# 192459/lmc-atomi

Measured on AMD Instinct MI355X. Metric: lmc_chain_iterations_per_s, higher is better.
Workload: dtype f32; 1 GPU; 512x512 MYULA deblur (5x5 uniform box blur, sigma=0.75) + isotropic TV prox K=10 (tau_reg=0.3), 1024 chains/GPU x 1 GPU, Philox noise, x0=0, posterior moments every 1 it; chains_per_gpu=1024, chains_total=1024, tv_iters=10, sampler=MYULA (algs.py:477-587), parallelism=chains sharded x1, collective=none

## Files before the change

include/lmc_atomi.h:

```cpp
#ifndef LMC_ATOMI_H
#define LMC_ATOMI_H

#include <stddef.h>
#include <stdint.h>

#ifdef __cplusplus
extern "C" {
#endif

#define LMC_ATOMI_ABI_VERSION 3

typedef enum lmc_status {
  LMC_OK = 0,
  LMC_E_INVALID = -1,
  LMC_E_UNSUPPORTED = -2,
  LMC_E_HIP = -3,
  LMC_E_NOMEM = -4,
  LMC_E_STATE = -5
} lmc_status;

typedef enum lmc_data_kind {
  LMC_DATA_NONE = 0,
  LMC_DATA_IDENTITY = 1,
  LMC_DATA_BLUR = 2,
  LMC_DATA_MASK = 3
} lmc_data_kind;

typedef enum lmc_prior_kind {
  LMC_PRIOR_NONE = 0,
  LMC_PRIOR_L2 = 1,
  LMC_PRIOR_L1 = 2,
  LMC_PRIOR_TV_ISO = 3,
  LMC_PRIOR_TV_ANISO = 4,
  LMC_PRIOR_HAAR_L1 = 5,
  LMC_PRIOR_EPROX = 6
} lmc_prior_kind;

typedef enum lmc_ncvx_kind {
  LMC_NCVX_NONE = 0,
  LMC_NCVX_MC_TV = 1,
  LMC_NCVX_ME_TV = 2,
  LMC_NCVX_MC_TV_ANISO = 3,
  LMC_NCVX_ME_TV_ANISO = 4
} lmc_ncvx_kind;

typedef enum lmc_noise_mode {
  LMC_NOISE_PHILOX = 0,
  LMC_NOISE_INJECTED = 1,
  LMC_NOISE_NONE = 2
} lmc_noise_mode;

#define LMC_MAX_BLUR 9
#define LMC_MAX_TV_ITERS 64

typedef struct lmc_problem {
  uint32_t struct_size;
  int32_t H, W;
  int32_t data_kind;
  float sigma_f;
  const float* y_dev;
  const float* mask_dev;
  int32_t kh, kw, oy, ox;
  const float* h_host;
  int32_t prior_kind;
  float prior_sigma;
  int32_t tv_niter;
  float tv_step;
  const float* tv_betas_host;
  int32_t ncvx_kind;
  float ncvx_lambda;
  float ncvx_gamma;
  int32_t ncvx_niter;
  int32_t tv_lagged_output;
  float tv_rtol;
  int32_t step_variant;
  float implicit_tol;
  int32_t tv_warm;
  float ncvx_rtol;
  int32_t tv_exit_path;
  int32_t iterations_per_launch;
  int32_t moments_overlap;
  int32_t moments_bg_workgroups;
  int32_t graph_replay;
  int32_t eprox_kind;
  float eprox_p0, eprox_p1;
  int32_t eprox_scale_mask;
  const float* prox_scale;
  int64_t prox_scale_chain_stride;
  int32_t prox_scale_pixel_stride;
} lmc_problem;

int lmc_version(void);
const char* lmc_last_error(void);
int lmc_device_info(int* device, int* n_cu, size_t* lds_bytes, size_t* hbm_bytes);
int lmc_hbm_copy_probe(size_t bytes, int32_t reps, float* gbs_out, void* stream);


int lmc_blur(const float* x_dev, float* out_dev, int64_t n_img, int32_t H, int32_t W,
             const float* h_host, int32_t kh, int32_t kw, int32_t oy, int32_t ox, int32_t adjoint, void* stream);

int lmc_gradient(const float* x_dev, float* out_dev, int64_t n_img, int32_t H, int32_t W, void* stream);
int lmc_gradient_adjoint(const float* y_dev, float* out_dev, int64_t n_img, int32_t H, int32_t W, void* stream);

int lmc_fused_eval(const lmc_problem* prob, const float* x_dev, float* out_dev, int64_t n_img,
                   float a, float t, float b, float pt, void* stream);

size_t lmc_l2_prox_workspace_bytes(int64_t n_img, int32_t H, int32_t W);
int lmc_l2_prox(const lmc_problem* prob, const float* x_dev, float* out_dev, int64_t n_img, float tau, int32_t niter,
                int32_t warm, void* workspace_dev, void* stream);

int lmc_energies(const lmc_problem* prob, const float* x_dev, int64_t n_img,
                 double* f_out_dev, double* g_out_dev, void* stream);

int lmc_haar_l1_prox(const float* x_dev, float* out_dev, int64_t n_img, int32_t H, int32_t W, float thr, void* stream);

int lmc_chain_probes(const float* x_dev, float* out_dev, int64_t n_img, int32_t H, int32_t W, int32_t ph, int32_t pw, void* stream);

int lmc_dual_project(const float* y_dev, float* out_dev, int64_t n_img, int32_t H, int32_t W,
                     float radius, int32_t isotropic, void* stream);

typedef enum lmc_eprox_kind {
  LMC_EPROX_LAPLACE = 0,
  LMC_EPROX_UNCENTERED_LAPLACE = 1,
  LMC_EPROX_GAUSSIAN = 2,
  LMC_EPROX_GEN_GAUSSIAN_4_3 = 3,
  LMC_EPROX_GEN_GAUSSIAN_3_2 = 4,
  LMC_EPROX_GEN_GAUSSIAN_3 = 5,
  LMC_EPROX_GEN_GAUSSIAN_4 = 6,
  LMC_EPROX_HUBER = 7,
  LMC_EPROX_SMOOTHED_LAPLACE = 8,
  LMC_EPROX_EXP = 9,
  LMC_EPROX_GAMMA = 10,
  LMC_EPROX_CHI = 11,
  LMC_EPROX_UNIFORM = 12,
  LMC_EPROX_TRIANGULAR = 13,
  LMC_EPROX_LAPLACE_CONJ = 14
} lmc_eprox_kind;
int lmc_prox_elementwise(int32_t kind, const float* x_dev, float* out_dev, int64_t n,
                         const float* params_host, int32_t n_params, void* stream);


typedef struct lmc_sampler lmc_sampler;

typedef struct lmc_myula_config {
  uint32_t struct_size;
  lmc_problem problem;
  int32_t n_chains;
  int64_t chain_offset;
  float tau, gamma, epsg;
  uint64_t seed;
  int32_t noise_mode;
  int32_t moments;
  int32_t burn_in;
  int32_t thin;
} lmc_myula_config;

int lmc_myula_create(const lmc_myula_config* cfg, lmc_sampler** out);
void lmc_sampler_destroy(lmc_sampler* s);

int lmc_mymala_create(const lmc_myula_config* cfg, lmc_sampler** out);
int lmc_sampler_get_acceptance(lmc_sampler* s, uint64_t* accepted_dev, double* last_log_alpha_dev, void* stream);

int lmc_sampler_set_state(lmc_sampler* s, const float* x_dev, void* stream);
int lmc_sampler_get_state(lmc_sampler* s, float* x_dev, void* stream);
int lmc_sampler_step(lmc_sampler* s, int32_t n_iters, const float* noise_dev, void* stream);
int64_t lmc_sampler_iteration(const lmc_sampler* s);
int lmc_sampler_set_iteration(lmc_sampler* s, int64_t it);

int lmc_sampler_get_moments(lmc_sampler* s, double* sum_dev, double* sumsq_dev, uint64_t* count, void* stream);
int lmc_sampler_reset_moments(lmc_sampler* s, void* stream);
int lmc_sampler_energies(lmc_sampler* s, double* f_out_dev, double* g_out_dev, void* stream);
int lmc_sampler_noise(lmc_sampler* s, int64_t iteration, float* out_dev, void* stream);
int lmc_sampler_enable_timing(lmc_sampler* s, int32_t on);
int lmc_sampler_last_step_timing(lmc_sampler* s, float* total_ms, int32_t* n_launches);
const char* lmc_sampler_kernel_name(const lmc_sampler* s);
int lmc_sampler_tv_exit_stats(lmc_sampler* s, int32_t which, int32_t* passes_dev, uint64_t* reruns_host, void* stream);

#define LMC_RCCL_UNIQUE_ID_BYTES 128
int lmc_rccl_available(void);
int lmc_rccl_unique_id(void* id128_host);
int lmc_rccl_comm_create(void** comm_out, int32_t world, int32_t rank, const void* id128_host);
int lmc_rccl_comm_destroy(void* comm);
int lmc_allreduce_moments(lmc_sampler* s, void* rccl_comm, double* sum_dev, double* sumsq_dev, uint64_t* count, void* stream);

typedef struct lmc_ulpda_config {
  uint32_t struct_size;
  lmc_problem problem;
  int32_t n_chains;
  int64_t chain_offset;
  float tau, mu, theta;
  int32_t gfirst;
  int32_t cg_niter;
  int32_t warm;
  const float* z_dev;
  uint64_t seed;
  int32_t noise_mode;
  int32_t moments, burn_in, thin;
} lmc_ulpda_config;

int lmc_ulpda_create(const lmc_ulpda_config* cfg, lmc_sampler** out);
int lmc_sampler_set_dual(lmc_sampler* s, const float* y_dev, void* stream);
int lmc_sampler_get_dual(lmc_sampler* s, float* y_dev, void* stream);
int lmc_sampler_set_steps(lmc_sampler* s, float tau, float mu);

float lmc_set_cg_tolerance(float tol);

int lmc_set_step_variant(int32_t variant);

#ifdef __cplusplus
}
#endif
#endif
```

lmc_atomi_amd/_capi.py:

```python
from __future__ import annotations

import ctypes as C
import os
import threading

_HERE = os.path.dirname(os.path.abspath(__file__))
LIB_PATH = os.path.join(_HERE, "lib", "liblmc_atomi.so")
ABI_VERSION = 3

DATA_NONE, DATA_IDENTITY, DATA_BLUR, DATA_MASK = 0, 1, 2, 3
PRIOR_NONE, PRIOR_L2, PRIOR_L1, PRIOR_TV_ISO, PRIOR_TV_ANISO, PRIOR_HAAR_L1, PRIOR_EPROX = 0, 1, 2, 3, 4, 5, 6
NOISE_PHILOX, NOISE_INJECTED, NOISE_NONE = 0, 1, 2
NCVX_NONE, NCVX_MC_TV, NCVX_ME_TV, NCVX_MC_TV_ANISO, NCVX_ME_TV_ANISO = 0, 1, 2, 3, 4
MAX_BLUR = 9
MAX_TV_ITERS = 64
(EPROX_LAPLACE, EPROX_UNCENTERED_LAPLACE, EPROX_GAUSSIAN, EPROX_GEN_GAUSSIAN_4_3, EPROX_GEN_GAUSSIAN_3_2,
 EPROX_GEN_GAUSSIAN_3, EPROX_GEN_GAUSSIAN_4, EPROX_HUBER, EPROX_SMOOTHED_LAPLACE, EPROX_EXP, EPROX_GAMMA,
 EPROX_CHI, EPROX_UNIFORM, EPROX_TRIANGULAR, EPROX_LAPLACE_CONJ) = range(15)


class LMCError(RuntimeError):

    def __init__(self, code, msg):
        super().__init__(f"liblmc_atomi error {code}: {msg}")
        self.code = code


class lmc_problem(C.Structure):
    _fields_ = [
        ("struct_size", C.c_uint32),
        ("H", C.c_int32), ("W", C.c_int32),
        ("data_kind", C.c_int32),
        ("sigma_f", C.c_float),
        ("y_dev", C.c_void_p),
        ("mask_dev", C.c_void_p),
        ("kh", C.c_int32), ("kw", C.c_int32), ("oy", C.c_int32), ("ox", C.c_int32),
        ("h_host", C.POINTER(C.c_float)),
        ("prior_kind", C.c_int32),
        ("prior_sigma", C.c_float),
        ("tv_niter", C.c_int32),
        ("tv_step", C.c_float),
        ("tv_betas_host", C.POINTER(C.c_float)),
        ("ncvx_kind", C.c_int32),
        ("ncvx_lambda", C.c_float),
        ("ncvx_gamma", C.c_float),
        ("ncvx_niter", C.c_int32),
        ("tv_lagged_output", C.c_int32),
        ("tv_rtol", C.c_float),
        ("step_variant", C.c_int32),
        ("implicit_tol", C.c_float),
        ("tv_warm", C.c_int32),
        ("ncvx_rtol", C.c_float),
        ("tv_exit_path", C.c_int32),
        ("iterations_per_launch", C.c_int32),
        ("moments_overlap", C.c_int32),
        ("moments_bg_workgroups", C.c_int32),
        ("graph_replay", C.c_int32),
        ("eprox_kind", C.c_int32), ("eprox_p0", C.c_float), ("eprox_p1", C.c_float), ("eprox_scale_mask", C.c_int32),
        ("prox_scale", C.c_void_p), ("prox_scale_chain_stride", C.c_int64), ("prox_scale_pixel_stride", C.c_int32),
    ]


class lmc_myula_config(C.Structure):
    _fields_ = [
        ("struct_size", C.c_uint32),
        ("problem", lmc_problem),
        ("n_chains", C.c_int32),
        ("chain_offset", C.c_int64),
        ("tau", C.c_float), ("gamma", C.c_float), ("epsg", C.c_float),
        ("seed", C.c_uint64),
        ("noise_mode", C.c_int32),
        ("moments", C.c_int32),
        ("burn_in", C.c_int32),
        ("thin", C.c_int32),
    ]


class lmc_ulpda_config(C.Structure):
    _fields_ = [
        ("struct_size", C.c_uint32),
        ("problem", lmc_problem),
        ("n_chains", C.c_int32),
        ("chain_offset", C.c_int64),
        ("tau", C.c_float), ("mu", C.c_float), ("theta", C.c_float),
        ("gfirst", C.c_int32),
        ("cg_niter", C.c_int32),
        ("warm", C.c_int32),
        ("z_dev", C.c_void_p),
        ("seed", C.c_uint64),
        ("noise_mode", C.c_int32),
        ("moments", C.c_int32), ("burn_in", C.c_int32), ("thin", C.c_int32),
    ]


_P = C.c_void_p
_F = C.POINTER(C.c_float)
_SIGNATURES = {
    "lmc_version": (C.c_int, []),
    "lmc_last_error": (C.c_char_p, []),
    "lmc_device_info": (C.c_int, [C.POINTER(C.c_int), C.POINTER(C.c_int), C.POINTER(C.c_size_t), C.POINTER(C.c_size_t)]),
    "lmc_hbm_copy_probe": (C.c_int, [C.c_size_t, C.c_int32, C.POINTER(C.c_float), _P]),
    "lmc_blur": (C.c_int, [_P, _P, C.c_int64, C.c_int32, C.c_int32, _F, C.c_int32, C.c_int32, C.c_int32, C.c_int32, C.c_int32, _P]),
    "lmc_gradient": (C.c_int, [_P, _P, C.c_int64, C.c_int32, C.c_int32, _P]),
    "lmc_gradient_adjoint": (C.c_int, [_P, _P, C.c_int64, C.c_int32, C.c_int32, _P]),
    "lmc_fused_eval": (C.c_int, [C.POINTER(lmc_problem), _P, _P, C.c_int64, C.c_float, C.c_float, C.c_float, C.c_float, _P]),
    "lmc_l2_prox_workspace_bytes": (C.c_size_t, [C.c_int64, C.c_int32, C.c_int32]),
    "lmc_l2_prox": (C.c_int, [C.POINTER(lmc_problem), _P, _P, C.c_int64, C.c_float, C.c_int32, C.c_int32, _P, _P]),
    "lmc_energies": (C.c_int, [C.POINTER(lmc_problem), _P, C.c_int64, _P, _P, _P]),
    "lmc_mymala_create": (C.c_int, [C.POINTER(lmc_myula_config), C.POINTER(_P)]),
    "lmc_sampler_get_acceptance": (C.c_int, [_P, _P, _P, _P]),
    "lmc_set_cg_tolerance": (C.c_float, [C.c_float]),
    "lmc_chain_probes": (C.c_int, [_P, _P, C.c_int64, C.c_int32, C.c_int32, C.c_int32, C.c_int32, _P]),
    "lmc_haar_l1_prox": (C.c_int, [_P, _P, C.c_int64, C.c_int32, C.c_int32, C.c_float, _P]),
    "lmc_dual_project": (C.c_int, [_P, _P, C.c_int64, C.c_int32, C.c_int32, C.c_float, C.c_int32, _P]),
    "lmc_prox_elementwise": (C.c_int, [C.c_int32, _P, _P, C.c_int64, _F, C.c_int32, _P]),
    "lmc_myula_create": (C.c_int, [C.POINTER(lmc_myula_config), C.POINTER(_P)]),
    "lmc_sampler_destroy": (None, [_P]),
    "lmc_sampler_set_state": (C.c_int, [_P, _P, _P]),
    "lmc_sampler_get_state": (C.c_int, [_P, _P, _P]),
    "lmc_sampler_step": (C.c_int, [_P, C.c_int32, _P, _P]),
    "lmc_sampler_iteration": (C.c_int64, [_P]),
    "lmc_sampler_set_iteration": (C.c_int, [_P, C.c_int64]),
    "lmc_sampler_get_moments": (C.c_int, [_P, _P, _P, C.POINTER(C.c_uint64), _P]),
    "lmc_sampler_reset_moments": (C.c_int, [_P, _P]),
    "lmc_sampler_energies": (C.c_int, [_P, _P, _P, _P]),
    "lmc_sampler_noise": (C.c_int, [_P, C.c_int64, _P, _P]),
    "lmc_sampler_enable_timing": (C.c_int, [_P, C.c_int32]),
    "lmc_sampler_last_step_timing": (C.c_int, [_P, C.POINTER(C.c_float), C.POINTER(C.c_int32)]),
    "lmc_sampler_kernel_name": (C.c_char_p, [_P]),
    "lmc_sampler_tv_exit_stats": (C.c_int, [_P, C.c_int32, _P, C.POINTER(C.c_uint64), _P]),
    "lmc_set_step_variant": (C.c_int, [C.c_int32]),
    "lmc_ulpda_create": (C.c_int, [C.POINTER(lmc_ulpda_config), C.POINTER(_P)]),
    "lmc_sampler_set_dual": (C.c_int, [_P, _P, _P]),
    "lmc_sampler_get_dual": (C.c_int, [_P, _P, _P]),
    "lmc_sampler_set_steps": (C.c_int, [_P, C.c_float, C.c_float]),
    "lmc_rccl_available": (C.c_int, []),
    "lmc_rccl_unique_id": (C.c_int, [_P]),
    "lmc_rccl_comm_create": (C.c_int, [C.POINTER(_P), C.c_int32, C.c_int32, _P]),
    "lmc_rccl_comm_destroy": (C.c_int, [_P]),
    "lmc_allreduce_moments": (C.c_int, [_P, _P, _P, _P, C.POINTER(C.c_uint64), _P]),
}
RCCL_UNIQUE_ID_BYTES = 128
VARIANTS = ["auto", "tile", "(removed)", "split", "point", "block", "rows", "pipe", "pipe2"]

_lib = None
_lock = threading.Lock()


def load(path: str | None = None):
    global _lib
    with _lock:
        if _lib is not None:
            return _lib
        import torch
        p = path or os.environ.get("LMC_ATOMI_LIB", LIB_PATH)
        if not os.path.exists(p):
            raise ImportError(
                f"{p} not found: build it with `python -c 'import __graft_entry__ as g; g.build()'` "
                "(or `make -C lmc_atomi_amd/csrc`).  lmc_atomi_amd has no CPU fallback.")
        lib = C.CDLL(p, mode=C.RTLD_GLOBAL)
        for name, (res, args) in _SIGNATURES.items():
            fn = getattr(lib, name)
            fn.restype = res
            fn.argtypes = args
        v = lib.lmc_version()
        if v != ABI_VERSION:
            raise ImportError(f"liblmc_atomi ABI {v} != binding ABI {ABI_VERSION}")
        _lib = lib
        return lib


def check(rc: int):
    if rc != 0:
        raise LMCError(rc, load().lmc_last_error().decode("utf-8", "replace"))


def exported_symbols():
    return sorted(_SIGNATURES)
```

lmc_atomi_amd/algs.py:

```python
from __future__ import annotations

import ctypes as C
import time

import numpy as np
import torch
from numpy.random import default_rng

from . import _capi, _dev
from .proximal import _Problem


def _prior_descriptor(proxg):
    if proxg is None:
        return {"prior_kind": _capi.PRIOR_NONE}
    fn = getattr(proxg, "prior_descriptor", None)
    if fn is None:
        raise NotImplementedError(
            f"{type(proxg).__name__} has no device functor (prior_descriptor()); new proxes are added as "
            "functors compiled into liblmc_atomi -- there is no CPU fallback")
    return fn()


def _data_descriptor(proxf):
    if proxf is None:
        return {"data_kind": _capi.DATA_NONE}
    fn = getattr(proxf, "descriptor", None)
    if fn is None:
        raise NotImplementedError(f"{type(proxf).__name__} has no device functor (descriptor())")
    return fn()


class MYULASampler:

    def __init__(self, proxf, proxg, dims, n_chains=1, tau=None, gamma=0.1, epsg=1.0, seed=0,
                 chain_offset=0, noise="philox", moments=False, burn_in=0, thin=1, device=None, variant=None, tv_warm=None, policy=None):
        if tau is None:
            raise NotImplementedError("tau=None (backtracking) is not implemented by the reference loop either")
        self.dims = (int(dims[0]), int(dims[1]))
        self.n_chains = int(n_chains)
        self.device = _dev.device(device)
        self.proxf, self.proxg = proxf, proxg
        opts = {"step_variant": variant or 0}
        if tv_warm is not None:
            opts["tv_warm"] = bool(tv_warm)
        opts.update(policy or {})
        self.epsg = epsg
        if np.asarray(epsg).size > 1:
            opts["prox_scale"] = self._epsg_array(epsg)
            epsg = 1.0
        self._problem = _Problem(self.dims, _data_descriptor(proxf), _prior_descriptor(proxg), self.device, options=opts)
        cfg = _capi.lmc_myula_config()
        cfg.struct_size = C.sizeof(_capi.lmc_myula_config)
        cfg.problem = self._problem.c
        cfg.n_chains = self.n_chains
        cfg.chain_offset = int(chain_offset)
        cfg.tau, cfg.gamma, cfg.epsg = float(tau), float(gamma), float(epsg)
        cfg.seed = int(seed) & 0xFFFFFFFFFFFFFFFF
        cfg.noise_mode = {"philox": _capi.NOISE_PHILOX, "injected": _capi.NOISE_INJECTED, "none": _capi.NOISE_NONE}[noise]
        cfg.moments = 1 if moments else 0
        cfg.burn_in = int(burn_in)
        cfg.thin = int(thin)
        self.noise_mode = noise
        self.moments_on = bool(moments)
        self._h = C.c_void_p()
        with torch.cuda.device(self.device):
            _capi.check(getattr(_dev.lib(), self._create_fn)(C.byref(cfg), C.byref(self._h)))

    _create_fn = "lmc_myula_create"

    def _epsg_array(self, epsg):
        e = np.asarray(epsg, dtype=np.float32)
        n = self.dims[0] * self.dims[1]
        if e.size == n and e.shape in ((n,), self.dims):
            cs, ps = 0, 1
        elif e.shape == (self.n_chains,):
            cs, ps = 1, 0
        elif e.size == self.n_chains * n and e.shape[0] == self.n_chains:
            cs, ps = n, 1
        else:
            raise ValueError(f"epsg of shape {e.shape} matches neither the image {self.dims}, nor the {self.n_chains} chains, nor both")
        return _dev.to_dev(np.ascontiguousarray(e.ravel()), self.device), cs, ps

    def close(self):
        if getattr(self, "_h", None) is not None and self._h.value:
            _dev.lib().lmc_sampler_destroy(self._h)
            self._h = C.c_void_p()

    __del__ = close

    def __enter__(self):
        return self

    def __exit__(self, *exc):
        self.close()

    @property
    def shape(self):
        return (self.n_chains,) + self.dims

    def set_state(self, x):
        xt = _dev.to_dev(x, self.device)
        n = self.dims[0] * self.dims[1]
        if xt.numel() == n:
            xt = xt.reshape(1, *self.dims).expand(self.shape).contiguous()
        if xt.numel() != self.n_chains * n:
            raise ValueError(f"state of shape {tuple(xt.shape)} does not match {self.shape}")
        _capi.check(_dev.lib().lmc_sampler_set_state(self._h, _dev.ptr(xt), _dev.stream_ptr(self.device)))
        torch.cuda.current_stream(self.device).synchronize()

    def get_state(self, out=None):
        if out is None:
            out = torch.empty(self.shape, dtype=torch.float32, device=self.device)
        _capi.check(_dev.lib().lmc_sampler_get_state(self._h, _dev.ptr(out), _dev.stream_ptr(self.device)))
        return out

    @property
    def iteration(self):
        return int(_dev.lib().lmc_sampler_iteration(self._h))

    @iteration.setter
    def iteration(self, it):
        _capi.check(_dev.lib().lmc_sampler_set_iteration(self._h, int(it)))

    def step(self, n_iters=1, noise=None):
        nt = None
        if noise is not None:
            nt = _dev.to_dev(noise, self.device)
            if nt.numel() != n_iters * self.n_chains * self.dims[0] * self.dims[1]:
                raise ValueError("noise must have shape [n_iters, n_chains, H, W]")
        _capi.check(_dev.lib().lmc_sampler_step(self._h, int(n_iters), _dev.ptr(nt), _dev.stream_ptr(self.device)))
        if nt is not None:
            torch.cuda.current_stream(self.device).synchronize()

    def enable_timing(self, on=True):
        _capi.check(_dev.lib().lmc_sampler_enable_timing(self._h, 1 if on else 0))

    def last_step_timing(self):
        ms, n = C.c_float(), C.c_int32()
        _capi.check(_dev.lib().lmc_sampler_last_step_timing(self._h, C.byref(ms), C.byref(n)))
        return ms.value, n.value

    @property
    def kernel_name(self):
        return _dev.lib().lmc_sampler_kernel_name(self._h).decode()

    def tv_exit_stats(self, which="prior"):
        passes = torch.empty(self.n_chains, dtype=torch.int32, device=self.device)
        rr = (C.c_uint64 * 4)()
        _capi.check(_dev.lib().lmc_sampler_tv_exit_stats(self._h, {"prior": 0, "ncvx": 1}[which], _dev.ptr(passes), rr, _dev.stream_ptr(self.device)))
        return passes, [int(v) for v in rr]

    def energies(self):
        f = torch.empty(self.n_chains, dtype=torch.float64, device=self.device)
        g = torch.empty(self.n_chains, dtype=torch.float64, device=self.device)
        _capi.check(_dev.lib().lmc_sampler_energies(self._h, _dev.ptr(f), _dev.ptr(g), _dev.stream_ptr(self.device)))
        return f, g

    def noise_field(self, iteration):
        out = torch.empty(self.shape, dtype=torch.float32, device=self.device)
        _capi.check(_dev.lib().lmc_sampler_noise(self._h, int(iteration), _dev.ptr(out), _dev.stream_ptr(self.device)))
        return out

    def moments(self):
        s1 = torch.empty(self.dims, dtype=torch.float64, device=self.device)
        s2 = torch.empty(self.dims, dtype=torch.float64, device=self.device)
        cnt = C.c_uint64()
        _capi.check(_dev.lib().lmc_sampler_get_moments(self._h, _dev.ptr(s1), _dev.ptr(s2), C.byref(cnt),
                                                       _dev.stream_ptr(self.device)))
        return s1, s2, int(cnt.value)

    def reset_moments(self):
        _capi.check(_dev.lib().lmc_sampler_reset_moments(self._h, _dev.stream_ptr(self.device)))

    def allreduce_moments(self, rccl_comm):
        s1 = torch.empty(self.dims, dtype=torch.float64, device=self.device)
        s2 = torch.empty(self.dims, dtype=torch.float64, device=self.device)
        cnt = C.c_uint64()
        comm = rccl_comm if isinstance(rccl_comm, C.c_void_p) else C.c_void_p(int(rccl_comm or 0))
        _capi.check(_dev.lib().lmc_allreduce_moments(self._h, comm, _dev.ptr(s1), _dev.ptr(s2), C.byref(cnt),
                                                     _dev.stream_ptr(self.device)))
        return s1, s2, int(cnt.value)


class ULPDASampler(MYULASampler):

    def __init__(self, proxf, proxg, A, dims, n_chains=1, tau=None, mu=None, theta=1.0, gfirst=True, z=None, seed=0,
                 chain_offset=0, noise="philox", moments=False, burn_in=0, thin=1, device=None, variant=None, implicit_tol=None):
        from .operators import Gradient
        from .proximal import L1, L21
        if not isinstance(A, Gradient):
            raise NotImplementedError("ULPDA on the GPU supports A = Gradient (the reference's operator, prox_lmc_deconv.py:98)")
        if isinstance(proxg, L21):
            prior = {"prior_kind": _capi.PRIOR_TV_ISO, "prior_sigma": proxg.sigma, "tv_niter": 1, "tv_betas": [0.0]}
        elif isinstance(proxg, L1):
            prior = {"prior_kind": _capi.PRIOR_TV_ANISO, "prior_sigma": proxg.sigma}
        else:
            raise NotImplementedError(f"{type(proxg).__name__} has no dual-prox device functor (L21 or L1 expected)")
        self.dims = (int(dims[0]), int(dims[1]))
        self.n_chains = int(n_chains)
        self.device = _dev.device(device)
        self.proxf, self.proxg = proxf, proxg
        tol = 0.0 if implicit_tol is None else (float(implicit_tol) if implicit_tol > 0 else -1.0)
        self._problem = _Problem(self.dims, _data_descriptor(proxf), prior, self.device,
                                 options={"step_variant": variant or 0, "implicit_tol": tol})
        cfg = _capi.lmc_ulpda_config()
        cfg.struct_size = C.sizeof(_capi.lmc_ulpda_config)
        cfg.problem = self._problem.c
        cfg.n_chains = self.n_chains
        cfg.chain_offset = int(chain_offset)
        cfg.tau, cfg.mu, cfg.theta = float(tau), float(mu), float(theta)
        cfg.gfirst = 1 if gfirst else 0
        cfg.cg_niter = int(getattr(proxf, "niter", 10) or 10)
        cfg.warm = 1 if getattr(proxf, "warm", True) else 0
        self._z = None
        if z is not None:
            self._z = _dev.to_dev(z, self.device).reshape(self.dims)
            cfg.z_dev = self._z.data_ptr()
        cfg.seed = int(seed) & 0xFFFFFFFFFFFFFFFF
        cfg.noise_mode = {"philox": _capi.NOISE_PHILOX, "injected": _capi.NOISE_INJECTED, "none": _capi.NOISE_NONE}[noise]
        cfg.moments = 1 if moments else 0
        cfg.burn_in = int(burn_in)
        cfg.thin = int(thin)
        self.noise_mode = noise
        self.moments_on = bool(moments)
        self._h = C.c_void_p()
        with torch.cuda.device(self.device):
            _capi.check(_dev.lib().lmc_ulpda_create(C.byref(cfg), C.byref(self._h)))

    def set_steps(self, tau, mu):
        _capi.check(_dev.lib().lmc_sampler_set_steps(self._h, float(tau), float(mu)))

    def set_dual(self, y):
        yt = _dev.to_dev(y, self.device)
        n2 = 2 * self.dims[0] * self.dims[1]
        if yt.numel() == n2:
            yt = yt.reshape(1, n2).expand(self.n_chains, n2).contiguous()
        if yt.numel() != self.n_chains * n2:
            raise ValueError("dual state must have 2*H*W entries per chain")
        _capi.check(_dev.lib().lmc_sampler_set_dual(self._h, _dev.ptr(yt), _dev.stream_ptr(self.device)))
        torch.cuda.current_stream(self.device).synchronize()

    def get_dual(self):
        out = torch.empty((self.n_chains, 2) + self.dims, dtype=torch.float32, device=self.device)
        _capi.check(_dev.lib().lmc_sampler_get_dual(self._h, _dev.ptr(out), _dev.stream_ptr(self.device)))
        return out


def UnadjustedLangevinPrimalDual(proxf, proxg, A, x0, tau, mu, y0=None, z=None, theta=1., niter=10, seed=0, gfirst=True,
                                 callback=None, callbacky=False, returny=False, show=False, *, n_chains=None, dims=None,
                                 rng="philox", chain_offset=0, burn_in=0, thin=1, device=None, diagnostics=None):
    if dims is None:
        dims = getattr(A, "dims", None) or getattr(proxf, "dims", None)
    if dims is None:
        raise ValueError("image shape unknown: pass dims=(ny, nx)")
    many = n_chains is not None
    C_ = int(n_chains) if many else 1
    n = int(dims[0]) * int(dims[1])
    if rng not in ("philox", "pcg64"):
        raise ValueError("rng must be 'philox' or 'pcg64'")
    if rng == "pcg64" and C_ != 1:
        raise ValueError("rng='pcg64' reproduces the reference's single chain; use n_chains=None")
    taus = np.full(niter, tau, dtype=np.float64) if np.isscalar(tau) else np.asarray(tau, dtype=np.float64)
    mus = np.full(niter, mu, dtype=np.float64) if np.isscalar(mu) else np.asarray(mu, dtype=np.float64)
    smp = ULPDASampler(proxf, proxg, A, dims, n_chains=C_, tau=taus[0], mu=mus[0], theta=theta, gfirst=gfirst, z=z,
                       seed=seed, chain_offset=chain_offset, noise="injected" if rng == "pcg64" else "philox",
                       moments=many, burn_in=burn_in, thin=thin, device=device)
    try:
        smp.set_state(x0)
        if y0 is not None:
            smp.set_dual(y0)
        tstart = time.time()
        if show:
            print('Unadjusted Langevin primal-dual (lmc_atomi_amd / HIP): U(x) = f(x) + x^T z + g(Ax)\n'
                  '---------------------------------------------------------\n'
                  'Proximal operator (f): %s\nProximal operator (g): %s\nLinear operator (A): %s\n'
                  'tau = %s\t\tmu = %s\ntheta = %.2f\t\tniter = %d\tchains = %d\n' %
                  (type(proxf), type(proxg), type(A), str(taus[0]), str(mus[0]), theta, niter, C_))
            print('   Itn       x[0]          f         g o A      U = f + g o A')
        host_rng = default_rng(seed) if rng == "pcg64" else None
        xs = np.empty((niter, n), dtype=np.float64) if not many else None
        ys = np.empty((niter, 2 * n), dtype=np.float64) if (returny and not many) else None
        tracer = None
        if diagnostics and many:
            from .diagnostics import ChainTrace
            tracer = ChainTrace(smp, (8, 8) if diagnostics is True else diagnostics)
        for it in range(niter):
            smp.set_steps(taus[it], mus[it])
            if host_rng is not None:
                xi = host_rng.standard_normal(n)
                smp.step(1, noise=xi.reshape(1, 1, *smp.dims))
            else:
                smp.step(1)
            if not many:
                xs[it] = smp.get_state().reshape(-1).cpu().numpy()
                if returny or callbacky:
                    yk = smp.get_dual().reshape(-1).cpu().numpy()
                    if returny:
                        ys[it] = yk
                if callback is not None:
                    callback(xs[it], yk) if callbacky else callback(xs[it])
            elif callback is not None:
                callback(smp.get_state(), smp.get_dual()) if callbacky else callback(smp.get_state())
            if tracer is not None and it >= burn_in and (it - burn_in) % thin == 0:
                tracer.record()
            if show and (it < 10 or niter - it < 10 or it % max(niter // 10, 1) == 0):
                f, g = smp.energies()
                x00 = float(smp.get_state().reshape(-1)[0])
                print('%6g  %12.5e  %10.3e  %10.3e      %10.3e' % (it + 1, x00, float(f.mean()), float(g.mean()),
                                                                  float((f + g).mean())))
        if show:
            print('\nTotal time (s) = %.2f' % (time.time() - tstart))
            print('---------------------------------------------------------\n')
        if not many:
            return (xs, ys) if returny else xs
        s1, s2, cnt = smp.moments()
        f, g = smp.energies()
        state = smp.get_state()
        torch.cuda.current_stream().synchronize()
        mean, var = mean_var_from_moments(s1, s2, max(cnt, 1))
        diag = tracer.summary() if tracer is not None and len(tracer) else None
        return MYULAResult(state, mean, var, cnt, f, g, time.time() - tstart, diagnostics=diag,
                           trace=tracer.trace() if diag is not None else None)
    finally:
        smp.close()


def mean_var_from_moments(s1, s2, count):
    mean = s1 / count
    var = s2 / count - mean * mean
    return mean, var


class MYULAResult:

    def __init__(self, state, mean, var, count, energy_f, energy_g, elapsed, diagnostics=None, trace=None):
        self.state, self.mean, self.var, self.count = state, mean, var, count
        self.energy_f, self.energy_g, self.elapsed = energy_f, energy_g, elapsed
        self.diagnostics, self.trace = diagnostics, trace


def MoreauYosidaUnadjustedLangevin(proxf, proxg, x0, tau=None, gamma=.1, epsg=1., niter=10, seed=0,
                                   callback=None, show=False, *, n_chains=None, dims=None, rng="philox",
                                   chain_offset=0, burn_in=0, thin=1, device=None, diagnostics=None):
    if dims is None:
        dims = getattr(proxf, "dims", None) or getattr(proxg, "dims", None)
    if dims is None:
        raise ValueError("image shape unknown: pass dims=(ny, nx)")
    many = n_chains is not None
    C_ = int(n_chains) if many else 1
    n = int(dims[0]) * int(dims[1])
    if rng not in ("philox", "pcg64"):
        raise ValueError("rng must be 'philox' or 'pcg64'")
    if rng == "pcg64" and C_ != 1:
        raise ValueError("rng='pcg64' reproduces the reference's single chain; use n_chains=None")
    smp = MYULASampler(proxf, proxg, dims, n_chains=C_, tau=tau, gamma=gamma, epsg=epsg, seed=seed,
                       chain_offset=chain_offset, noise="injected" if rng == "pcg64" else "philox",
                       moments=many, burn_in=burn_in, thin=thin, device=device)
    try:
        smp.set_state(x0)
        tstart = time.time()
        if show:
            print('Moreau--Yosida Unadjusted Langevin (lmc_atomi_amd / HIP)\n'
                  '---------------------------------------------------------\n'
                  'Proximal operator (f): %s\nProximal operator (g): %s\n'
                  'tau = %s\tgamma=%10e\nepsg = %s\tniter = %d\tchains = %d\n' %
                  (type(proxf), type(proxg), str(tau), gamma, str(epsg) if np.asarray(epsg).size == 1 else 'Multi', niter, C_))
            print('   Itn       x[0]          f           g     J = f + eps*g')
        if not many:
            samples = np.empty((niter, n), dtype=np.asarray(x0).dtype if not isinstance(x0, torch.Tensor) else np.float32)
            host_rng = default_rng(seed) if rng == "pcg64" else None
            buf = torch.empty(smp.shape, dtype=torch.float32, device=smp.device)
            for it in range(niter):
                if host_rng is not None:
                    xi = host_rng.standard_normal(n)
                    smp.step(1, noise=xi.reshape(1, 1, *smp.dims))
                else:
                    smp.step(1)
                smp.get_state(buf)
                xk = buf.reshape(-1).cpu().numpy()
                samples[it] = xk
                if callback is not None:
                    callback(samples[it])
                if show and (it < 10 or niter - it < 10 or it % max(niter // 10, 1) == 0):
                    f, g = smp.energies()
                    pf, pg = float(f[0]), float(g[0])
                    print('%6g  %12.5e  %10.3e  %10.3e  %10.3e' % (it + 1, samples[it][0], pf, pg, pf + float(np.sum(epsg * pg))))
            if show:
                print('\nTotal time (s) = %.2f' % (time.time() - tstart))
                print('---------------------------------------------------------\n')
            return samples
        tracer = None
        if diagnostics:
            from .diagnostics import ChainTrace
            tracer = ChainTrace(smp, (8, 8) if diagnostics is True else diagnostics)
        next_rec = burn_in + 1
        done = 0
        while done < niter:
            chunk = niter - done if (callback is None and not show) else 1
            if tracer is not None and next_rec > done:
                chunk = min(chunk, next_rec - done)
            smp.step(chunk)
            done += chunk
            if tracer is not None and done == next_rec:
                tracer.record()
                next_rec += thin
            if callback is not None:
                callback(smp.get_state())
            if show and (done <= 10 or niter - done < 10 or (done - 1) % max(niter // 10, 1) == 0):
                f, g = smp.energies()
                x00 = float(smp.get_state()[0, 0, 0])
                print('%6g  %12.5e  %10.3e  %10.3e  %10.3e' % (done, x00, float(f.mean()), float(g.mean()),
                                                              float((f + (epsg if np.asarray(epsg).size == 1 else float(np.sum(epsg))) * g).mean())))
        s1, s2, cnt = smp.moments()
        f, g = smp.energies()
        state = smp.get_state()
        torch.cuda.current_stream().synchronize()
        mean, var = mean_var_from_moments(s1, s2, max(cnt, 1))
        diag = tracer.summary() if tracer is not None and len(tracer) else None
        return MYULAResult(state, mean, var, cnt, f, g, time.time() - tstart, diagnostics=diag,
                           trace=tracer.trace() if diag is not None else None)
    finally:
        smp.close()


class MYMALASampler(MYULASampler):

    _create_fn = "lmc_mymala_create"

    def acceptance(self):
        acc = torch.empty(self.n_chains, dtype=torch.int64, device=self.device)
        la = torch.empty(self.n_chains, dtype=torch.float64, device=self.device)
        _capi.check(_dev.lib().lmc_sampler_get_acceptance(self._h, _dev.ptr(acc), _dev.ptr(la), _dev.stream_ptr(self.device)))
        return acc, la

    def acceptance_rate(self):
        acc, _ = self.acceptance()
        return acc.double() / max(self.iteration, 1)


def MoreauYosidaMetropolisAdjustedLangevin(proxf, proxg, x0, tau=None, gamma=.1, epsg=1., niter=10, seed=0, callback=None, *,
                                           n_chains=1, dims=None, chain_offset=0, burn_in=0, thin=1, device=None):
    if dims is None:
        dims = getattr(proxf, "dims", None) or getattr(proxg, "dims", None)
    if dims is None:
        raise ValueError("image shape unknown: pass dims=(ny, nx)")
    smp = MYMALASampler(proxf, proxg, dims, n_chains=int(n_chains), tau=tau, gamma=gamma, epsg=epsg, seed=seed,
                        chain_offset=chain_offset, moments=True, burn_in=burn_in, thin=thin, device=device)
    try:
        smp.set_state(x0)
        tstart = time.time()
        if callback is None:
            smp.step(niter)
        else:
            for _ in range(niter):
                smp.step(1)
                callback(smp.get_state())
        s1, s2, cnt = smp.moments()
        f, g = smp.energies()
        state = smp.get_state()
        acc, _ = smp.acceptance()
        torch.cuda.current_stream().synchronize()
        mean, var = mean_var_from_moments(s1, s2, max(cnt, 1))
        res = MYULAResult(state, mean, var, cnt, f, g, time.time() - tstart)
        res.accepted = acc
        res.acceptance_rate = acc.double() / max(niter, 1)
        return res
    finally:
        smp.close()


def set_cg_tolerance(tol=1e-6):
    return float(_dev.lib().lmc_set_cg_tolerance(float(tol)))


def set_step_variant(variant="auto"):
    names = _capi.VARIANTS
    if variant not in names or variant.startswith("("):
        raise ValueError(f"unknown step-kernel variant {variant!r} (the one-group 'stream' kernel of ABI 1 was removed)")
    prev = _dev.lib().lmc_set_step_variant(names.index(variant))
    if prev < 0:
        _capi.check(prev)
    return names[prev]
```

lmc_atomi_amd/csrc/lmc_host.h:

```cpp
#pragma once
#include <string>
#include <vector>

#include "lmc_launch.h"

namespace lmc::host {

int fail(int code, const char* fmt, ...);

#define HIP_TRY(expr)                                                                          \
  do {                                                                                         \
    hipError_t e_ = (expr);                                                                    \
    if (e_ != hipSuccess) return fail(LMC_E_HIP, "%s failed: %s", #expr, hipGetErrorString(e_)); \
  } while (0)

inline hipStream_t S(void* s) { return reinterpret_cast<hipStream_t>(s); }

struct Problem {
  int H = 0, W = 0;
  int data_kind = 0;
  float sigma_f = 0.f;
  const float* y = nullptr;
  const float* mask = nullptr;
  lmc::BlurTaps taps{};
  int prior_kind = 0;
  float prior_sigma = 0.f;
  int tv_niter = 0;
  float tv_step = 0.125f;
  float betas[lmc::kMaxTvIters] = {};
  int ncvx_kind = 0;
  float ncvx_lambda = 0.f, ncvx_gamma = 1.f;
  int ncvx_niter = 0;
  int ncvx_aniso = 0;
  int tv_warm = 0;
  float tv_rtol = 0.f;
  float ncvx_rtol = 0.f;
  int tv_exit_path = 0;
  int iters_per_launch = 0, moments_overlap = 0, moments_bg_wgs = 0;
  int cheb_pair = 1;
  int eprox_kind = 0, eprox_mask = 0;
  float eprox_p0 = 0.f, eprox_p1 = 0.f;
  const float* prox_scale = nullptr;
  int64_t prox_scale_cs = 0, prox_scale_ps = 0;
  int variant = 0;
  float implicit_tol = 0.f;
};

struct RtState {
  int* kc = nullptr;
  int* start = nullptr;
  int* pred = nullptr;
  double* obj = nullptr;
  unsigned long long* reruns = nullptr;
  int stride = 0;
  size_t n = 0;
  hipError_t need(size_t n_img, int niter) {
    if (n_img <= n && niter + 1 <= stride) return hipSuccess;
    release();
    hipError_t e = hipMalloc(&kc, sizeof(int) * n_img);
    if (e == hipSuccess) e = hipMalloc(&start, sizeof(int) * n_img);
    if (e == hipSuccess) e = hipMalloc(&pred, sizeof(int) * n_img);
    if (e == hipSuccess) e = hipMalloc(&obj, sizeof(double) * n_img * (size_t)(niter + 1));
    if (e == hipSuccess) e = hipMalloc(&reruns, sizeof(unsigned long long) * 4);
    if (e == hipSuccess) e = hipMemset(pred, 0, sizeof(int) * n_img);
    if (e == hipSuccess) e = hipMemset(reruns, 0, sizeof(unsigned long long) * 4);
    if (e == hipSuccess) { n = n_img; stride = niter + 1; }
    return e;
  }
  void release() {
    if (kc) (void)hipFree(kc);
    if (start) (void)hipFree(start);
    if (pred) (void)hipFree(pred);
    if (obj) (void)hipFree(obj);
    if (reruns) (void)hipFree(reruns);
    kc = start = pred = nullptr; obj = nullptr; reruns = nullptr; n = 0; stride = 0;
  }
};

struct Scratch {
  float* state[2] = {nullptr, nullptr};
  float* extra = nullptr;
  float* prox = nullptr;
  float* rtmp = nullptr;
  double* dbl = nullptr;
  RtState rt_tv, rt_me;
  size_t n_state[2] = {0, 0}, n_extra = 0, n_prox = 0, n_rtmp = 0, n_dbl = 0;
  template <class T>
  static hipError_t grow(T*& p, size_t& have, size_t n) {
    if (n <= have) return hipSuccess;
    if (p) (void)hipFree(p);
    p = nullptr; have = 0;
    hipError_t e = hipMalloc(&p, sizeof(T) * n);
    if (e == hipSuccess) have = n;
    return e;
  }
  hipError_t need_state(size_t n) {
    hipError_t e = grow(state[0], n_state[0], n);
    return e == hipSuccess ? grow(state[1], n_state[1], n) : e;
  }
  hipError_t need_extra(size_t n) { return grow(extra, n_extra, n); }
  hipError_t need_prox(size_t n) { return grow(prox, n_prox, n); }
  hipError_t need_rtmp(size_t n) { return grow(rtmp, n_rtmp, n); }
  hipError_t need_dbl(size_t n) { return grow(dbl, n_dbl, n); }
};
Scratch& scratch_here();

struct DeviceGuard {
  int prev = -1;
  bool switched = false;
  explicit DeviceGuard(int dev) {
    if (dev < 0) return;
    if (hipGetDevice(&prev) == hipSuccess && prev != dev) switched = hipSetDevice(dev) == hipSuccess;
  }
  ~DeviceGuard() { if (switched) (void)hipSetDevice(prev); }
};

constexpr int kSideBatches = 4;

int fill_taps(lmc::BlurTaps& T, const float* h, int kh, int kw, int oy, int ox);
void default_betas(float* b, int n);
int load_problem(const lmc_problem* p, Problem& q);
int make_step_args(const Problem& q, float a, float t, float b, float pt, float s, lmc::StepArgs& A);
void sanitize_pointers(lmc::StepArgs& A);
int variant_of(const Problem& q);
float tol_of(const Problem& q);
hipError_t launch_step(const lmc::StepArgs& A_in, int variant, hipStream_t st, const char** name, float* state0 = nullptr,
                       float* state1 = nullptr, float* pxbuf = nullptr);

int cg_solve_fused(const Problem& q, float ts, float* u, const float* rhs, float* r, float* p, float* qq, double* scal,
                   int64_t C, int niter, const float* zero_y, hipStream_t st, float* alt_out = nullptr, float** result = nullptr);

bool needs_tv_state(const Problem& q);
int tv_prox_rtol(const Problem& q, float pt, const float* x, float* sol, float* tmp, double* obj, int* flag, int64_t n, float* st0, float* st1,
                 hipStream_t st);
int me_tv_prox(const Problem& q, const float* x, float* extra, int64_t n_img, float* state0, float* state1, hipStream_t st, RtState* rt = nullptr);
int tv_prior_rt(const Problem& q, float pt, lmc::StepArgs& A, RtState& rt, float* proxbuf, float* st0, float* st1, hipStream_t st);
int tv_prior_rt_mode(const Problem& q, const lmc::StepArgs& A_probe, float pt);
lmc::EnergyArgs energy_args(const Problem& q);
int me_tv_energy(const Problem& q, const float* x, int64_t n_img, double* f_out, float* extra, float* st0, float* st1,
                 double* dbl , hipStream_t st, RtState* rt);

}

struct lmc_sampler {
  int kind = 0;
  int device = -1;
  float mu = 0, theta = 1;
  int gfirst = 0, cg_niter = 0, warm = 1;
  const float* z = nullptr;
  float* xhat = nullptr; float* ydual = nullptr; float* uw = nullptr; float* rhs = nullptr;
  float* uw2 = nullptr;
  float* cr = nullptr; float* cp = nullptr; float* cq = nullptr; float* ctmp = nullptr; float* xi = nullptr;
  float* htb = nullptr; double* scal = nullptr; float* zero_y = nullptr;
  float* tvstate[2] = {nullptr, nullptr};
  float* tvwarm[2] = {nullptr, nullptr};
  int wcur = 0;
  float* extra = nullptr;
  float* pxbuf = nullptr;
  float* rtmp = nullptr; double* robj = nullptr; int* rflag = nullptr;
  lmc::host::RtState rt_tv, rt_me;
  int pol_pair = 1;
  int pol_blockpair = 1;
  int pol_overlap = 0;
  int pol_bg_wgs = -1;
  lmc::host::Problem prob;
  int C = 0;
  int64_t chain_offset = 0;
  float tau = 0, gamma = 0, epsg = 1;
  uint64_t seed = 0;
  int noise_mode = 0;
  int moments = 0, burn_in = 0, thin = 1;
  int64_t iteration = 0;
  uint64_t count = 0;
  float* x[2] = {nullptr, nullptr};
  float* xspare = nullptr;
  float* xmid[2] = {nullptr, nullptr};
  int cur = 0;
  double* s1 = nullptr;
  double* s2 = nullptr;
  double* packed = nullptr;
  lmc::StepArgs base{};
  float* mx = nullptr; float* xp = nullptr; float* mxp = nullptr;
  double* mala_d = nullptr;
  int* flag = nullptr;
  unsigned long long* nacc = nullptr;
  bool mala_fresh = false;
  hipStream_t side = nullptr;
  hipEvent_t side_ev[1 + lmc::host::kSideBatches] = {};
  std::vector<hipEvent_t> ev;
  bool timing = false;
  bool timed = false;
  int last_launches = 0;
  std::string kernel_name;
};
```

lmc_atomi_amd/csrc/lmc_launch.h:

```cpp
#pragma once
#include "lmc_common.h"

namespace lmc {

struct EnergyArgs {
  int H, W;
  int data_kind;
  float sigma_f;
  const float* y;
  const float* mask;
  BlurTaps blur;
  int prior_kind;
  float prior_sigma;
  int ncvx_kind;
  float ncvx_lambda, ncvx_gamma;
};

hipError_t launch_step_tile(StepArgs a, hipStream_t st);
bool tile_needs_chunks(const StepArgs& a);
hipError_t launch_step_tile_chunked(const StepArgs& a, float* state0, float* state1, hipStream_t st);
hipError_t launch_axpy_env(double* f, const double* tvv, const double* sq, int64_t n, float lambda, float gamma, hipStream_t st);
hipError_t launch_sqdiff(const float* a, const float* b, int64_t n_img, size_t img, double* out, hipStream_t st);
hipError_t launch_blur(const float* x, float* out, int64_t n_img, int H, int W, const BlurTaps& T, int adjoint,
                       hipStream_t st);
hipError_t launch_gradient(const float* x, float* out, int64_t n_img, int H, int W, bool adjoint, hipStream_t st);
hipError_t launch_dual_project(const float* y, float* out, int64_t n_img, int H, int W, float radius, int iso,
                               hipStream_t st);
hipError_t launch_eprox(int kind, const float* x, float* out, int64_t n, float p0, float p1, hipStream_t st);
hipError_t launch_prior_prox_scaled(int prior, int kind, const float* x, float* out, int64_t n_chains, int64_t img, const float* scale, int64_t cs, int64_t ps,
                                    float pt, float sigma, float p0, float p1, int mask, hipStream_t st);
hipError_t launch_haar_prox(const float* x, float* out, int64_t n_img, int H, int W, float thr, hipStream_t st);
hipError_t launch_chain_probes(const float* x, float* out, int64_t n_img, int H, int W, int ph, int pw, hipStream_t st);
hipError_t launch_haar_value(const float* x, int64_t n_img, int H, int W, float sigma, double* val, hipStream_t st);
hipError_t launch_mc_tv_add(const float* x, float* out, int64_t n_img, int H, int W, float coef, float gamma, hipStream_t st);
hipError_t launch_moments(const float* x, int C, int H, int W, double* s1, double* s2, hipStream_t st);
hipError_t launch_moments_bg(const float* x, int C, int H, int W, double* s1, double* s2, int n_wg, hipStream_t st);
hipError_t launch_energies(const float* x, int64_t n_img, const EnergyArgs& E, double* f_out, double* g_out,
                           hipStream_t st);
hipError_t launch_tv_objective(const float* x, const float* sol, int64_t n, int H, int W, float gam, const int* flag, double* obj, hipStream_t st);
hipError_t launch_tv_rtol_decide(int64_t n, double* prev, double* cur, int* flag, int pass, double rtol, int* n_active, hipStream_t st);
hipError_t launch_tv_rtol_select(const float* tmp, float* sol, const int* flag, int pass, int64_t n, size_t img, hipStream_t st);
hipError_t launch_tv1d_sol(const float* x, const float* rr, float* out, int64_t n, size_t N, float gam, const int* flag, hipStream_t st);
hipError_t launch_tv1d_iter(const float* x, const float* rr_in, float* p, float* rr_out, int64_t n, size_t N, float gam, float cstep, float beta, const int* flag,
                            hipStream_t st);
hipError_t launch_tv1d_objective(const float* x, const float* sol, int64_t n, size_t N, float gam, const int* flag, double* obj, hipStream_t st);
hipError_t launch_tv_rt_begin(int64_t n, const int* pred, int* kc, int* start, double* obj, int stride, int niter, hipStream_t st);
hipError_t launch_tv_rt_decide(int64_t n, int* kc, int* start, int* pred, double* obj, int stride, int niter, double rtol, int round,
                               unsigned long long* reruns, hipStream_t st);
int hbm_copy_probe_shapes();
hipError_t launch_hbm_copy_probe(const float* x, float* y, size_t n_floats, int shape, hipStream_t st);
hipError_t launch_noise(float* out, int C, int H, int W, uint32_t key0, uint32_t key1, uint32_t iteration,
                        uint32_t chain_offset, hipStream_t st);

}

namespace lmc {
bool point_supported(const StepArgs& a);
hipError_t launch_step_point(StepArgs a, hipStream_t st);
bool block_supported(const StepArgs& a);
bool block_pair_supported(const StepArgs& a);
hipError_t launch_step_block(const StepArgs& a, hipStream_t st);
bool rows_supported(const StepArgs& a);
hipError_t launch_step_rows(StepArgs a, hipStream_t st);
bool rows_pair_supported(const StepArgs& a);
hipError_t launch_step_rows_pair(StepArgs a, float* x_mid, hipStream_t st);
int centred_blur_taps(const StepArgs& a, float* uc, float* vc);
int centred_blur_taps(const BlurTaps& T, float* uc, float* vc);
bool pipe_supported(const StepArgs& a);
int pipe_links(const StepArgs& a);
hipError_t launch_step_pipe(StepArgs a, hipStream_t st, float* state0 = nullptr, float* state1 = nullptr, int teams = 0);
bool pipe_teams_covered(const StepArgs& a, int KT);
bool pipe_warm_supported(const StepArgs& a);
hipError_t launch_step_pipe_warm(StepArgs a, hipStream_t st);
bool pipe_rt_supported(const StepArgs& a);
hipError_t launch_step_pipe_rt(StepArgs a, hipStream_t st, float* state0 = nullptr, float* state1 = nullptr);
bool split_supported(const StepArgs& a);
hipError_t launch_step_split(StepArgs a, hipStream_t st);
}

namespace lmc {
hipError_t ulpda_dual_update(const float* xhat, float* y, int64_t C, int H, int W, float mu, float radius, int iso, hipStream_t st);
hipError_t ulpda_rhs(const float* x, const float* y, const float* z, const float* htb, float* rhs, int64_t C, int H, int W,
                     float tau, float ts, hipStream_t st);
hipError_t ulpda_me_rhs(const float* v, const float* extra, const float* htb, float* rhs, int64_t C, int H, int W, float coef,
                        float ts, hipStream_t st);
hipError_t ulpda_ncvx_rhs(const float* v, const float* htb, float* rhs, int64_t C, int H, int W, float coef, float gamma, float ts,
                          hipStream_t st);
hipError_t ulpda_pointwise_prox(const float* v, float* u, const float* b, const float* m, int64_t C, int H, int W, float ts,
                                int kind, hipStream_t st);
hipError_t ulpda_finish_philox(float* x, float* xhat, const float* u, int64_t C, int H, int W, float s, float theta, uint32_t key0,
                               uint32_t key1, uint32_t iteration, uint32_t chain_offset, hipStream_t st);
hipError_t ulpda_finish(float* x, float* xhat, const float* u, const float* xi, int64_t C, int H, int W, float s, float theta,
                        hipStream_t st);
hipError_t cg_dot(const float* p, const float* q, int64_t C, size_t img, double* pq, const int* done, hipStream_t st);
hipError_t cg_init(const float* rhs, const float* q, float* r, float* p, int64_t C, size_t img, double* rs, double* b2, hipStream_t st);
hipError_t cg_update(float* u, float* r, const float* p, const float* q, int64_t C, size_t img, const double* rs, const double* pq,
                     double* rs_new, const int* done, hipStream_t st);
hipError_t cg_dir(float* p, const float* r, int64_t C, size_t img, double* rs, const double* rs_new, const int* done, hipStream_t st);
hipError_t cheb_count(int64_t C, const double* stat, double inv_alpha2, double tol, double inv_log_inv_c, int kmax, int* count,
                      hipStream_t st);
hipError_t cg_check(int64_t C, const double* rsv, const double* b2, double tol2, int* done, hipStream_t st);

struct ChebPairArgs {
  int H, W, C;
  float cbox;
  const float* cur;
  const float* prv;
  const float* rhs;
  float* f1;
  float* f2;
  float* f2_last;
  float a0, tg0, b0, s0, a1, tg1, b1, s1;
  const int* run_count;
  int run_index, last_index, force_last;
  double* dot_out;
};
bool cheb_pair_supported(int H, int W, const BlurTaps& taps);
bool cheb_pair_pays(int64_t C, int H);
hipError_t launch_cheb_pair(ChebPairArgs a, const BlurTaps& taps, hipStream_t st);
}

namespace lmc {
hipError_t mala_propose(const float* mx, const float* xi, float* xp, int64_t C, size_t img, float s, double* d1, hipStream_t st);
hipError_t mala_propose_philox(const float* mx, float* xp, int64_t C, int H, int W, float s, uint32_t key0, uint32_t key1,
                               uint32_t iteration, uint32_t chain_offset, double* d1, hipStream_t st);
hipError_t mala_accept(int C, double* U, const double* fp, const double* gp, float epsg, const double* d1, const double* d2, float tau,
                       uint32_t key0, uint32_t key1, uint32_t iteration, uint32_t chain_offset, int* flag,
                       unsigned long long* nacc, double* log_alpha, hipStream_t st);
hipError_t mala_select(const int* flag, float* x, float* mx, const float* xp, const float* mxp, int64_t C, size_t img, int when,
                       hipStream_t st);
}
```

lmc_atomi_amd/csrc/lmc_problem.hip:

```cpp
#include <cmath>
#include <cstdlib>
#include <cstring>

#include "lmc_host.h"

namespace lmc::host {

int fill_taps(lmc::BlurTaps& T, const float* h, int kh, int kw, int oy, int ox) {
  if (!h) return fail(LMC_E_INVALID, "blur kernel pointer is NULL");
  if (kh < 1 || kw < 1 || kh > lmc::kMaxBlur || kw > lmc::kMaxBlur)
    return fail(LMC_E_UNSUPPORTED, "blur kernel %dx%d outside 1..%d", kh, kw, lmc::kMaxBlur);
  if (oy < 0 || oy >= kh || ox < 0 || ox >= kw) return fail(LMC_E_INVALID, "blur offset (%d,%d) outside kernel", oy, ox);
  T.kh = kh; T.kw = kw; T.oy = oy; T.ox = ox;
  std::memset(T.h, 0, sizeof T.h);
  std::memcpy(T.h, h, sizeof(float) * kh * kw);
  return LMC_OK;
}

void default_betas(float* b, int n) {
  double t = 1.0;
  for (int k = 0; k < n; ++k) {
    const double tn = (1.0 + std::sqrt(4.0 * t * t)) / 2.0;
    b[k] = (float)((t - 1.0) / tn);
    t = tn;
  }
}

int load_problem(const lmc_problem* p, Problem& q) {
  if (!p) return fail(LMC_E_INVALID, "lmc_problem is NULL");
  if (p->struct_size != sizeof(lmc_problem))
    return fail(LMC_E_INVALID, "lmc_problem.struct_size %u != %zu (ABI mismatch)", p->struct_size, sizeof(lmc_problem));
  if (p->H < 1 || p->W < 1 || (int64_t)p->H * p->W > (int64_t)1 << 30) return fail(LMC_E_INVALID, "bad image size %dx%d", p->H, p->W);
  q.H = p->H; q.W = p->W;
  q.data_kind = p->data_kind;
  q.sigma_f = p->sigma_f;
  q.y = p->y_dev;
  q.mask = p->mask_dev;
  switch (p->data_kind) {
    case LMC_DATA_NONE: break;
    case LMC_DATA_IDENTITY:
      if (!p->y_dev) return fail(LMC_E_INVALID, "data term needs y_dev");
      break;
    case LMC_DATA_MASK:
      if (!p->y_dev || !p->mask_dev) return fail(LMC_E_INVALID, "mask data term needs y_dev and mask_dev");
      break;
    case LMC_DATA_BLUR: {
      if (!p->y_dev) return fail(LMC_E_INVALID, "data term needs y_dev");
      int rc = fill_taps(q.taps, p->h_host, p->kh, p->kw, p->oy, p->ox);
      if (rc) return rc;
      break;
    }
    default: return fail(LMC_E_INVALID, "unknown data_kind %d", p->data_kind);
  }
  q.prior_kind = p->prior_kind;
  q.prior_sigma = p->prior_sigma;
  switch (p->prior_kind) {
    case LMC_PRIOR_NONE: case LMC_PRIOR_L2: case LMC_PRIOR_L1: case LMC_PRIOR_TV_ANISO: break;
    case LMC_PRIOR_EPROX:
      if (p->eprox_kind < 0 || p->eprox_kind > LMC_EPROX_LAPLACE_CONJ) return fail(LMC_E_INVALID, "unknown eprox_kind %d", p->eprox_kind);
      if (p->eprox_scale_mask < 0 || p->eprox_scale_mask > 3) return fail(LMC_E_INVALID, "eprox_scale_mask must be 0..3");
      if (!(p->eprox_p0 == p->eprox_p0) || !(p->eprox_p1 == p->eprox_p1)) return fail(LMC_E_INVALID, "eprox parameter is NaN");
      q.eprox_kind = p->eprox_kind; q.eprox_mask = p->eprox_scale_mask; q.eprox_p0 = p->eprox_p0; q.eprox_p1 = p->eprox_p1;
      break;
    case LMC_PRIOR_HAAR_L1:
      if ((p->H & 7) || (p->W & 7)) return fail(LMC_E_UNSUPPORTED, "the Haar-l1 prior needs H and W to be multiples of 8 (got %dx%d)", p->H, p->W);
      break;
    case LMC_PRIOR_TV_ISO:
      if (p->tv_niter < 1 || p->tv_niter > lmc::kMaxTvIters)
        return fail(LMC_E_UNSUPPORTED, "tv_niter %d outside 1..%d", p->tv_niter, lmc::kMaxTvIters);
      if (!(p->tv_rtol >= 0.f) || p->tv_rtol >= 1.f) return fail(LMC_E_INVALID, "tv_rtol must be in [0, 1)");
      q.tv_rtol = p->tv_rtol;
      q.tv_niter = p->tv_niter - (p->tv_lagged_output ? 1 : 0);
      q.tv_step = p->tv_step > 0.f ? p->tv_step : 0.125f;
      if (p->tv_betas_host) std::memcpy(q.betas, p->tv_betas_host, sizeof(float) * p->tv_niter);
      else default_betas(q.betas, p->tv_niter);
      break;
    default: return fail(LMC_E_INVALID, "unknown prior_kind %d", p->prior_kind);
  }
  if (p->prior_kind != LMC_PRIOR_NONE && p->prior_kind != LMC_PRIOR_EPROX && !(p->prior_sigma >= 0.f)) return fail(LMC_E_INVALID, "prior_sigma must be >= 0");
  if (p->ncvx_kind != LMC_NCVX_NONE) {
    if (p->ncvx_kind != LMC_NCVX_MC_TV && p->ncvx_kind != LMC_NCVX_ME_TV && p->ncvx_kind != LMC_NCVX_MC_TV_ANISO && p->ncvx_kind != LMC_NCVX_ME_TV_ANISO)
      return fail(LMC_E_INVALID, "unknown ncvx_kind %d", p->ncvx_kind);
    if (!(p->ncvx_gamma > 0.f)) return fail(LMC_E_INVALID, "ncvx_gamma must be > 0");
    const bool me = p->ncvx_kind == LMC_NCVX_ME_TV || p->ncvx_kind == LMC_NCVX_ME_TV_ANISO;
    if (me && (p->ncvx_niter < 1 || p->ncvx_niter > lmc::kMaxTvIters))
      return fail(LMC_E_INVALID, "ncvx_niter %d outside 1..%d", p->ncvx_niter, lmc::kMaxTvIters);
    q.ncvx_kind = p->ncvx_kind; q.ncvx_lambda = p->ncvx_lambda; q.ncvx_gamma = p->ncvx_gamma;
    if (p->ncvx_kind == LMC_NCVX_ME_TV_ANISO) { q.ncvx_kind = LMC_NCVX_ME_TV; q.ncvx_aniso = 1; }
    if (p->ncvx_kind == LMC_NCVX_MC_TV_ANISO) { q.ncvx_kind = LMC_NCVX_MC_TV; q.ncvx_gamma = -p->ncvx_gamma; }
    q.ncvx_niter = p->ncvx_niter - ((me && p->tv_lagged_output) ? 1 : 0);
    if (me) {
      if (!(p->ncvx_rtol >= 0.f) || p->ncvx_rtol >= 1.f) return fail(LMC_E_INVALID, "ncvx_rtol must be in [0, 1)");
      q.ncvx_rtol = p->ncvx_rtol;
    }
  }
  if (p->tv_exit_path != 0 && p->tv_exit_path != 1) return fail(LMC_E_INVALID, "tv_exit_path must be 0 (device path where covered) or 1 (pass by pass)");
  q.tv_exit_path = p->tv_exit_path;
  if (p->iterations_per_launch < 0 || p->iterations_per_launch > 2) return fail(LMC_E_INVALID, "iterations_per_launch must be 0 (auto), 1 or 2");
  if (p->moments_overlap < -1 || p->moments_overlap > 1) return fail(LMC_E_INVALID, "moments_overlap must be 0 (auto), 1 (on) or -1 (off)");
  if (p->moments_bg_workgroups < 0 || p->graph_replay < 0 || p->graph_replay > 1) return fail(LMC_E_INVALID, "bad moments_bg_workgroups / graph_replay");
  q.iters_per_launch = p->iterations_per_launch; q.moments_overlap = p->moments_overlap;
  q.moments_bg_wgs = p->moments_bg_workgroups;
  {
    const char* e = getenv("LMC_CHEB_PAIR");
    const char* e2 = getenv("LMC_ITERS_PER_LAUNCH");
    const int ipl = q.iters_per_launch ? q.iters_per_launch : (e2 ? atoi(e2) : 0);
    q.cheb_pair = ipl == 1 ? 0 : (ipl == 2 ? 2 : (e ? atoi(e) : 1));
  }
  if (p->step_variant < 0 || p->step_variant > 8 || p->step_variant == 2)
    return fail(LMC_E_INVALID, "step_variant %d: 0 (library default), 1 tile, 3 split, 4 point, 5 block, 6 rows, 7 pipe, 8 pipe2", p->step_variant);
  q.variant = p->step_variant;
  if (p->prox_scale) {
    if (p->prior_kind != LMC_PRIOR_L2 && p->prior_kind != LMC_PRIOR_L1 && p->prior_kind != LMC_PRIOR_EPROX)
      return fail(LMC_E_UNSUPPORTED, "prox_scale (array-valued epsg) is built for the closed-form priors (l2, l1, prox.py closed forms) only");
    if (p->prox_scale_chain_stride < 0 || p->prox_scale_pixel_stride < 0) return fail(LMC_E_INVALID, "prox_scale strides must be >= 0");
    q.prox_scale = p->prox_scale; q.prox_scale_cs = p->prox_scale_chain_stride; q.prox_scale_ps = p->prox_scale_pixel_stride;
  }
  q.tv_warm = (p->tv_warm != 0 && p->prior_kind == LMC_PRIOR_TV_ISO) ? 1 : 0;
  if (!(p->implicit_tol == p->implicit_tol)) return fail(LMC_E_INVALID, "implicit_tol is NaN");
  q.implicit_tol = p->implicit_tol;
  return LMC_OK;
}

int make_step_args(const Problem& q, float a, float t, float b, float pt, float s, lmc::StepArgs& A) {
  std::memset(&A, 0, sizeof A);
  A.H = q.H; A.W = q.W;
  A.data_kind = (t == 0.f) ? LMC_DATA_NONE : q.data_kind;
  A.sigma_f = q.sigma_f;
  A.y = q.y; A.mask = q.mask;
  A.blur = q.taps;
  A.prior_kind = (b == 0.f) ? LMC_PRIOR_NONE : q.prior_kind;
  if (A.prior_kind == LMC_PRIOR_TV_ISO && q.tv_niter == 0) A.prior_kind = LMC_PRIOR_NONE;
  if (A.prior_kind == LMC_PRIOR_HAAR_L1) A.prior_p0 = pt * q.prior_sigma;
  if (A.prior_kind == LMC_PRIOR_L2) A.prior_p0 = 1.f / (1.f + pt * q.prior_sigma);
  if (A.prior_kind == LMC_PRIOR_L1) A.prior_p0 = pt * q.prior_sigma;
  if (A.prior_kind == LMC_PRIOR_EPROX) {
    A.eprox_kind = q.eprox_kind;
    A.prior_p0 = (q.eprox_mask & 1) ? pt * q.eprox_p0 : q.eprox_p0;
    A.prior_p1 = (q.eprox_mask & 2) ? pt * q.eprox_p1 : q.eprox_p1;
  }
  if (A.prior_kind == LMC_PRIOR_TV_ISO) {
    const float gam = pt * q.prior_sigma;
    if (!(gam > 0.f)) return fail(LMC_E_INVALID, "TV prox parameter must be > 0 (got %g)", (double)gam);
    A.tv.niter = q.tv_niter;
    A.tv.gamma = gam;
    A.tv.c = q.tv_step / gam;
    std::memcpy(A.tv.betas, q.betas, sizeof(float) * q.tv_niter);
  }
  if (t != 0.f && q.ncvx_kind == LMC_NCVX_MC_TV) {
    A.ncvx_kind = q.ncvx_kind; A.ncvx_lambda = q.ncvx_lambda; A.ncvx_gamma = q.ncvx_gamma; A.ncvx_inv_gamma = 1.f / q.ncvx_gamma;
  }
  A.a = a; A.t = t; A.b = b; A.s = s;
  A.noise_mode = LMC_NOISE_NONE;
  return LMC_OK;
}

void sanitize_pointers(lmc::StepArgs& A) {
  if (!A.y) A.y = A.x_in;
  if (!A.mask) A.mask = A.x_in;
  if (!A.noise) A.noise = A.x_in;
}

int g_variant = 0;
float g_cg_tol = 1e-6f;
int variant_of(const Problem& q) { return q.variant ? q.variant : g_variant; }
float tol_of(const Problem& q) { return q.implicit_tol > 0.f ? q.implicit_tol : (q.implicit_tol < 0.f ? 0.f : g_cg_tol); }

hipError_t launch_step(const lmc::StepArgs& A_in, int variant, hipStream_t st, const char** name, float* state0, float* state1, float* pxbuf) {
  int v = variant;
  if ((v == 0 || v == 5) && lmc::block_supported(A_in)) {
    if (name) *name = "myula_step_block_kernel";
    return lmc::launch_step_block(A_in, st);
  }
  if ((v == 0 || v == 5) && A_in.ncvx_kind == LMC_NCVX_MC_TV) {
    lmc::StepArgs B = A_in;
    B.ncvx_kind = LMC_NCVX_NONE;
    if (lmc::block_supported(B)) {
      if (name) *name = "myula_step_block_kernel";
      hipError_t e = lmc::launch_step_block(B, st);
      if (e != hipSuccess) return e;
      return lmc::launch_mc_tv_add(A_in.x_in, A_in.x_out, A_in.C, A_in.H, A_in.W, A_in.t * A_in.ncvx_lambda, A_in.ncvx_gamma, st);
    }
  }
  if (v == 5) return hipErrorInvalidConfiguration;
  lmc::StepArgs A = A_in;
  if (A.prior_kind == LMC_PRIOR_HAAR_L1) {
    if (!pxbuf) return hipErrorInvalidConfiguration;
    hipError_t e = lmc::launch_haar_prox(A.x_in, pxbuf, A.C, A.H, A.W, A.prior_p0, st);
    if (e != hipSuccess) return e;
    A.prior_kind = LMC_PRIOR_NONE;
    A.prox_ext = pxbuf;
  }
  if ((v == 0 || v == 6) && lmc::rows_supported(A)) {
    if (name) *name = "myula_step_rows_kernel";
    return lmc::launch_step_rows(A, st);
  }
  if (v == 6) return hipErrorInvalidConfiguration;
  if (v == 0 || v == 7 || v == 8) {
    const int links = lmc::pipe_links(A);
    if (links == 1 || (links > 1 && state0 && state1 && v != 8)) {
      if (name) *name = "myula_step_pipe_kernel";
      return lmc::launch_step_pipe(A, st, state0, state1, v == 7 ? 1 : v == 8 ? 2 : 0);
    }
  }
  if (v == 7 || v == 8) return hipErrorInvalidConfiguration;
  if (A.prior_kind == LMC_PRIOR_EPROX) {
    if ((v == 0 || v == 4) && lmc::point_supported(A)) v = 4;
    else {
      if (!pxbuf) return hipErrorInvalidConfiguration;
      hipError_t e = lmc::launch_eprox(A.eprox_kind, A.x_in, pxbuf, (int64_t)A.C * A.H * A.W, A.prior_p0, A.prior_p1, st);
      if (e != hipSuccess) return e;
      A.prior_kind = LMC_PRIOR_NONE;
      A.prox_ext = pxbuf;
    }
  }
  if (v == 0) v = lmc::split_supported(A) ? 3 : (lmc::point_supported(A) ? 4 : 1);
  if (v == 4) {
    if (!lmc::point_supported(A)) return hipErrorInvalidConfiguration;
    if (name) *name = "myula_step_point_kernel";
    return lmc::launch_step_point(A, st);
  }
  if (v == 3) {
    if (!lmc::split_supported(A)) return hipErrorInvalidConfiguration;
    if (name) *name = "myula_step_split_kernel";
    return lmc::launch_step_split(A, st);
  }
  if (name) *name = "myula_step_tile_kernel";
  if (lmc::tile_needs_chunks(A)) {
    if (!state0 || !state1) return hipErrorInvalidConfiguration;
    return lmc::launch_step_tile_chunked(A, state0, state1, st);
  }
  return lmc::launch_step_tile(A, st);
}

}

using namespace lmc::host;

extern "C" {

float lmc_set_cg_tolerance(float tol) {
  const float prev = g_cg_tol;
  if (tol >= 0.f) g_cg_tol = tol;
  return prev;
}

int lmc_set_step_variant(int32_t variant) {
  if (variant < 0 || variant > 8 || variant == 2)
    return fail(LMC_E_INVALID, "variant must be 0 (auto), 1 (tile), 3 (split), 4 (point), 5 (block), 6 (rows), 7 (pipe) or 8 (pipe2); 2 (the one-group "
                "streaming kernel of ABI 1) was removed");
  const int prev = g_variant;
  g_variant = variant;
  return prev;
}

}
```

lmc_atomi_amd/csrc/lmc_sampler.hip:

```cpp
#include <cmath>
#include <cstdlib>
#include <new>

#include "lmc_host.h"

using namespace lmc::host;

namespace {
int env_int(const char* name, int dflt) { const char* e = getenv(name); return e ? atoi(e) : dflt; }

template <class Cfg>
int check_config(const Cfg& cfg, bool steps_ok, const char* steps_msg) {
  if (cfg.n_chains < 1) return fail(LMC_E_INVALID, "n_chains must be >= 1");
  if (cfg.chain_offset < 0 || cfg.chain_offset + cfg.n_chains > 0xFFFFFFFFLL)
    return fail(LMC_E_INVALID, "global chain ids must fit 32 bits");
  if (!steps_ok) return fail(LMC_E_INVALID, "%s", steps_msg);
  if (cfg.noise_mode < LMC_NOISE_PHILOX || cfg.noise_mode > LMC_NOISE_NONE) return fail(LMC_E_INVALID, "bad noise_mode");
  return LMC_OK;
}

hipError_t alloc_moments(lmc_sampler* s) {
  if (!s->moments) return hipSuccess;
  const size_t mb = sizeof(double) * (size_t)s->prob.H * s->prob.W;
  hipError_t e = hipMalloc(&s->s1, mb);
  if (e == hipSuccess) e = hipMalloc(&s->s2, mb);
  if (e == hipSuccess) e = hipMemset(s->s1, 0, mb);
  if (e == hipSuccess) e = hipMemset(s->s2, 0, mb);
  return e;
}

int alloc_failed(lmc_sampler* s, hipError_t e) {
  const int rc = fail(e == hipErrorOutOfMemory ? LMC_E_NOMEM : LMC_E_HIP, "sampler allocation failed: %s", hipGetErrorString(e));
  lmc_sampler_destroy(s);
  return rc;
}
}

extern "C" {


int lmc_myula_create(const lmc_myula_config* cfg, lmc_sampler** out) {
  if (!cfg || !out) return fail(LMC_E_INVALID, "NULL argument");
  *out = nullptr;
  if (cfg->struct_size != sizeof(lmc_myula_config))
    return fail(LMC_E_INVALID, "lmc_myula_config.struct_size %u != %zu (ABI mismatch)", cfg->struct_size, sizeof(lmc_myula_config));
  int rc = check_config(*cfg, cfg->tau > 0.f && cfg->gamma > 0.f, "tau and gamma must be > 0");
  if (rc) return rc;
  if (cfg->moments && cfg->thin < 1) return fail(LMC_E_INVALID, "thin must be >= 1");
  lmc_sampler* s = new (std::nothrow) lmc_sampler();
  if (!s) return fail(LMC_E_NOMEM, "host allocation failed");
  rc = load_problem(&cfg->problem, s->prob);
  if (rc) { delete s; return rc; }
  if (hipGetDevice(&s->device) != hipSuccess) { delete s; return fail(LMC_E_HIP, "hipGetDevice failed"); }
  s->C = cfg->n_chains;
  s->chain_offset = cfg->chain_offset;
  s->tau = cfg->tau; s->gamma = cfg->gamma; s->epsg = cfg->epsg;
  s->seed = cfg->seed;
  s->noise_mode = cfg->noise_mode;
  s->moments = cfg->moments; s->burn_in = cfg->burn_in; s->thin = cfg->thin < 1 ? 1 : cfg->thin;
  rc = make_step_args(s->prob, 1.f - s->tau / s->gamma, s->tau, s->tau / s->gamma, s->epsg * s->gamma,
                      std::sqrt(2.f * s->tau), s->base);
  if (rc) { delete s; return rc; }
  s->base.C = s->C;
  s->base.noise_mode = s->noise_mode;
  s->base.key0 = (uint32_t)(s->seed & 0xFFFFFFFFu);
  s->base.key1 = (uint32_t)(s->seed >> 32);
  s->base.chain_offset = (uint32_t)s->chain_offset;
  const size_t nbytes = sizeof(float) * (size_t)s->C * s->prob.H * s->prob.W;
  hipError_t e = hipMalloc(&s->x[0], nbytes);
  if (e == hipSuccess) e = hipMalloc(&s->x[1], nbytes);
  if (e == hipSuccess) e = hipMemset(s->x[0], 0, nbytes);
  if (e == hipSuccess && needs_tv_state(s->prob)) {
    e = hipMalloc(&s->tvstate[0], 4 * nbytes);
    if (e == hipSuccess) e = hipMalloc(&s->tvstate[1], 4 * nbytes);
  }
  if (e == hipSuccess && s->prob.ncvx_kind == LMC_NCVX_ME_TV) e = hipMalloc(&s->extra, nbytes);
  if (e == hipSuccess && (s->prob.prior_kind == LMC_PRIOR_HAAR_L1 || s->prob.prior_kind == LMC_PRIOR_EPROX || s->prob.prox_scale)) e = hipMalloc(&s->pxbuf, nbytes);
  if (e == hipSuccess && s->prob.tv_rtol > 0.f && s->base.prior_kind == LMC_PRIOR_TV_ISO) {
    if (s->prob.tv_warm) { lmc_sampler_destroy(s); return fail(LMC_E_UNSUPPORTED, "tv_rtol > 0 and tv_warm exclude each other"); }
    const int mode = tv_prior_rt_mode(s->prob, s->base, s->epsg * s->gamma);
    if (mode != 2) e = s->rt_tv.need((size_t)s->C, s->prob.tv_niter);
    if (e == hipSuccess && mode != 1 && !s->pxbuf) e = hipMalloc(&s->pxbuf, nbytes);
    if (mode == 2) {
      if (e == hipSuccess) e = hipMalloc(&s->rtmp, nbytes);
      if (e == hipSuccess) e = hipMalloc(&s->robj, sizeof(double) * 2 * (size_t)s->C);
      if (e == hipSuccess) e = hipMalloc(&s->rflag, sizeof(int) * ((size_t)s->C + 1));
    }
  }
  if (e == hipSuccess && s->prob.ncvx_kind == LMC_NCVX_ME_TV && s->prob.ncvx_rtol > 0.f) e = s->rt_me.need((size_t)s->C, s->prob.ncvx_niter);
  {
    const Problem& q = s->prob;
    const int ipl = q.iters_per_launch ? q.iters_per_launch : env_int("LMC_ITERS_PER_LAUNCH", 0);
    s->pol_pair = ipl == 1 ? 0 : (ipl == 2 ? 2 : env_int("LMC_ROWS_PAIR", 1));
    s->pol_blockpair = ipl == 1 ? 0 : (ipl == 2 ? 1 : (env_int("LMC_BLOCK_PAIR", 1) != 0));
    s->pol_overlap = q.moments_overlap ? q.moments_overlap : (getenv("LMC_MOMENTS_OVERLAP") ? (env_int("LMC_MOMENTS_OVERLAP", 0) ? 1 : -1) : 0);
    s->pol_bg_wgs = q.moments_bg_wgs > 0 ? q.moments_bg_wgs : env_int("LMC_MOMENTS_BG_WGS", -1);
    if (q.prox_scale) { s->pol_pair = 0; s->pol_blockpair = 0; }
  }
  if (e == hipSuccess && s->prob.tv_warm) {
    lmc::StepArgs probe = s->base;
    probe.x_in = s->x[0];
    if (s->base.prior_kind != LMC_PRIOR_TV_ISO || !lmc::pipe_warm_supported(probe)) {
      lmc_sampler_destroy(s);
      return fail(LMC_E_UNSUPPORTED, "tv_warm: needs tv_niter in {1, 2, 3} (after tv_lagged_output) and the full-width pipeline kernel "
                  "(W > 128, W %% 4 == 0 (%% 8 above 256), separable blur <= 7 taps / pointwise / no data term)");
    }
    for (int i = 0; i < 2 && e == hipSuccess; ++i) {
      e = hipMalloc(&s->tvwarm[i], 2 * nbytes);
      if (e == hipSuccess) e = hipMemset(s->tvwarm[i], 0, 2 * nbytes);
    }
  }
  if (e == hipSuccess) e = alloc_moments(s);
  if (e != hipSuccess) return alloc_failed(s, e);
  s->kernel_name = "(no step launched yet)";
  *out = s;
  return LMC_OK;
}

void lmc_sampler_destroy(lmc_sampler* s) {
  if (!s) return;
  DeviceGuard dg(s->device);
  for (float* b : {s->xmid[0], s->xmid[1], s->xspare, s->zero_y, s->xhat, s->ydual, s->uw, s->uw2, s->rhs, s->cr, s->cp, s->cq, s->ctmp, s->xi, s->htb, s->tvstate[0], s->tvstate[1], s->extra, s->pxbuf,
                   s->mx, s->xp, s->mxp, s->tvwarm[0], s->tvwarm[1], s->rtmp})
    if (b) (void)hipFree(b);
  if (s->robj) (void)hipFree(s->robj);
  if (s->rflag) (void)hipFree(s->rflag);
  s->rt_tv.release();
  s->rt_me.release();
  if (s->mala_d) (void)hipFree(s->mala_d);
  if (s->flag) (void)hipFree(s->flag);
  if (s->nacc) (void)hipFree(s->nacc);
  if (s->scal) (void)hipFree(s->scal);
  if (s->x[0]) (void)hipFree(s->x[0]);
  if (s->x[1]) (void)hipFree(s->x[1]);
  if (s->s1) (void)hipFree(s->s1);
  if (s->s2) (void)hipFree(s->s2);
  if (s->packed) (void)hipFree(s->packed);
  for (hipEvent_t e : s->ev) (void)hipEventDestroy(e);
  if (s->side) { (void)hipStreamSynchronize(s->side); (void)hipStreamDestroy(s->side); }
  for (hipEvent_t e : s->side_ev) if (e) (void)hipEventDestroy(e);
  delete s;
}

int lmc_sampler_set_state(lmc_sampler* s, const float* x_dev, void* stream) {
  if (!s || !x_dev) return fail(LMC_E_INVALID, "NULL argument");
  DeviceGuard dg(s->device);
  const size_t nbytes = sizeof(float) * (size_t)s->C * s->prob.H * s->prob.W;
  HIP_TRY(hipMemcpyAsync(s->x[s->cur], x_dev, nbytes, hipMemcpyDeviceToDevice, S(stream)));
  if (s->kind == 1) HIP_TRY(hipMemcpyAsync(s->xhat, x_dev, nbytes, hipMemcpyDeviceToDevice, S(stream)));
  if (s->tvwarm[s->wcur]) HIP_TRY(hipMemsetAsync(s->tvwarm[s->wcur], 0, 2 * nbytes, S(stream)));
  s->mala_fresh = false;
  return LMC_OK;
}

int lmc_sampler_get_state(lmc_sampler* s, float* x_dev, void* stream) {
  if (!s || !x_dev) return fail(LMC_E_INVALID, "NULL argument");
  DeviceGuard dg(s->device);
  const size_t nbytes = sizeof(float) * (size_t)s->C * s->prob.H * s->prob.W;
  HIP_TRY(hipMemcpyAsync(x_dev, s->x[s->cur], nbytes, hipMemcpyDeviceToDevice, S(stream)));
  return LMC_OK;
}

static int ulpda_step(lmc_sampler* s, int32_t n_iters, const float* noise_dev, hipStream_t st);
static int mymala_step(lmc_sampler* s, int32_t n_iters, const float* noise_dev, hipStream_t st);

static int sampler_energies_at(lmc_sampler* s, const float* x, double* f_out_dev, double* g_out_dev, hipStream_t st) {
  HIP_TRY(lmc::launch_energies(x, s->C, energy_args(s->prob), f_out_dev, g_out_dev, st));
  if (s->prob.prior_kind == LMC_PRIOR_HAAR_L1 && g_out_dev)
    HIP_TRY(lmc::launch_haar_value(x, s->C, s->prob.H, s->prob.W, s->prob.prior_sigma, g_out_dev, st));
  if (s->prob.ncvx_kind == LMC_NCVX_ME_TV && f_out_dev) {
    Scratch& sc = scratch_here();
    HIP_TRY(sc.need_dbl(3 * (size_t)s->C + 2));
    int rc = me_tv_energy(s->prob, x, s->C, f_out_dev, s->extra, s->tvstate[0], s->tvstate[1], sc.dbl, st, &s->rt_me);
    if (rc) return rc;
  }
  return LMC_OK;
}

static bool kept(const lmc_sampler* s, int64_t it) { return s->moments && it >= s->burn_in && (it - s->burn_in) % s->thin == 0; }

static int me_tv_extra(lmc_sampler* s, lmc::StepArgs& A, hipStream_t st) {
  if (s->prob.ncvx_kind != LMC_NCVX_ME_TV) return LMC_OK;
  int rc = me_tv_prox(s->prob, A.x_in, s->extra, s->C, s->tvstate[0], s->tvstate[1], st, &s->rt_me);
  if (rc) return rc;
  A.extra = s->extra;
  A.extra_coef = -s->prob.ncvx_lambda / s->prob.ncvx_gamma;
  return LMC_OK;
}

static int sampler_update(lmc_sampler* s, const float* x_in, float* x_out, bool with_noise, const float* noise, uint32_t iteration,
                          hipStream_t st, const char** kname, double* f_out = nullptr, double* g_out = nullptr, bool* fused = nullptr) {
  lmc::StepArgs A = s->base;
  if (fused) *fused = false;
  if (f_out && g_out && (variant_of(s->prob) == 0 || variant_of(s->prob) == 7) && s->prob.ncvx_kind == LMC_NCVX_NONE && s->prob.prior_kind == LMC_PRIOR_TV_ISO) {
    lmc::StepArgs probe = A;
    probe.x_in = x_in;
    if (lmc::pipe_supported(probe)) {
      HIP_TRY(hipMemsetAsync(f_out, 0, sizeof(double) * s->C, st));
      HIP_TRY(hipMemsetAsync(g_out, 0, sizeof(double) * s->C, st));
      A.f_out = f_out; A.g_out = g_out; A.g_scale = s->prob.prior_sigma;
      if (fused) *fused = true;
    }
  }
  A.x_in = x_in;
  A.x_out = x_out;
  A.iteration = iteration;
  A.noise = noise;
  if (!with_noise) { A.s = 0.f; A.noise_mode = LMC_NOISE_NONE; A.noise = nullptr; }
  sanitize_pointers(A);
  int rc = me_tv_extra(s, A, st);
  if (rc) return rc;
  hipError_t e = launch_step(A, variant_of(s->prob), st, kname, s->tvstate[0], s->tvstate[1], s->pxbuf);
  if (e == hipErrorInvalidConfiguration) return fail(LMC_E_UNSUPPORTED, "no step-kernel variant covers this configuration");
  HIP_TRY(e);
  return LMC_OK;
}

struct SideMoments {
  lmc_sampler* s;
  hipStream_t st;
  bool overlap;
  int bg_wgs;
  const float* reads[kSideBatches][2] = {};
  int head = 0, n = 0;

  hipError_t wait_through(int i) {
    const int slot = (head + i) % kSideBatches;
    head = (slot + 1) % kSideBatches;
    n -= i + 1;
    return hipStreamWaitEvent(st, s->side_ev[1 + slot], 0);
  }
  hipError_t before_write(const float* a, const float* b = nullptr) {
    for (int i = n - 1; i >= 0; --i)
      for (const float* r : reads[(head + i) % kSideBatches])
        if (r && (r == a || r == b)) return wait_through(i);
    return hipSuccess;
  }
  hipError_t join() { return n ? wait_through(n - 1) : hipSuccess; }
  int keep(const float* a, const float* b, bool beside) {
    if (!a && !b) return LMC_OK;
    if (beside) {
      if (n == kSideBatches) HIP_TRY(wait_through(0));
      const int slot = (head + n) % kSideBatches;
      HIP_TRY(hipEventRecord(s->side_ev[0], st));
      HIP_TRY(hipStreamWaitEvent(s->side, s->side_ev[0], 0));
      for (const float* x : {a, b})
        if (x) HIP_TRY(lmc::launch_moments_bg(x, s->C, s->prob.H, s->prob.W, s->s1, s->s2, bg_wgs, s->side));
      HIP_TRY(hipEventRecord(s->side_ev[1 + slot], s->side));
      reads[slot][0] = a;
      reads[slot][1] = b;
      ++n;
    } else {
      HIP_TRY(join());
      for (const float* x : {a, b})
        if (x) HIP_TRY(lmc::launch_moments(x, s->C, s->prob.H, s->prob.W, s->s1, s->s2, st));
    }
    s->count += (uint64_t)s->C * ((a ? 1 : 0) + (b ? 1 : 0));
    return LMC_OK;
  }
};

static hipError_t xmid_array(lmc_sampler* s, float** out) {
  float*& xm = s->xmid[s->last_launches & 1];
  const hipError_t e = xm ? hipSuccess : hipMalloc(&xm, sizeof(float) * (size_t)s->C * s->prob.H * s->prob.W);
  *out = xm;
  return e;
}


static int myula_rows_pair(lmc_sampler* s, SideMoments& m, int left) {
  if (!s->pol_pair || left < 2 || s->tvwarm[0] || s->rtmp || s->prob.ncvx_kind != LMC_NCVX_NONE ||
      (variant_of(s->prob) != 0 && variant_of(s->prob) != 6) || (s->pol_pair != 2 && (long long)s->C * s->prob.H < (1 << 17)))
    return 0;
  lmc::StepArgs A = s->base;
  A.x_in = s->x[s->cur];
  A.iteration = (uint32_t)s->iteration;
  A.noise = nullptr;
  sanitize_pointers(A);
  if (!lmc::rows_pair_supported(A)) return 0;
  if (!s->xspare) HIP_TRY(hipMalloc(&s->xspare, sizeof(float) * (size_t)s->C * s->prob.H * s->prob.W));
  const bool keep_mid = kept(s, s->iteration), keep_out = kept(s, s->iteration + 1);
  float* mid = keep_mid ? s->x[s->cur ^ 1] : nullptr;
  if (keep_mid && m.overlap) HIP_TRY(xmid_array(s, &mid));
  HIP_TRY(m.before_write(s->xspare, mid));
  A.x_out = s->xspare;
  if (s->timing) HIP_TRY(hipEventRecord(s->ev[2 * s->last_launches], m.st));
  HIP_TRY(lmc::launch_step_rows_pair(A, mid, m.st));
  if (s->timing) HIP_TRY(hipEventRecord(s->ev[2 * s->last_launches + 1], m.st));
  s->kernel_name = "myula_step_rows_pair_kernel";
  int rc = m.keep(mid, keep_out ? s->xspare : nullptr, m.overlap);
  if (rc) return rc;
  std::swap(s->x[s->cur], s->xspare);
  s->iteration += 2;
  ++s->last_launches;
  return 2;
}

static int myula_block_pair(lmc_sampler* s, SideMoments& m, int left) {
  if (!s->pol_blockpair || left < 2 || s->tvwarm[0] || s->rtmp || s->prob.ncvx_kind != LMC_NCVX_NONE ||
      (variant_of(s->prob) != 0 && variant_of(s->prob) != 5))
    return 0;
  lmc::StepArgs A = s->base;
  A.x_in = s->x[s->cur];
  A.x_out = s->x[s->cur ^ 1];
  A.iteration = (uint32_t)s->iteration;
  A.noise = nullptr;
  sanitize_pointers(A);
  if (!lmc::block_pair_supported(A)) return 0;
  const bool four = left >= 4 && !kept(s, s->iteration) && !kept(s, s->iteration + 1) && !kept(s, s->iteration + 2);
  const int nf = four ? 4 : 2;
  const bool keep_mid = !four && kept(s, s->iteration), keep_out = kept(s, s->iteration + nf - 1);
  A.fused_iters = nf;
  A.x_mid = keep_mid ? s->x[s->cur] : nullptr;
  if (keep_mid && m.overlap) HIP_TRY(xmid_array(s, &A.x_mid));
  HIP_TRY(m.before_write(A.x_out, A.x_mid));
  if (s->timing) HIP_TRY(hipEventRecord(s->ev[2 * s->last_launches], m.st));
  HIP_TRY(lmc::launch_step_block(A, m.st));
  if (s->timing) HIP_TRY(hipEventRecord(s->ev[2 * s->last_launches + 1], m.st));
  s->kernel_name = four ? "myula_step_block_kernel(4 iterations)" : "myula_step_block_kernel(2 iterations)";
  int rc = m.keep(A.x_mid, keep_out ? A.x_out : nullptr, m.overlap);
  if (rc) return rc;
  s->cur ^= 1;
  s->iteration += nf;
  ++s->last_launches;
  return nf;
}

static int myula_single(lmc_sampler* s, SideMoments& m, const float* noise, bool last) {
  hipStream_t st = m.st;
  lmc::StepArgs A = s->base;
  A.x_in = s->x[s->cur];
  A.x_out = s->x[s->cur ^ 1];
  A.iteration = (uint32_t)s->iteration;
  A.noise = noise;
  sanitize_pointers(A);
  int rc = me_tv_extra(s, A, st);
  if (rc) return rc;
  HIP_TRY(m.before_write(A.x_out));
  if (s->timing) HIP_TRY(hipEventRecord(s->ev[2 * s->last_launches], st));
  const char* kname = nullptr;
  hipError_t e;
  bool stepped = false;
  if (s->rt_tv.kc && A.prior_kind == LMC_PRIOR_TV_ISO) {
    rc = tv_prior_rt(s->prob, s->epsg * s->gamma, A, s->rt_tv, s->pxbuf, s->tvstate[0], s->tvstate[1], st);
    if (rc < 0) return rc;
    if (rc == 2) return fail(LMC_E_STATE, "the device-side early exit no longer covers this sampler");
    if (rc == 1) { stepped = true; kname = "myula_step_pipe_kernel(per-chain exit)"; }
  }
  if (s->rtmp && A.prior_kind == LMC_PRIOR_TV_ISO) {
    rc = tv_prox_rtol(s->prob, s->epsg * s->gamma, A.x_in, s->pxbuf, s->rtmp, s->robj, s->rflag, s->C, s->tvstate[0], s->tvstate[1], st);
    if (rc) return rc;
    A.prior_kind = LMC_PRIOR_NONE;
    A.prox_ext = s->pxbuf;
  }
  if (s->prob.prox_scale && A.prior_kind != LMC_PRIOR_NONE) {
    const Problem& q = s->prob;
    HIP_TRY(lmc::launch_prior_prox_scaled(q.prior_kind, q.eprox_kind, A.x_in, s->pxbuf, s->C, (int64_t)q.H * q.W, q.prox_scale, q.prox_scale_cs, q.prox_scale_ps,
                                          s->epsg * s->gamma, q.prior_sigma, q.eprox_p0, q.eprox_p1, q.eprox_mask, st));
    A.prior_kind = LMC_PRIOR_NONE;
    A.prox_ext = s->pxbuf;
  }
  if (stepped) {
    e = hipSuccess;
  } else if (s->tvwarm[0]) {
    A.tv_in = s->tvwarm[s->wcur];
    A.tv_out = s->tvwarm[s->wcur ^ 1];
    e = lmc::launch_step_pipe_warm(A, st);
    kname = "myula_step_pipe_kernel(warm)";
    s->wcur ^= 1;
  } else {
    e = launch_step(A, variant_of(s->prob), st, &kname, s->tvstate[0], s->tvstate[1], s->pxbuf);
  }
  if (e == hipErrorInvalidConfiguration) return fail(LMC_E_UNSUPPORTED, "no step-kernel variant covers this configuration");
  HIP_TRY(e);
  if (kname) s->kernel_name = kname;
  if (s->timing) HIP_TRY(hipEventRecord(s->ev[2 * s->last_launches + 1], st));
  s->cur ^= 1;
  if (kept(s, s->iteration)) {
    const bool beside = m.overlap && !last &&
                        (s->pol_overlap > 0 || s->base.prior_kind == LMC_PRIOR_TV_ISO || (long long)s->C * s->prob.H * s->prob.W <= (1LL << 25));
    rc = m.keep(s->x[s->cur], nullptr, beside);
    if (rc) return rc;
  }
  ++s->iteration;
  ++s->last_launches;
  return 1;
}

static int myula_step(lmc_sampler* s, int32_t n_iters, const float* noise_dev, hipStream_t st) {
  const size_t per_iter = (size_t)s->C * s->prob.H * s->prob.W;
  s->timed = false;
  s->last_launches = 0;
  if (n_iters == 0) return LMC_OK;
  if (s->timing) {
    while ((int)s->ev.size() < 2 * n_iters) {
      hipEvent_t e;
      HIP_TRY(hipEventCreate(&e));
      s->ev.push_back(e);
    }
  }
  const bool overlap = !s->timing && s->pol_overlap >= 0 && s->moments && n_iters > 1;
  const int bg_wgs = s->pol_bg_wgs >= 0 ? s->pol_bg_wgs : ((long long)per_iter <= (1LL << 25) ? 128 : 256);
  if (overlap && !s->side) {
    int prio_least = 0, prio_greatest = 0;
    HIP_TRY(hipDeviceGetStreamPriorityRange(&prio_least, &prio_greatest));
    HIP_TRY(hipStreamCreateWithPriority(&s->side, hipStreamNonBlocking, prio_least));
    for (hipEvent_t& e : s->side_ev) HIP_TRY(hipEventCreateWithFlags(&e, hipEventDisableTiming));
  }
  SideMoments m{s, st, overlap, bg_wgs};
  for (int k = 0; k < n_iters;) {
    int done = 0;
    if (!noise_dev) done = myula_rows_pair(s, m, n_iters - k);
    if (!noise_dev && !done) done = myula_block_pair(s, m, n_iters - k);
    if (!done) done = myula_single(s, m, noise_dev ? noise_dev + (size_t)k * per_iter : nullptr, k + 1 == n_iters);
    if (done < 0) {
      (void)m.join();
      return done;
    }
    k += done;
  }
  HIP_TRY(m.join());
  s->timed = s->timing;
  return LMC_OK;
}

int lmc_sampler_step(lmc_sampler* s, int32_t n_iters, const float* noise_dev, void* stream) {
  if (!s) return fail(LMC_E_INVALID, "NULL sampler");
  DeviceGuard dg(s->device);
  if (n_iters < 0) return fail(LMC_E_INVALID, "n_iters < 0");
  if (s->noise_mode == LMC_NOISE_INJECTED && !noise_dev && n_iters > 0)
    return fail(LMC_E_INVALID, "noise_mode is INJECTED but noise_dev is NULL");
  if (s->noise_mode != LMC_NOISE_INJECTED && noise_dev)
    return fail(LMC_E_INVALID, "noise_dev given but noise_mode is not INJECTED");
  if (s->iteration + n_iters > 0xFFFFFFFFLL) return fail(LMC_E_STATE, "iteration counter would exceed 32 bits");
  if (s->kind == 2) return mymala_step(s, n_iters, noise_dev, S(stream));
  if (s->kind == 1) return ulpda_step(s, n_iters, noise_dev, S(stream));
  return myula_step(s, n_iters, noise_dev, S(stream));
}

int lmc_mymala_create(const lmc_myula_config* cfg, lmc_sampler** out) {
  int rc = lmc_myula_create(cfg, out);
  if (rc) return rc;
  lmc_sampler* s = *out;
  *out = nullptr;
  if (s->tvwarm[0]) { lmc_sampler_destroy(s); return fail(LMC_E_UNSUPPORTED, "MYMALA needs a proposal mean that is a function of x alone: tv_warm is not allowed"); }
  if (s->rtmp || s->rt_tv.kc) { lmc_sampler_destroy(s); return fail(LMC_E_UNSUPPORTED, "MYMALA with tv_rtol > 0 is not built (use the fixed-count prox, tv_rtol = 0)"); }
  if (s->prob.prox_scale) { lmc_sampler_destroy(s); return fail(LMC_E_UNSUPPORTED, "MYMALA takes a scalar epsg (the reference's array-valued epsg is MYULA's, algs.py:509)"); }
  s->kind = 2;
  const size_t nbytes = sizeof(float) * (size_t)s->C * s->prob.H * s->prob.W;
  hipError_t e = hipMalloc(&s->mx, nbytes);
  if (e == hipSuccess) e = hipMalloc(&s->xp, nbytes);
  if (e == hipSuccess) e = hipMalloc(&s->mxp, nbytes);
  if (e == hipSuccess) e = hipMalloc(&s->mala_d, sizeof(double) * 6 * (size_t)s->C);
  if (e == hipSuccess) e = hipMalloc(&s->flag, sizeof(int) * (size_t)s->C);
  if (e == hipSuccess) e = hipMalloc(&s->nacc, sizeof(unsigned long long) * (size_t)s->C);
  if (e == hipSuccess) e = hipMemset(s->nacc, 0, sizeof(unsigned long long) * (size_t)s->C);
  if (e == hipSuccess) e = hipMemset(s->mala_d, 0, sizeof(double) * 6 * (size_t)s->C);
  if (e != hipSuccess) return alloc_failed(s, e);
  *out = s;
  return LMC_OK;
}

static int mymala_step(lmc_sampler* s, int32_t n_iters, const float* noise_dev, hipStream_t st) {
  const size_t img = (size_t)s->prob.H * s->prob.W, per_iter = (size_t)s->C * img;
  const int C = s->C;
  double *U = s->mala_d, *fp = U + C, *gp = U + 2 * C, *d1 = U + 3 * C, *d2 = U + 4 * C, *la = U + 5 * C;
  float* x = s->x[s->cur];
  s->timed = false;
  s->last_launches = 0;
  const char* kname = nullptr;
  if (!s->mala_fresh && n_iters > 0) {
    bool fused = false;
    int rc = sampler_update(s, x, s->mx, false, nullptr, (uint32_t)s->iteration, st, &kname, fp, gp, &fused);
    if (rc) return rc;
    if (!fused) rc = sampler_energies_at(s, x, fp, gp, st);
    if (rc) return rc;
    HIP_TRY(hipMemsetAsync(d1, 0, sizeof(double) * C, st));
    HIP_TRY(lmc::launch_axpy_env(fp, gp, d1, C, -s->epsg, 1.f, st));
    HIP_TRY(hipMemcpyAsync(U, fp, sizeof(double) * C, hipMemcpyDeviceToDevice, st));
    s->mala_fresh = true;
  }
  for (int k = 0; k < n_iters; ++k) {
    const float* xi = noise_dev ? noise_dev + (size_t)k * per_iter : s->xi;
    if (s->noise_mode == LMC_NOISE_PHILOX) {
      HIP_TRY(lmc::mala_propose_philox(s->mx, s->xp, C, s->prob.H, s->prob.W, s->base.s, s->base.key0, s->base.key1, (uint32_t)s->iteration,
                                       s->base.chain_offset, d1, st));
    } else if (s->noise_mode == LMC_NOISE_NONE) {
      HIP_TRY(hipMemcpyAsync(s->xp, s->mx, sizeof(float) * per_iter, hipMemcpyDeviceToDevice, st));
      HIP_TRY(hipMemsetAsync(d1, 0, sizeof(double) * C, st));
    } else {
      HIP_TRY(lmc::mala_propose(s->mx, xi, s->xp, C, img, s->base.s, d1, st));
    }
    bool fused = false;
    int rc = sampler_update(s, s->xp, s->mxp, false, nullptr, (uint32_t)s->iteration, st, &kname, fp, gp, &fused);
    if (rc) return rc;
    if (!fused) rc = sampler_energies_at(s, s->xp, fp, gp, st);
    if (rc) return rc;
    HIP_TRY(lmc::launch_sqdiff(x, s->mxp, C, img, d2, st));
    HIP_TRY(lmc::mala_accept(C, U, fp, gp, s->epsg, d1, d2, s->tau, s->base.key0, s->base.key1, (uint32_t)s->iteration, s->base.chain_offset,
                             s->flag, s->nacc, la, st));
    HIP_TRY(lmc::mala_select(s->flag, x, s->mx, s->xp, s->mxp, C, img, 1, st));
    if (kept(s, s->iteration)) {
      HIP_TRY(lmc::launch_moments(x, C, s->prob.H, s->prob.W, s->s1, s->s2, st));
      s->count += (uint64_t)C;
    }
    ++s->iteration;
  }
  if (kname) s->kernel_name = kname;
  return LMC_OK;
}

int lmc_sampler_get_acceptance(lmc_sampler* s, uint64_t* accepted_dev, double* last_log_alpha_dev, void* stream) {
  if (!s) return fail(LMC_E_INVALID, "NULL sampler");
  DeviceGuard dg(s->device);
  if (s->kind != 2) return fail(LMC_E_STATE, "not a MYMALA sampler");
  if (accepted_dev) HIP_TRY(hipMemcpyAsync(accepted_dev, s->nacc, sizeof(uint64_t) * (size_t)s->C, hipMemcpyDeviceToDevice, S(stream)));
  if (last_log_alpha_dev)
    HIP_TRY(hipMemcpyAsync(last_log_alpha_dev, s->mala_d + 5 * (size_t)s->C, sizeof(double) * (size_t)s->C, hipMemcpyDeviceToDevice, S(stream)));
  return LMC_OK;
}

int lmc_sampler_enable_timing(lmc_sampler* s, int32_t on) {
  if (!s) return fail(LMC_E_INVALID, "NULL sampler");
  s->timing = on != 0;
  s->timed = false;
  return LMC_OK;
}


static int ulpda_step(lmc_sampler* s, int32_t n_iters, const float* noise_dev, hipStream_t st) {
  const int H = s->prob.H, W = s->prob.W;
  const int64_t C = s->C;
  const size_t per_iter = (size_t)C * H * W;
  const int iso = s->prob.prior_kind == LMC_PRIOR_TV_ISO;
  s->timed = false;
  s->last_launches = 0;
  bool used_pairs = false;
  for (int k = 0; k < n_iters; ++k) {
    float* x = s->x[s->cur];
    const float ts = s->tau * s->prob.sigma_f;
    const float* htb_nc = s->prob.data_kind == LMC_DATA_BLUR ? s->htb : s->prob.y;
    const float ts_nc = s->prob.data_kind == LMC_DATA_BLUR ? ts : 0.f;
    if (s->gfirst)
      HIP_TRY(lmc::ulpda_dual_update(s->xhat, s->ydual, C, H, W, s->mu, s->prob.prior_sigma, iso, st));
    if (s->prob.ncvx_kind == LMC_NCVX_MC_TV) {
      HIP_TRY(lmc::ulpda_rhs(x, s->ydual, s->z, nullptr, s->ctmp, C, H, W, s->tau, ts, st));
      HIP_TRY(lmc::ulpda_ncvx_rhs(s->ctmp, htb_nc, s->rhs, C, H, W, s->tau * s->prob.ncvx_lambda, s->prob.ncvx_gamma, ts_nc, st));
    } else if (s->prob.ncvx_kind == LMC_NCVX_ME_TV) {
      HIP_TRY(lmc::ulpda_rhs(x, s->ydual, s->z, nullptr, s->ctmp, C, H, W, s->tau, ts, st));
      int rc = me_tv_prox(s->prob, s->ctmp, s->extra, C, s->tvstate[0], s->tvstate[1], st, &s->rt_me);
      if (rc) return rc;
      HIP_TRY(lmc::ulpda_me_rhs(s->ctmp, s->extra, htb_nc, s->rhs, C, H, W, s->tau * s->prob.ncvx_lambda / s->prob.ncvx_gamma, ts_nc, st));
    } else {
      HIP_TRY(lmc::ulpda_rhs(x, s->ydual, s->z, s->prob.data_kind == LMC_DATA_BLUR ? s->htb : nullptr, s->rhs, C, H, W, s->tau, ts, st));
    }
    const float* u = s->rhs;
    if (s->prob.data_kind == LMC_DATA_BLUR) {
      if (!s->warm) HIP_TRY(hipMemsetAsync(s->uw, 0, sizeof(float) * per_iter, st));
      float* where = s->uw;
      { int rc = cg_solve_fused(s->prob, ts, s->uw, s->rhs, s->cr, s->cp, s->cq, s->scal, C, s->cg_niter, s->zero_y, st, s->uw2, &where); if (rc) return rc; }
      if (where != s->uw) { s->uw2 = s->uw; s->uw = where; used_pairs = true; }
      u = s->uw;
    } else if (s->prob.data_kind != LMC_DATA_NONE) {
      HIP_TRY(lmc::ulpda_pointwise_prox(s->rhs, s->uw, s->prob.y, s->prob.mask, C, H, W, ts, s->prob.data_kind, st));
      u = s->uw;
    }
    if (s->noise_mode == LMC_NOISE_PHILOX && (W & 3) == 0) {
      HIP_TRY(lmc::ulpda_finish_philox(x, s->xhat, u, C, H, W, std::sqrt(2.f * s->tau), s->theta, s->base.key0, s->base.key1,
                                       (uint32_t)s->iteration, s->base.chain_offset, st));
    } else {
      const float* xi = nullptr;
      if (s->noise_mode == LMC_NOISE_INJECTED) xi = noise_dev + (size_t)k * per_iter;
      else if (s->noise_mode == LMC_NOISE_PHILOX) {
        HIP_TRY(lmc::launch_noise(s->xi, (int)C, H, W, s->base.key0, s->base.key1, (uint32_t)s->iteration, s->base.chain_offset, st));
        xi = s->xi;
      }
      HIP_TRY(lmc::ulpda_finish(x, s->xhat, u, xi, C, H, W, std::sqrt(2.f * s->tau), s->theta, st));
    }
    if (!s->gfirst)
      HIP_TRY(lmc::ulpda_dual_update(s->xhat, s->ydual, C, H, W, s->mu, s->prob.prior_sigma, iso, st));
    if (kept(s, s->iteration)) {
      HIP_TRY(lmc::launch_moments(x, s->C, H, W, s->s1, s->s2, st));
      s->count += (uint64_t)s->C;
    }
    ++s->iteration;
  }
  s->kernel_name = used_pairs ? "ulpda (multi-kernel, chebyshev pairs)" : "ulpda (multi-kernel)";
  return LMC_OK;
}

int lmc_ulpda_create(const lmc_ulpda_config* cfg, lmc_sampler** out) {
  if (!cfg || !out) return fail(LMC_E_INVALID, "NULL argument");
  *out = nullptr;
  if (cfg->struct_size != sizeof(lmc_ulpda_config))
    return fail(LMC_E_INVALID, "lmc_ulpda_config.struct_size %u != %zu (ABI mismatch)", cfg->struct_size, sizeof(lmc_ulpda_config));
  int rc = check_config(*cfg, cfg->tau > 0.f && cfg->mu > 0.f, "tau and mu must be > 0");
  if (rc) return rc;
  if (cfg->problem.prior_kind != LMC_PRIOR_TV_ISO && cfg->problem.prior_kind != LMC_PRIOR_TV_ANISO)
    return fail(LMC_E_UNSUPPORTED, "ULPDA needs g o A with g = L21 (LMC_PRIOR_TV_ISO) or L1 (LMC_PRIOR_TV_ANISO)");
  if (!(cfg->problem.prior_sigma > 0.f)) return fail(LMC_E_INVALID, "prior_sigma (dual ball radius) must be > 0");
  if (cfg->problem.data_kind == LMC_DATA_BLUR && cfg->cg_niter < 1) return fail(LMC_E_INVALID, "cg_niter must be >= 1");
  if (cfg->problem.ncvx_kind != LMC_NCVX_NONE && cfg->problem.data_kind == LMC_DATA_NONE)
    return fail(LMC_E_UNSUPPORTED, "the non-convex term belongs to a data term (blur, identity or mask)");
  lmc_sampler* s = new (std::nothrow) lmc_sampler();
  if (!s) return fail(LMC_E_NOMEM, "host allocation failed");
  lmc_problem pr = cfg->problem;
  if (pr.prior_kind == LMC_PRIOR_TV_ISO && pr.tv_niter < 1) pr.tv_niter = 1;
  rc = load_problem(&pr, s->prob);
  if (rc) { delete s; return rc; }
  if (hipGetDevice(&s->device) != hipSuccess) { delete s; return fail(LMC_E_HIP, "hipGetDevice failed"); }
  s->kind = 1;
  s->C = cfg->n_chains;
  s->chain_offset = cfg->chain_offset;
  s->tau = cfg->tau; s->mu = cfg->mu; s->theta = cfg->theta;
  s->gfirst = cfg->gfirst != 0; s->cg_niter = cfg->cg_niter; s->warm = cfg->warm != 0;
  s->z = cfg->z_dev;
  s->seed = cfg->seed;
  s->noise_mode = cfg->noise_mode;
  s->moments = cfg->moments; s->burn_in = cfg->burn_in; s->thin = cfg->thin < 1 ? 1 : cfg->thin;
  s->base.key0 = (uint32_t)(s->seed & 0xFFFFFFFFu);
  s->base.key1 = (uint32_t)(s->seed >> 32);
  s->base.chain_offset = (uint32_t)s->chain_offset;
  const size_t n = (size_t)s->C * s->prob.H * s->prob.W, img = (size_t)s->prob.H * s->prob.W;
  hipError_t e = hipSuccess;
  auto alloc = [&](float** p, size_t count) { if (e == hipSuccess) e = hipMalloc(p, sizeof(float) * count); if (e == hipSuccess) e = hipMemset(*p, 0, sizeof(float) * count); };
  alloc(&s->x[0], n); alloc(&s->xhat, n); alloc(&s->ydual, 2 * n); alloc(&s->uw, n); alloc(&s->rhs, n);
  if (s->noise_mode == LMC_NOISE_PHILOX) alloc(&s->xi, n);
  if (s->prob.data_kind == LMC_DATA_BLUR) {
    alloc(&s->cr, n); alloc(&s->cp, n); alloc(&s->cq, n); alloc(&s->ctmp, n); alloc(&s->htb, img); alloc(&s->zero_y, img);
    if (lmc::cheb_pair_supported(s->prob.H, s->prob.W, s->prob.taps)) alloc(&s->uw2, n);
    if (e == hipSuccess) e = hipMalloc(&s->scal, sizeof(double) * (4 * (size_t)s->C + 1));
    if (e == hipSuccess) e = lmc::launch_blur(s->prob.y, s->htb, 1, s->prob.H, s->prob.W, s->prob.taps, 1, nullptr);
    if (e == hipSuccess) e = hipDeviceSynchronize();
  }
  if (s->prob.ncvx_kind != LMC_NCVX_NONE && !s->ctmp) alloc(&s->ctmp, n);
  if (s->prob.ncvx_kind == LMC_NCVX_ME_TV) {
    alloc(&s->extra, n);
    if (needs_tv_state(s->prob)) { alloc(&s->tvstate[0], 4 * n); alloc(&s->tvstate[1], 4 * n); }
    if (e == hipSuccess && s->prob.ncvx_rtol > 0.f) e = s->rt_me.need((size_t)s->C, s->prob.ncvx_niter);
  }
  if (e == hipSuccess) e = alloc_moments(s);
  if (e != hipSuccess) return alloc_failed(s, e);
  s->kernel_name = "(no step launched yet)";
  *out = s;
  return LMC_OK;
}

int lmc_sampler_set_dual(lmc_sampler* s, const float* y_dev, void* stream) {
  if (!s || !y_dev) return fail(LMC_E_INVALID, "NULL argument");
  DeviceGuard dg(s->device);
  if (s->kind != 1) return fail(LMC_E_STATE, "not a ULPDA sampler");
  HIP_TRY(hipMemcpyAsync(s->ydual, y_dev, sizeof(float) * 2 * (size_t)s->C * s->prob.H * s->prob.W, hipMemcpyDeviceToDevice, S(stream)));
  return LMC_OK;
}

int lmc_sampler_get_dual(lmc_sampler* s, float* y_dev, void* stream) {
  if (!s || !y_dev) return fail(LMC_E_INVALID, "NULL argument");
  DeviceGuard dg(s->device);
  if (s->kind != 1) return fail(LMC_E_STATE, "not a ULPDA sampler");
  HIP_TRY(hipMemcpyAsync(y_dev, s->ydual, sizeof(float) * 2 * (size_t)s->C * s->prob.H * s->prob.W, hipMemcpyDeviceToDevice, S(stream)));
  return LMC_OK;
}

int lmc_sampler_set_steps(lmc_sampler* s, float tau, float mu) {
  if (!s) return fail(LMC_E_INVALID, "NULL sampler");
  if (s->kind != 1) return fail(LMC_E_STATE, "not a ULPDA sampler");
  if (!(tau > 0.f) || !(mu > 0.f)) return fail(LMC_E_INVALID, "tau and mu must be > 0");
  s->tau = tau; s->mu = mu;
  return LMC_OK;
}

int64_t lmc_sampler_iteration(const lmc_sampler* s) { return s ? s->iteration : -1; }

int lmc_sampler_set_iteration(lmc_sampler* s, int64_t it) {
  if (!s || it < 0 || it > 0xFFFFFFFFLL) return fail(LMC_E_INVALID, "bad iteration");
  s->iteration = it;
  return LMC_OK;
}

int lmc_sampler_get_moments(lmc_sampler* s, double* sum_dev, double* sumsq_dev, uint64_t* count, void* stream) {
  if (!s) return fail(LMC_E_INVALID, "NULL sampler");
  DeviceGuard dg(s->device);
  if (!s->moments) return fail(LMC_E_STATE, "sampler was created with moments = 0");
  const size_t mb = sizeof(double) * (size_t)s->prob.H * s->prob.W;
  if (sum_dev) HIP_TRY(hipMemcpyAsync(sum_dev, s->s1, mb, hipMemcpyDeviceToDevice, S(stream)));
  if (sumsq_dev) HIP_TRY(hipMemcpyAsync(sumsq_dev, s->s2, mb, hipMemcpyDeviceToDevice, S(stream)));
  HIP_TRY(hipStreamSynchronize(S(stream)));
  if (count) *count = s->count;
  return LMC_OK;
}

int lmc_sampler_reset_moments(lmc_sampler* s, void* stream) {
  if (!s) return fail(LMC_E_INVALID, "NULL sampler");
  DeviceGuard dg(s->device);
  if (!s->moments) return fail(LMC_E_STATE, "sampler was created with moments = 0");
  const size_t mb = sizeof(double) * (size_t)s->prob.H * s->prob.W;
  HIP_TRY(hipMemsetAsync(s->s1, 0, mb, S(stream)));
  HIP_TRY(hipMemsetAsync(s->s2, 0, mb, S(stream)));
  s->count = 0;
  return LMC_OK;
}

int lmc_sampler_energies(lmc_sampler* s, double* f_out_dev, double* g_out_dev, void* stream) {
  if (!s) return fail(LMC_E_INVALID, "NULL sampler");
  DeviceGuard dg(s->device);
  return sampler_energies_at(s, s->x[s->cur], f_out_dev, g_out_dev, S(stream));
}

int lmc_sampler_noise(lmc_sampler* s, int64_t iteration, float* out_dev, void* stream) {
  if (!s || !out_dev) return fail(LMC_E_INVALID, "NULL argument");
  DeviceGuard dg(s->device);
  if (iteration < 0 || iteration > 0xFFFFFFFFLL) return fail(LMC_E_INVALID, "bad iteration");
  HIP_TRY(lmc::launch_noise(out_dev, s->C, s->prob.H, s->prob.W, s->base.key0, s->base.key1, (uint32_t)iteration,
                            s->base.chain_offset, S(stream)));
  return LMC_OK;
}

int lmc_sampler_last_step_timing(lmc_sampler* s, float* total_ms, int32_t* n_launches) {
  if (!s) return fail(LMC_E_INVALID, "NULL sampler");
  DeviceGuard dg(s->device);
  if (!s->timed || s->last_launches < 1)
    return fail(LMC_E_STATE, "no timed lmc_sampler_step call to report (lmc_sampler_enable_timing first)");
  HIP_TRY(hipEventSynchronize(s->ev[2 * s->last_launches - 1]));
  float ms = 0.f;
  for (int k = 0; k < s->last_launches; ++k) {
    float d = 0.f;
    HIP_TRY(hipEventElapsedTime(&d, s->ev[2 * k], s->ev[2 * k + 1]));
    ms += d;
  }
  if (total_ms) *total_ms = ms;
  if (n_launches) *n_launches = s->last_launches;
  return LMC_OK;
}

const char* lmc_sampler_kernel_name(const lmc_sampler* s) { return s ? s->kernel_name.c_str() : ""; }

int lmc_sampler_tv_exit_stats(lmc_sampler* s, int32_t which, int32_t* passes_dev, uint64_t* reruns_host, void* stream) {
  if (!s || (which != 0 && which != 1)) return fail(LMC_E_INVALID, "bad arguments");
  DeviceGuard dg(s->device);
  RtState& rt = which == 0 ? s->rt_tv : s->rt_me;
  if (!rt.kc) return fail(LMC_E_STATE, "this sampler does not run the device-side early exit for that prox (tv_rtol / ncvx_rtol = 0, or the pass-by-pass path)");
  hipStream_t st = S(stream);
  if (passes_dev) HIP_TRY(hipMemcpyAsync(passes_dev, rt.pred, sizeof(int) * (size_t)s->C, hipMemcpyDeviceToDevice, st));
  unsigned long long r[4] = {0, 0, 0, 0};
  if (reruns_host) HIP_TRY(hipMemcpyAsync(r, rt.reruns, sizeof r, hipMemcpyDeviceToHost, st));
  HIP_TRY(hipStreamSynchronize(st));
  if (reruns_host) for (int i = 0; i < 4; ++i) reruns_host[i] = r[i];
  return LMC_OK;
}

}
```

lmc_atomi_amd/csrc/lmc_step_pipe.hip:

```cpp
#include "lmc_step_pipe_kernel.h"

namespace lmc {

int centred_blur_taps(const StepArgs& a, float* uc, float* vc);

bool pipe_geometry_ok(const StepArgs& a) {
  if (a.prior_kind != LMC_PRIOR_TV_ISO || a.prox_ext) return false;
  if (a.W <= 128 || a.H < 1 || a.W > 16384) return false;
  if (a.W > 512 && (a.f_out || a.g_out)) return false;
  if ((a.W & (a.W > 256 ? 7 : 3)) && !(a.tv.niter == 10 || (a.tv.niter >= 20 && a.tv.niter % 10 == 0))) return false;
  if (a.data_kind == LMC_DATA_BLUR) {
    float uc[kMaxBlur], vc[kMaxBlur];
    if (centred_blur_taps(a, uc, vc) == 0) return false;
  } else if (a.data_kind != LMC_DATA_NONE && a.data_kind != LMC_DATA_IDENTITY && a.data_kind != LMC_DATA_MASK) {
    return false;
  }
  if (a.data_kind != LMC_DATA_BLUR && (a.ncvx_kind != LMC_NCVX_NONE || a.f_out)) return false;
  return true;
}

int pipe_links(const StepArgs& a) {
  if (a.prior_kind != LMC_PRIOR_TV_ISO || a.tv.niter > kMaxTvIters) return 0;
  const int n = a.tv.niter;
  const bool single = n == 2 || n == 6 || n == 8 || n == 9 || n == 10;
  if (!single && (n < 19 || (n % 10 != 0 && n % 10 != 9))) return 0;
  if (a.tv_in || a.tv_out || a.tv_state_only || a.tv_warm) return 0;
  if (!pipe_geometry_ok(a)) return 0;
  return single ? 1 : (n + 9) / 10;
}

bool pipe_supported(const StepArgs& a) { return pipe_links(a) == 1; }

bool pipe_warm_supported(const StepArgs& a) {
  const int n = a.tv.niter;
  if (!(n == 1 || n == 2 || n == 3)) return false;
  return pipe_geometry_ok(a);
}

int pipe_taps(StepArgs& a) {
  int KT = 0;
  if (a.data_kind == LMC_DATA_BLUR) {
    float uc[kMaxBlur] = {0}, vc[kMaxBlur] = {0};
    KT = centred_blur_taps(a, uc, vc);
    for (int i = 0; i < kMaxBlur; ++i) { a.blur.h[i] = i < KT ? uc[i] : 0.f; a.blur.h[kMaxBlur + i] = i < KT ? vc[i] : 0.f; }
  }
  return KT;
}

hipError_t launch_step_pipe_warm(StepArgs a, hipStream_t st) {
  if (!pipe_warm_supported(a) || !a.tv_in || !a.tv_out || a.tv_in == a.tv_out) return hipErrorInvalidConfiguration;
  a.tv_warm = 1;
  a.tv_state_only = 0;
  const int KT = pipe_taps(a);
  return pipe_dispatch_chain(a, a.tv.niter, KT, st);
}

bool pipe_teams_covered(const StepArgs& a, int KT) {
  return a.tv.niter == 10 && KT == 5 && a.W >= 264 && a.W <= 512 && (a.W & 7) == 0 && !a.f_out && !a.g_out &&
         a.ncvx_kind == LMC_NCVX_NONE && !a.extra;
}

hipError_t launch_step_pipe(StepArgs a, hipStream_t st, float* state0, float* state1, int teams) {
  const int links = pipe_links(a);
  if (links == 0 || (links > 1 && (!state0 || !state1))) return hipErrorInvalidConfiguration;
  const int KT = pipe_taps(a);
  const bool two = links == 1 && pipe_teams_covered(a, KT);
  if (teams == 2 && !two) return hipErrorInvalidConfiguration;
  if (two && teams != 1) return pipe_launch_teams<10, 5>(a, st);
  if (links == 1) {
    switch (a.tv.niter) {
      case 2: return pipe_dispatch_k<2, false>(a, KT, st);
      case 6: return pipe_dispatch_k<6, false>(a, KT, st);
      case 8: return pipe_dispatch_k<8, false>(a, KT, st);
      case 9: return pipe_dispatch_k<9, false>(a, KT, st);
      default: return pipe_dispatch_k<10, false>(a, KT, st);
    }
  }
  float* st_buf[2] = {state0, state1};
  for (int j = 0; j < links; ++j) {
    StepArgs b = a;
    const int kl = (j == links - 1) ? a.tv.niter - 10 * j : 10;
    b.tv.niter = kl;
    for (int i = 0; i < kl; ++i) b.tv.betas[i] = a.tv.betas[10 * j + i];
    b.tv_in = j > 0 ? st_buf[(j - 1) & 1] : nullptr;
    b.tv_out = j < links - 1 ? st_buf[j & 1] : nullptr;
    b.tv_state_only = j < links - 1;
    hipError_t e = pipe_dispatch_chain(b, kl, b.tv_state_only ? 0 : KT, st);
    if (e != hipSuccess) return e;
  }
  return hipSuccess;
}

}
```

lmc_atomi_amd/csrc/lmc_step_pipe_kernel.h:

```cpp
#pragma once
#include "lmc_device.h"
#include "lmc_launch.h"

namespace lmc {

#ifndef LMC_RT_SPREAD
#define LMC_RT_SPREAD 1
#endif
#ifndef LMC_RT_CHAIN_MAP
#define LMC_RT_CHAIN_MAP 1
#endif
#ifndef LMC_RT_MAP_SPREAD
#define LMC_RT_MAP_SPREAD 3
#endif
#ifndef LMC_WARM_MIN_WAVES
#define LMC_WARM_MIN_WAVES 1
#endif
#ifdef LMC_EXP_NOBARRIER
#define PIPE_TICK_SYNC() asm volatile("" ::: "memory")
#elif defined(LMC_EXP_SLEEP_MASK)
#define PIPE_TICK_SYNC() do { __syncthreads(); if ((LMC_EXP_SLEEP_MASK >> wave) & 1) __builtin_amdgcn_s_sleep(LMC_EXP_SLEEP_N); } while (0)
#else
#define PIPE_TICK_SYNC() __syncthreads()
#endif

template <int K>
struct PipeGeom {
  static constexpr int D = (2 * K + 2 > 10) ? 2 * K + 2 : 10;
  static constexpr int E = D - (2 * K + 2);
  static constexpr int RB = D + 1;
  static constexpr int NT = (K + 1) / 2;
};

template <int K, int PXL, bool CHAIN = false, int TEAMS = 1>
struct PipeLds {
  static constexpr int BW = 64 * PXL;
  static constexpr int RP = TEAMS * BW;
  static constexpr int o_x = 0;
  static constexpr int o_hand = o_x + PipeGeom<K>::RB * RP;
  static constexpr int o_hand_last = o_hand + (PipeGeom<K>::NT - 1) * 8 * RP;
  static constexpr int o_hand0 = o_hand_last + 4 * RP;
  static constexpr int o_g = CHAIN ? o_hand0 + 8 * RP : o_hand + PipeGeom<K>::NT * 2 * 4 * RP;
  static constexpr int SLAB = 2 * 4 * PXL * 64;
  static constexpr int o_slab = o_g + 2 * RP;
  static constexpr int o_seam = o_slab + TEAMS * SLAB;
  static constexpr int total = o_seam + (TEAMS == 2 ? 64 : 0);
};

template <int PXL>
__device__ __forceinline__ void prow_load(float (&v)[PXL], const float* row, int lane) {
#pragma unroll
  for (int g = 0; g < PXL / 4; ++g) {
    const float4 q = *reinterpret_cast<const float4*>(row + g * 256 + lane * 4);
    v[4 * g] = q.x; v[4 * g + 1] = q.y; v[4 * g + 2] = q.z; v[4 * g + 3] = q.w;
  }
}
template <int PXL>
__device__ __forceinline__ void prow_store(float* row, int lane, const float (&v)[PXL]) {
#pragma unroll
  for (int g = 0; g < PXL / 4; ++g)
    *reinterpret_cast<float4*>(row + g * 256 + lane * 4) = make_float4(v[4 * g], v[4 * g + 1], v[4 * g + 2], v[4 * g + 3]);
}

typedef float v2f __attribute__((ext_vector_type(2)));
__device__ __forceinline__ v2f pk_fma(v2f a, v2f b, v2f c) { return __builtin_elementwise_fma(a, b, c); }
__device__ __forceinline__ v2f pk_set(float a) { return v2f{a, a}; }

template <int NP>
__device__ __forceinline__ void pairs_load(v2f (&v)[NP], const float* row, int lane) {
#pragma unroll
  for (int g = 0; g < NP / 2; ++g) {
    const float4 q = *reinterpret_cast<const float4*>(row + g * 256 + lane * 4);
    v[2 * g] = v2f{q.x, q.y};
    v[2 * g + 1] = v2f{q.z, q.w};
  }
}
template <int NP>
__device__ __forceinline__ void pairs_store(float* row, int lane, const v2f (&v)[NP]) {
#pragma unroll
  for (int g = 0; g < NP / 2; ++g)
    *reinterpret_cast<float4*>(row + g * 256 + lane * 4) = make_float4(v[2 * g].x, v[2 * g].y, v[2 * g + 1].x, v[2 * g + 1].y);
}

template <int NP>
struct DualRow { v2f rr[NP], ss[NP], p[NP], q[NP]; };

__device__ __forceinline__ float wave_from_left(float v, float edge) {
  return __builtin_bit_cast(float, __builtin_amdgcn_update_dpp(__builtin_bit_cast(int, edge), __builtin_bit_cast(int, v), 0x138, 0xf, 0xf, false));
}
__device__ __forceinline__ float wave_from_right(float v, float edge) {
  return __builtin_bit_cast(float, __builtin_amdgcn_update_dpp(__builtin_bit_cast(int, edge), __builtin_bit_cast(int, v), 0x130, 0xf, 0xf, false));
}

template <int NP>
struct PipeCr { float cstep, cr_last; v2f ncrv[NP]; };
template <int NP, bool LASTLANE>
__device__ __forceinline__ v2f pipe_ncr(const PipeCr<NP>& c, int i) {
  if constexpr (LASTLANE) return i == NP - 1 ? v2f{-c.cstep, -c.cr_last} : pk_set(-c.cstep);
  else return c.ncrv[i];
}

struct StageObj { v2f sq, tv; };
template <int NP, bool PERPIX = false>
struct ObjMask {
  float md; v2f mlast;
  v2f mx[PERPIX ? NP : 1], my[PERPIX ? NP : 1];
};
template <int NP, bool LASTLANE>
__device__ __forceinline__ v2f obj_sq(const ObjMask<NP, !LASTLANE>* om, int i, v2f T) {
  if constexpr (LASTLANE) return T;
  else return T * om->mx[i];
}
template <int NP, bool LASTLANE>
__device__ __forceinline__ v2f obj_tv(const ObjMask<NP, !LASTLANE>* om, int i, v2f dxv, v2f dyv) {
  v2f dxm, dym;
  if constexpr (LASTLANE) { dxm = dxv * pk_set(om->md); dym = i == NP - 1 ? dyv * om->mlast : dyv; }
  else { dxm = dxv * pk_set(om->md) * om->mx[i]; dym = dyv * om->my[i]; }
  const v2f n = pk_fma(dxm, dxm, dym * dym);
  return v2f{__builtin_amdgcn_sqrtf(n.x), __builtin_amdgcn_sqrtf(n.y)};
}

template <int NP, bool LASTLANE = true, bool OBJ = false, bool SEAML = false, bool SEAMR = false>
__device__ __forceinline__ void pipe_stage(const v2f (&xa)[NP], const v2f (&r1)[NP], const v2f (&s1)[NP], const DualRow<NP>& in0,
                                           v2f (&solb)[NP], float gam, float cdown, const PipeCr<NP>& cr, float beta,
                                           DualRow<NP>& out, StageObj* ob = nullptr, const ObjMask<NP, !LASTLANE>* om = nullptr,
                                           float ssl_edge = 0.f, float solr_edge = 0.f) {
  v2f sol[NP];
  const float ssl0 = SEAML ? wave_from_left(s1[NP - 1].y, ssl_edge) : dpp_left0(s1[NP - 1].y);
  const v2f ngam = pk_set(-gam), ncd = pk_set(-cdown), vb = pk_set(beta);
#pragma unroll
  for (int i = 0; i < NP; ++i) {
    const v2f ssl = v2f{i == 0 ? ssl0 : s1[i - 1].y, s1[i].x};
    const v2f T = (r1[i] - in0.rr[i]) + (s1[i] - ssl);
    sol[i] = pk_fma(ngam, T, xa[i]);
    if constexpr (OBJ) { const v2f Tm = obj_sq<NP, LASTLANE>(om, i, T); ob->sq = i == 0 ? Tm * Tm : pk_fma(Tm, Tm, ob->sq); }
  }
  const float solr_last = SEAMR ? wave_from_right(solb[0].x, solr_edge) : dpp_right0(solb[0].x);
#pragma unroll
  for (int i = 0; i < NP; ++i) {
    const v2f solr = v2f{solb[i].y, i == NP - 1 ? solr_last : solb[i + 1].x};
    const v2f ncr = pipe_ncr<NP, LASTLANE>(cr, i);
    const v2f dxv = sol[i] - solb[i], dyv = solr - solb[i];
    if constexpr (OBJ) {
      const v2f nr = obj_tv<NP, LASTLANE>(om, i, dxv, dyv);
      ob->tv = i == 0 ? nr : ob->tv + nr;
    }
    const v2f r = pk_fma(ncd, dxv, in0.rr[i]);
    const v2f s = pk_fma(ncr, dyv, in0.ss[i]);
    const v2f n2 = pk_fma(r, r, s * s);
    const v2f inv = v2f{__builtin_amdgcn_fmed3f(__builtin_amdgcn_rsqf(n2.x), 0.f, 1.f), __builtin_amdgcn_fmed3f(__builtin_amdgcn_rsqf(n2.y), 0.f, 1.f)};
    const v2f pn = r * inv, qn = s * inv;
    out.rr[i] = pk_fma(vb, pn - in0.p[i], pn);
    out.ss[i] = pk_fma(vb, qn - in0.q[i], qn);
    out.p[i] = pn;
    out.q[i] = qn;
  }
#pragma unroll
  for (int i = 0; i < NP; ++i) solb[i] = sol[i];
}

template <int NP, bool LASTLANE = true, bool OBJ = false, bool SEAMR = false>
__device__ __forceinline__ void pipe_stage_first(const v2f (&xa)[NP], v2f (&solb)[NP], float cdown, const PipeCr<NP>& cr, float beta,
                                                 DualRow<NP>& out, StageObj* ob = nullptr, const ObjMask<NP, !LASTLANE>* om = nullptr,
                                                 float solr_edge = 0.f) {
  const float solr_last = SEAMR ? wave_from_right(solb[0].x, solr_edge) : dpp_right0(solb[0].x);
  const v2f ncd = pk_set(-cdown), vb = pk_set(beta);
  if constexpr (OBJ) ob->sq = pk_set(0.f);
#pragma unroll
  for (int i = 0; i < NP; ++i) {
    const v2f solr = v2f{solb[i].y, i == NP - 1 ? solr_last : solb[i + 1].x};
    const v2f ncr = pipe_ncr<NP, LASTLANE>(cr, i);
    const v2f dxv = xa[i] - solb[i], dyv = solr - solb[i];
    if constexpr (OBJ) {
      const v2f nr = obj_tv<NP, LASTLANE>(om, i, dxv, dyv);
      ob->tv = i == 0 ? nr : ob->tv + nr;
    }
    const v2f r = ncd * dxv;
    const v2f s = ncr * dyv;
    const v2f n2 = pk_fma(r, r, s * s);
    const v2f inv = v2f{__builtin_amdgcn_fmed3f(__builtin_amdgcn_rsqf(n2.x), 0.f, 1.f), __builtin_amdgcn_fmed3f(__builtin_amdgcn_rsqf(n2.y), 0.f, 1.f)};
    const v2f pn = r * inv, qn = s * inv;
    out.rr[i] = pk_fma(vb, pn, pn);
    out.ss[i] = pk_fma(vb, qn, qn);
    out.p[i] = pn;
    out.q[i] = qn;
  }
#pragma unroll
  for (int i = 0; i < NP; ++i) solb[i] = xa[i];
}

template <int PXL>
__device__ __forceinline__ void gload_row(float (&dst)[PXL], const float* __restrict__ row, int c0, int W, bool ok, bool al = true) {
  if (al) {
#pragma unroll
    for (int g = 0; g < PXL / 4; ++g) {
      const bool okg = ok && c0 + 4 * g < W;
      const float4 v = *reinterpret_cast<const float4*>(row + (okg ? c0 + 4 * g : 0));
      dst[4 * g] = okg ? v.x : 0.f; dst[4 * g + 1] = okg ? v.y : 0.f; dst[4 * g + 2] = okg ? v.z : 0.f; dst[4 * g + 3] = okg ? v.w : 0.f;
    }
  } else {
#pragma unroll
    for (int g = 0; g < PXL / 4; ++g) {
      float v[4];
      load4_dword_aligned(v[0], v[1], v[2], v[3], row, c0 + 4 * g, W);
#pragma unroll
      for (int q = 0; q < 4; ++q) dst[4 * g + q] = (ok && c0 + 4 * g + q < W) ? v[q] : 0.f;
    }
  }
}

template <int PXL>
__device__ __forceinline__ void gload_raw(float (&dst)[PXL], const float* __restrict__ row, int c0, int W, bool al = true) {
  if (al) {
#pragma unroll
    for (int g = 0; g < PXL / 4; ++g) {
      const float4 v = *reinterpret_cast<const float4*>(row + (c0 + 4 * g < W ? c0 + 4 * g : 0));
      dst[4 * g] = v.x; dst[4 * g + 1] = v.y; dst[4 * g + 2] = v.z; dst[4 * g + 3] = v.w;
    }
  } else {
#pragma unroll
    for (int g = 0; g < PXL / 4; ++g) load4_dword_aligned_raw(dst[4 * g], dst[4 * g + 1], dst[4 * g + 2], dst[4 * g + 3], row, c0 + 4 * g, W);
  }
}
template <int PXL, bool AL>
__device__ __forceinline__ void gfix_raw(float (&r)[PXL], int c0, int W) {
  if constexpr (!AL) unshift_row_dword_aligned<PXL>(r, c0, W);
}

__device__ __forceinline__ void gstore4(float* __restrict__ row, int c, int lo, int hi, bool al, float v0, float v1, float v2, float v3) {
  if (al) {
    if (c >= lo && c < hi) *reinterpret_cast<float4*>(row + c) = make_float4(v0, v1, v2, v3);
  } else store4_dword_aligned(row, c, lo, hi, v0, v1, v2, v3);
}

__host__ __device__ constexpr int pipe_halo(int K, int KT, int PXL) {
  const int need = (K + 1 > KT - 1 ? K + 1 : KT - 1);
  return (need + PXL - 1) / PXL * PXL;
}

#ifndef LMC_PIPE2_ROLES
#define LMC_PIPE2_ROLES 0x5D3BC4A291E6F780ull
#endif
template <int K, int PXL, int KT, bool CHAIN, bool WARM, bool AL, bool RT, int TEAMS>
__device__ __forceinline__ void pipe_body(const StepArgs& A) {
  static_assert(!WARM || CHAIN, "the warm dual uses the state hand-over of the chained launches");
  static_assert(!RT || (!WARM && (K & 1) == 0), "per-chain exit: cold start, even K");
  static_assert(!RT || AL || pipe_halo(K, KT, PXL) >= K + 2, "per-chain exit on column strips: the halo holds the objective's extra column");
  static_assert(TEAMS == 1 || (TEAMS == 2 && K == 10 && PXL == 4 && KT == 5 && AL && !CHAIN && !WARM && !RT),
                "two teams: one fixed-count launch, 5 taps, aligned rows, 4 pixels per lane");
  using G = PipeGeom<K>;
  using L = PipeLds<K, PXL, CHAIN, TEAMS>;
  constexpr int D = G::D, E = G::E, RB = G::RB, NT = G::NT, BW = L::BW, RP = L::RP, HW = KT > 0 ? (KT - 1) / 2 : 0;
  constexpr int LAGT = TEAMS == 2 ? 1 : 0;
  static_assert(K >= 1, "at least one dual iteration");
  static_assert(D >= KT + 1 + LAGT, "the blur pipeline reads ring rows at least one tick old");
  extern __shared__ float lds_all[];
  const int lane = threadIdx.x & 63;
  const int hw_wave = __builtin_amdgcn_readfirstlane(threadIdx.x >> 6);
  int team = 0;
  const int chain = blockIdx.x;
  const int H = A.H, W = A.W;
  int kc = K;
  bool state_only = CHAIN && A.tv_state_only;
  if constexpr (RT) {
    const int kc_g = __builtin_amdgcn_readfirstlane(A.rt_kc[chain]);
    if (kc_g <= A.rt_base) return;
    if (CHAIN && A.rt_start && A.rt_base < K * (__builtin_amdgcn_readfirstlane(A.rt_start[chain]) & 0xFFFF)) return;
    kc = min(kc_g - A.rt_base, K);
    state_only = CHAIN && kc_g > A.rt_base + K;
  }
  int wave = hw_wave;
  if constexpr (TEAMS == 2) {
    const unsigned nib = (unsigned)(LMC_PIPE2_ROLES >> (4 * hw_wave)) & 15u;
    team = nib >> 3;
    wave = nib & 7;
  } else if constexpr (K == 10 && !RT && !CHAIN) {
    const unsigned code = A.ncvx_kind == LMC_NCVX_MC_TV ? 0x76354210u : (KT == 7 ? 0x75264310u : 0x76325410u);
    wave = (code >> (4 * hw_wave)) & 15;
  }
  if constexpr (K == 10 && !RT && CHAIN) wave = (0x67325410u >> (4 * hw_wave)) & 15;
  if constexpr (RT && K == 10) {
#ifndef LMC_RT_MAP
#define LMC_RT_MAP 0
#endif
    if (LMC_RT_SPREAD && LMC_RT_MAP_SPREAD >= 3 && kc <= NT) {
      const unsigned code = kc >= 5 ? 0x76543210u : kc == 4 ? 0x67514320u
                                                              : 0x64753210u;
      wave = (code >> (4 * hw_wave)) & 15;
    } else if (kc <= 4) {
      if (LMC_RT_MAP == 0) wave = hw_wave == 3 ? 6 : hw_wave == 4 ? 7 : hw_wave == 5 ? 4 : hw_wave == 6 ? 3 : hw_wave == 7 ? 5 : hw_wave;
      else if (LMC_RT_MAP == 1) wave = hw_wave == 4 ? 6 : hw_wave == 6 ? 4 : hw_wave;
      else wave = hw_wave == 3 ? 6 : hw_wave == 4 ? 5 : hw_wave == 5 ? 4 : hw_wave == 6 ? 3 : hw_wave;
    }
    else if (CHAIN && LMC_RT_CHAIN_MAP) wave = ((LMC_RT_CHAIN_MAP == 2 ? 0x76345210u : 0x67254310u) >> (4 * hw_wave)) & 15;
    else wave = hw_wave == 4 ? 6 : hw_wave == 6 ? 4 : hw_wave;
  }
#ifdef LMC_EXP_PERM
  if (TEAMS == 1 && A.PH && (LMC_EXP_PERM == 1 || CHAIN)) wave = (A.PH >> (4 * hw_wave)) & 15;
#endif
  constexpr int HALO = pipe_halo(K, KT, PXL);
  const int strip = blockIdx.y;
  const int strip_u = gridDim.y > 1 ? BW - 2 * HALO : W;
  int c0 = (strip ? strip * strip_u - HALO : 0) + lane * PXL;
  int st_lo = strip * strip_u, st_hi = min(W, st_lo + strip_u);
  if constexpr (TEAMS == 2) {
    const int Wt = W >> 1;
    c0 = team ? Wt + lane * PXL : Wt - BW + lane * PXL;
    st_lo = team ? Wt : 0;
    st_hi = team ? W : Wt;
  }
  const bool cok = c0 >= st_lo && c0 < st_hi;
  const int cl = TEAMS == 2 ? (cok ? c0 : 0) : c0;
  auto col_in = [&](int k) __attribute__((always_inline)) -> bool { return TEAMS == 2 ? cok : c0 + k < W; };
  constexpr bool al = AL;
  const size_t img = (size_t)H * W;
  const float* __restrict__ xin = A.x_in + (size_t)chain * img;
  float* __restrict__ xout = A.x_out + (size_t)chain * img;

  for (int e = threadIdx.x; e < (TEAMS == 2 ? L::total : L::o_slab); e += blockDim.x) lds_all[e] = 0.f;
  __syncthreads();
  float* const lds = lds_all + team * BW;
  float* const slab_base = lds_all + L::o_slab + team * L::SLAB;
  float* const seam = lds_all + L::o_seam;
  constexpr int SA = 0, SB = 4 * (NT + 1), SR = SB + 4 * NT;
  static_assert(TEAMS == 1 || SR + 8 <= L::total - L::o_seam, "seam records");

  const int T_end = (H + D + 3) & ~3;
  float* const xring = lds + L::o_x;
  auto ring_row = [&](int row) -> float* { return xring + ((unsigned)(row + RB) % (unsigned)RB) * RP; };

#ifdef LMC_EXP_SKIP
  if ((LMC_EXP_SKIP >> wave) & 1) return;
#endif
#ifndef LMC_PRIO_L
#define LMC_PRIO_L 3
#define LMC_PRIO_C 3
#define LMC_PRIO_T 1
#define LMC_PRIO_N 0
#endif
  if (wave == 0) __builtin_amdgcn_s_setprio(LMC_PRIO_L);
  else if (wave == NT + 1) __builtin_amdgcn_s_setprio(LMC_PRIO_C);
  else if (wave <= NT) __builtin_amdgcn_s_setprio(LMC_PRIO_T);
  else __builtin_amdgcn_s_setprio(LMC_PRIO_N);
  auto roles = [&](auto team_tag) __attribute__((always_inline)) {
  constexpr int TM = decltype(team_tag)::value;
  if (wave == 0) {
    const float* __restrict__ uv = A.blur.h;
    constexpr bool kRing4 = (KT == 5);
    constexpr int NWIN = KT > 1 ? KT - 1 : 1;
    constexpr int kXPF = 4;
    float xpre[kXPF][PXL], hxw[NWIN][PXL], hrw[NWIN][PXL], ypre[4][PXL];
    constexpr int kYPF = (KT == 7 || TEAMS == 2) ? 2 : 3;
#pragma unroll
    for (int a = 0; a < NWIN; ++a)
#pragma unroll
      for (int k = 0; k < PXL; ++k) { hxw[a][k] = 0.f; hrw[a][k] = 0.f; }
#pragma unroll
    for (int u = 0; u < kXPF; ++u) gload_raw<PXL>(xpre[u], xin + (size_t)min(u, H - 1) * W, cl, W, al);
    if constexpr (KT > 0) {
#pragma unroll
      for (int u = 0; u < kYPF; ++u) {
        const int r = u + 1 - D + (KT - 1) - HW + LAGT;
        gload_raw<PXL>(ypre[u], A.y + (size_t)min(max(r, 0), H - 1) * W, cl, W, al);
      }
    }
    const bool pw_id = KT == 0 && A.data_kind == LMC_DATA_IDENTITY, pw_mask = KT == 0 && A.data_kind == LMC_DATA_MASK;
    float mpre[KT == 0 ? 4 : 1][KT == 0 ? PXL : 1];
    if constexpr (KT == 0) {
#pragma unroll
      for (int u = 0; u < 4; ++u)
#pragma unroll
        for (int k = 0; k < PXL; ++k) { ypre[u][k] = 0.f; mpre[u][k] = 0.f; }
      if (pw_id || pw_mask) {
#pragma unroll
        for (int u = 0; u < kYPF; ++u) {
          const size_t ro = (size_t)min(max(u + 1 - D, 0), H - 1) * W;
          gload_raw<PXL>(ypre[u], A.y + ro, c0, W, al);
          if (pw_mask) gload_raw<PXL>(mpre[u], A.mask + ro, c0, W, al);
        }
      }
    }
    constexpr int nsf = CHAIN ? (WARM ? 2 : 4) : 0;
    constexpr int kSPF = 2;
    float spre[CHAIN ? kSPF : 1][CHAIN ? nsf : 1][CHAIN ? PXL : 1];
    const float* const sin = CHAIN && A.tv_in ? A.tv_in + (size_t)chain * nsf * img : nullptr;
    if constexpr (CHAIN) {
#pragma unroll
      for (int u = 0; u < kSPF; ++u) {
        const int rs = u - E - 1;
#pragma unroll
        for (int f = 0; f < nsf; ++f)
          gload_raw<PXL>(spre[u][f], sin ? sin + (size_t)f * img + (size_t)min(max(rs, 0), H - 1) * W : xin, c0, W, al);
      }
    }
    double facc = 0.0;
    float Rprev[TEAMS == 2 ? PXL : 1];
#pragma unroll
    for (int k = 0; k < (TEAMS == 2 ? PXL : 1); ++k) Rprev[k] = 0.f;
    auto tick = [&](auto uu, const int t) __attribute__((always_inline)) {
      constexpr int U = decltype(uu)::value, P = U & 1;
      if constexpr (KT > 0) {
        const int r3 = t + kYPF + 1 - D + (KT - 1) - HW + LAGT;
        gload_raw<PXL>(ypre[(U + kYPF) & 3], A.y + (size_t)min(max(r3, 0), H - 1) * W, cl, W, al);
      } else if (pw_id || pw_mask) {
        const size_t ro = (size_t)min(max(t + kYPF + 1 - D, 0), H - 1) * W;
        gload_raw<PXL>(ypre[(U + kYPF) & 3], A.y + ro, c0, W, al);
        if (pw_mask) gload_raw<PXL>(mpre[(U + kYPF) & 3], A.mask + ro, c0, W, al);
      }
      {
        float xv[PXL];
        gfix_raw<PXL, AL>(xpre[U], c0, W);
#pragma unroll
        for (int k = 0; k < PXL; ++k) xv[k] = (t < H && col_in(k)) ? xpre[U][k] : 0.f;
        prow_store<PXL>(ring_row(t), lane, xv);
        gload_raw<PXL>(xpre[U], xin + (size_t)min(t + kXPF, H - 1) * W, cl, W, al);
      }
      if constexpr (CHAIN) {
        float* hb = lds + L::o_hand0 + P * 4 * RP;
        constexpr int SP = U & (kSPF - 1);
        const int rh = t - E - 1;
        const bool rowok_h = sin && rh >= 0 && rh < H;
#pragma unroll
        for (int f = 0; f < nsf; ++f) {
          gfix_raw<PXL, AL>(spre[SP][f], c0, W);
          float sv[PXL];
#pragma unroll
          for (int k = 0; k < PXL; ++k) sv[k] = (rowok_h && c0 + (AL ? (k & ~3) : k) < W) ? spre[SP][f][k] : 0.f;
          prow_store<PXL>(hb + f * RP, lane, sv);
        }
        const int rs = t + kSPF - E - 1;
#pragma unroll
        for (int f = 0; f < nsf; ++f)
          gload_raw<PXL>(spre[SP][f], sin ? sin + (size_t)f * img + (size_t)min(max(rs, 0), H - 1) * W : xin, c0, W, al);
      }
      if constexpr (KT > 0) {
      const int i = t + 1 - D + (KT - 1) + LAGT;
      float hxn[PXL];
      {
        float xi[PXL], e[PXL + 2 * HW];
        const float* const xr = ring_row(i);
        prow_load<PXL>(xi, xr, lane);
#pragma unroll
        for (int m = 0; m < HW; ++m) e[m] = (TEAMS == 2 && TM == 1) ? wave_from_left(xi[PXL - HW + m], xr[m - HW]) : dpp_left0(xi[PXL - HW + m]);
#pragma unroll
        for (int k = 0; k < PXL; ++k) e[HW + k] = xi[k];
#pragma unroll
        for (int m = 0; m < HW; ++m) e[HW + PXL + m] = (TEAMS == 2 && TM == 0) ? wave_from_right(xi[m], xr[BW + m]) : dpp_right0(xi[m]);
#pragma unroll
        for (int k = 0; k < PXL; ++k) {
          float acc = uv[kMaxBlur] * e[k + 2 * HW];
#pragma unroll
          for (int b = 1; b < KT; ++b) acc = fmaf(uv[kMaxBlur + b], e[k + 2 * HW - b], acc);
          hxn[k] = acc;
        }
      }
      const int r = i - HW;
      float R[PXL];
      {
        const bool rowok = r >= 0 && r < H;
        const float rmask = rowok ? 1.f : 0.f;
        gfix_raw<PXL, AL>(ypre[U & 3], c0, W);
#pragma unroll
        for (int k = 0; k < PXL; ++k) {
          float acc = uv[0] * hxn[k];
#pragma unroll
          for (int a = 1; a < KT; ++a) acc = fmaf(uv[a], hxw[kRing4 ? ((U - a) & 3) : a - 1][k], acc);
          R[k] = (acc - ypre[U & 3][k]) * ((TEAMS == 2 ? cok : AL ? c0 < W : c0 + k < W) ? rmask : 0.f);
        }
        if (TEAMS == 1 && A.f_out) {
#pragma unroll
          for (int k = 0; k < PXL; ++k) facc = fma((double)R[k], (double)R[k], facc);
        }
        if constexpr (!kRing4) {
#pragma unroll
          for (int a = KT - 2; a >= 1; --a)
#pragma unroll
            for (int k = 0; k < PXL; ++k) hxw[a][k] = hxw[a - 1][k];
        }
#pragma unroll
        for (int k = 0; k < PXL; ++k) hxw[kRing4 ? (U & 3) : 0][k] = hxn[k];
      }
      if constexpr (TEAMS == 2) {
        if (TM == 0 ? lane == 63 : lane == 0) {
#pragma unroll
          for (int m = 0; m < HW; ++m) seam[SR + P * 4 + 2 * TM + m] = R[TM == 0 ? PXL - HW + m : m];
        }
#pragma unroll
        for (int k = 0; k < PXL; ++k) { const float tmp = R[k]; R[k] = Rprev[k]; Rprev[k] = tmp; }
      }
      {
        float e[PXL + 2 * HW], gout[PXL];
        const float* const sr = seam + SR + (P ^ 1) * 4;
#pragma unroll
        for (int m = 0; m < HW; ++m) e[m] = (TEAMS == 2 && TM == 1) ? wave_from_left(R[PXL - HW + m], sr[m]) : dpp_left0(R[PXL - HW + m]);
#pragma unroll
        for (int k = 0; k < PXL; ++k) e[HW + k] = R[k];
#pragma unroll
        for (int m = 0; m < HW; ++m) e[HW + PXL + m] = (TEAMS == 2 && TM == 0) ? wave_from_right(R[m], sr[2 + m]) : dpp_right0(R[m]);
#pragma unroll
        for (int k = 0; k < PXL; ++k) {
          float hrn = uv[kMaxBlur] * e[k];
#pragma unroll
          for (int b = 1; b < KT; ++b) hrn = fmaf(uv[kMaxBlur + b], e[k + b], hrn);
          float acc = uv[KT - 1] * hrn;
#pragma unroll
          for (int a = 0; a < KT - 1; ++a) acc = fmaf(uv[a], hrw[kRing4 ? ((U - (KT - 1 - a)) & 3) : KT - 2 - a][k], acc);
          if constexpr (!kRing4) {
#pragma unroll
            for (int a = KT - 2; a >= 1; --a) hrw[a][k] = hrw[a - 1][k];
          }
          hrw[kRing4 ? (U & 3) : 0][k] = hrn;
          gout[k] = A.sigma_f * acc;
        }
        prow_store<PXL>(lds + L::o_g + P * RP, lane, gout);
      }
      }
      if constexpr (KT == 0) {
        if (pw_id || pw_mask) {
          const int i = t + 1 - D;
          float xi[PXL], gout[PXL];
          prow_load<PXL>(xi, ring_row(i), lane);
          const bool rowok = i >= 0 && i < H;
          gfix_raw<PXL, AL>(ypre[U & 3], c0, W);
          if (pw_mask) gfix_raw<PXL, AL>(mpre[U & 3], c0, W);
#pragma unroll
          for (int k = 0; k < PXL; ++k) {
            float g = 0.f;
            if (rowok && c0 + k < W) {
              if (pw_id) g = A.sigma_f * (xi[k] - ypre[U & 3][k]);
              else g = A.sigma_f * mpre[U & 3][k] * fmaf(mpre[U & 3][k], xi[k], -ypre[U & 3][k]);
            }
            gout[k] = g;
          }
          prow_store<PXL>(lds + L::o_g + P * RP, lane, gout);
        }
      }
      PIPE_TICK_SYNC();
    };
    for (int t = 0; t < T_end; t += 4) static_for<0, 4>([&](auto uu) { tick(uu, t + decltype(uu)::value); });
    if (TEAMS == 1 && A.f_out) {
      const double tot = wave_sum(facc);
      if (lane == 0) unsafeAtomicAdd(&A.f_out[chain], 0.5 * (double)A.sigma_f * tot);
    }
  } else if (wave <= NT) {
    auto t_role = [&](auto first_tag, auto single_tag) __attribute__((always_inline)) {
    constexpr bool FIRST = decltype(first_tag)::value;
    constexpr bool SINGLE = decltype(single_tag)::value;
    const int k1 = 2 * wave - 1, k2 = 2 * wave;
    const bool spread = RT && LMC_RT_SPREAD && kc <= NT;
    const int g1 = spread ? wave : k1, g2 = k2;
    const float gam = A.tv.gamma, cstep = A.tv.c;
    const float beta1 = A.tv.betas[g1 - 1], beta2 = SINGLE ? 0.f : A.tv.betas[g2 - 1];
    PipeCr<PXL / 2> crc;
    crc.cstep = cstep;
    crc.cr_last = (c0 + PXL - 1 == W - 1 || (TEAMS == 2 && !cok)) ? 0.f : cstep;
#pragma unroll
    for (int i = 0; i < PXL / 2; ++i) crc.ncrv[i] = v2f{c0 + 2 * i == W - 1 ? 0.f : -cstep, c0 + 2 * i + 1 == W - 1 ? 0.f : -cstep};
    float* const hout = lds + L::o_hand + (wave - 1) * 8 * RP;
    const bool from_state = CHAIN && wave == 1 && A.tv_in != nullptr;
    constexpr bool warm = WARM;
    const float* const hin = from_state ? lds + L::o_hand0 : hout - 8 * RP;
    constexpr int nof = warm ? 2 : 4;
    float* const sout = CHAIN && wave == NT && A.tv_out && (!RT || state_only) ? A.tv_out + (size_t)chain * nof * img : nullptr;
    constexpr int NP = PXL / 2;
    const bool live1 = !RT || g1 <= kc, live2 = !RT || (!spread && g2 <= kc);
    const bool fullpass2 = spread && wave < kc;
    ObjMask<NP, !AL> om;
    om.md = 0.f;
    om.mlast = v2f{1.f, (c0 + PXL - 1 == W - 1) ? 0.f : 1.f};
    if constexpr (RT && !AL) {
#pragma unroll
      for (int i = 0; i < NP; ++i) {
        const int ca = c0 + 2 * i, cb = ca + 1;
        const bool ina = ca >= st_lo && ca < st_hi, inb_ = cb >= st_lo && cb < st_hi;
        om.mx[i] = v2f{ina ? 1.f : 0.f, inb_ ? 1.f : 0.f};
        om.my[i] = v2f{ina && ca < W - 1 ? 1.f : 0.f, inb_ && cb < W - 1 ? 1.f : 0.f};
      }
    }
    double osq1 = 0.0, otv1 = 0.0, osq2 = 0.0, otv2 = 0.0;
    DualRow<NP> inb[2], o1[2];
    v2f sol1[NP], sol2[NP];
    v2f xk[2][NP];
#pragma unroll
    for (int k = 0; k < NP; ++k) {
      sol1[k] = sol2[k] = pk_set(0.f);
      xk[0][k] = xk[1][k] = pk_set(0.f);
#pragma unroll
      for (int pp = 0; pp < 2; ++pp) {
        inb[pp].rr[k] = inb[pp].ss[k] = inb[pp].p[k] = inb[pp].q[k] = pk_set(0.f);
        o1[pp].rr[k] = o1[pp].ss[k] = o1[pp].p[k] = o1[pp].q[k] = pk_set(0.f);
      }
    }
    auto emit = [&](const DualRow<NP>& out, const int P, const int brow, const bool live) __attribute__((always_inline)) {
      if (RT && !live) {
        float* hb = hout + P * ((!CHAIN || wave < NT) ? 4 : 2) * RP;
        pairs_store<NP>(hb, lane, out.rr);
        pairs_store<NP>(hb + RP, lane, out.ss);
      } else if (!CHAIN || wave < NT) {
        float* hb = hout + P * 4 * RP;
#ifdef LMC_EXP_NO_HSTORE
        if (A.tv.niter == 12345)
#endif
        {
        pairs_store<NP>(hb, lane, out.rr);
        pairs_store<NP>(hb + RP, lane, out.ss);
#ifdef LMC_EXP_HALF_HSTORE
        if (A.tv.niter == 12345)
#endif
        if (wave < NT) {
        pairs_store<NP>(hb + 2 * RP, lane, out.p);
        pairs_store<NP>(hb + 3 * RP, lane, out.q);
        }
        }
      } else {
        float* hb = hout + P * 2 * RP;
        pairs_store<NP>(hb, lane, out.rr);
        pairs_store<NP>(hb + RP, lane, out.ss);
        if (sout && brow >= 0 && brow < H) {
#pragma unroll
          for (int g = 0; g < NP / 2; ++g) {
            float* d = sout + (size_t)brow * W;
            const int cg = c0 + 4 * g;
            if (warm) {
              gstore4(d, cg, st_lo, st_hi, al, out.p[2 * g].x, out.p[2 * g].y, out.p[2 * g + 1].x, out.p[2 * g + 1].y);
              gstore4(d + img, cg, st_lo, st_hi, al, out.q[2 * g].x, out.q[2 * g].y, out.q[2 * g + 1].x, out.q[2 * g + 1].y);
            } else {
              gstore4(d, cg, st_lo, st_hi, al, out.rr[2 * g].x, out.rr[2 * g].y, out.rr[2 * g + 1].x, out.rr[2 * g + 1].y);
              gstore4(d + img, cg, st_lo, st_hi, al, out.ss[2 * g].x, out.ss[2 * g].y, out.ss[2 * g + 1].x, out.ss[2 * g + 1].y);
              gstore4(d + 2 * img, cg, st_lo, st_hi, al, out.p[2 * g].x, out.p[2 * g].y, out.p[2 * g + 1].x, out.p[2 * g + 1].y);
              gstore4(d + 3 * img, cg, st_lo, st_hi, al, out.q[2 * g].x, out.q[2 * g].y, out.q[2 * g + 1].x, out.q[2 * g + 1].y);
            }
          }
        }
      }
    };
    constexpr bool SL = TEAMS == 2 && TM == 1, SRt = TEAMS == 2 && TM == 0;
    const float* const seam_in = seam + (TM == 1 ? SA + 2 * wave - 2 : SB + 2 * (wave - 1));
    float* const seam_out = seam + (TM == 0 ? SA + 2 * wave - 1 : SB + 2 * (wave - 1));
    auto tick = [&](auto uu, const int t) __attribute__((always_inline)) {
      constexpr int P = decltype(uu)::value & 1;
      const int a2 = t - E - 2 * k2, a1 = t - E - 2 * k1;
      float2 edge = make_float2(0.f, 0.f);
      if constexpr (TEAMS == 2) edge = *reinterpret_cast<const float2*>(seam_in + (P ^ 1) * (TM == 1 ? 2 * (NT + 1) : 2 * NT));
      float ss2_edge = 0.f;
      if constexpr (!SINGLE) {
        const float cdown = ((unsigned)(a2 - 1) >= (unsigned)(H - 1)) ? 0.f : cstep;
        DualRow<NP> out;
        if (live2) {
          StageObj ob;
          om.md = cdown != 0.f ? 1.f : 0.f;
          pipe_stage<NP, AL, RT, SL, SRt>(xk[P], o1[P ^ 1].rr, o1[P ^ 1].ss, o1[P], sol2, gam, cdown, crc, beta2, out, &ob, &om, edge.y, edge.y);
          if constexpr (RT) { osq2 += (double)(ob.sq.x + ob.sq.y); otv2 += (double)(ob.tv.x + ob.tv.y); }
        } else {
#pragma unroll
          for (int k = 0; k < NP; ++k) { out.rr[k] = o1[P].rr[k]; out.ss[k] = o1[P].ss[k]; }
          if (fullpass2) {
#pragma unroll
            for (int k = 0; k < NP; ++k) { out.p[k] = o1[P].p[k]; out.q[k] = o1[P].q[k]; }
          }
        }
        emit(out, P, a2 - 1, live2 || fullpass2);
        ss2_edge = out.ss[NP - 1].y;
      }
      {
        if constexpr (!FIRST) {
          if (k1 > 1 || from_state) {
            const float* hb = hin + (P ^ 1) * 4 * RP;
            pairs_load<NP>(inb[P].rr, hb, lane);
            pairs_load<NP>(inb[P].ss, hb + RP, lane);
            if (from_state && warm) {
#pragma unroll
              for (int k = 0; k < NP; ++k) { inb[P].p[k] = inb[P].rr[k]; inb[P].q[k] = inb[P].ss[k]; }
            } else if (live1) {
              pairs_load<NP>(inb[P].p, hb + 2 * RP, lane);
              pairs_load<NP>(inb[P].q, hb + 3 * RP, lane);
            }
          }
        }
        if (live1) {
          pairs_load<NP>(xk[P], ring_row(a1), lane);
          const float cdown = ((unsigned)(a1 - 1) >= (unsigned)(H - 1)) ? 0.f : cstep;
          StageObj ob;
          om.md = cdown != 0.f ? 1.f : 0.f;
          if constexpr (FIRST) pipe_stage_first<NP, AL, RT, SRt>(xk[P], sol1, cdown, crc, beta1, o1[P], &ob, &om, edge.x);
          else pipe_stage<NP, AL, RT, SL, SRt>(xk[P], inb[P].rr, inb[P].ss, inb[P ^ 1], sol1, gam, cdown, crc, beta1, o1[P], &ob, &om, edge.x, edge.x);
          if constexpr (RT) { osq1 += (double)(ob.sq.x + ob.sq.y); otv1 += (double)(ob.tv.x + ob.tv.y); }
        } else {
#pragma unroll
          for (int k = 0; k < NP; ++k) { o1[P].rr[k] = inb[P ^ 1].rr[k]; o1[P].ss[k] = inb[P ^ 1].ss[k]; }
        }
        if constexpr (SINGLE) emit(o1[P], P, a1 - 1, live1);
      }
      if constexpr (TEAMS == 2) {
        float* const so = seam_out + P * (TM == 0 ? 2 * (NT + 1) : 2 * NT);
        if (TM == 0 ? lane == 63 : lane == 0) {
          so[0] = TM == 0 ? o1[P].ss[NP - 1].y : sol1[0].x;
          so[1] = TM == 0 ? ss2_edge : sol2[0].x;
        }
      }
      PIPE_TICK_SYNC();
    };
    for (int t = 0; t < T_end; t += 4) static_for<0, 4>([&](auto uu) { tick(uu, t + decltype(uu)::value); });
    if constexpr (RT) {
      const double dg = (double)gam;
      double* const ob = A.rt_obj + (size_t)chain * A.rt_stride + A.rt_base;
      if (live1) {
        const double tot = wave_sum(0.5 * dg * dg * osq1 + dg * otv1);
        if (lane == 0) unsafeAtomicAdd(ob + (g1 - 1), tot);
      }
      if (!SINGLE && live2) {
        const double tot = wave_sum(0.5 * dg * dg * osq2 + dg * otv2);
        if (lane == 0) unsafeAtomicAdd(ob + (g2 - 1), tot);
      }
    }
    };
    constexpr bool kOdd = (K & 1) != 0;
    bool ran = false;
    if constexpr (!CHAIN) {
      if (wave == 1) {
        if constexpr (K == 1) t_role(std::true_type{}, std::true_type{});
        else t_role(std::true_type{}, std::false_type{});
        ran = true;
      }
    }
    if constexpr (kOdd) {
      if (!ran && wave == NT) { t_role(std::false_type{}, std::true_type{}); ran = true; }
    }
    if constexpr (K > 1) {
      if (!ran) t_role(std::false_type{}, std::false_type{});
    }
  } else if (wave == NT + 2) {
    float* const slab = slab_base + lane;
    const uint32_t iter = A.iteration;
    auto tick = [&](auto uu, const int t) __attribute__((always_inline)) {
      constexpr int U = decltype(uu)::value;
      constexpr int NI = ((U - D) % 4 + 4) % 4;
      const int o = t - D;
      if (A.noise_mode == LMC_NOISE_PHILOX && !state_only) {
        const int qn = ((o - NI) >> 2) + 1;
        if (qn >= 0 && 4 * qn < H) {
          float* const sl = slab + (qn & 1) * (4 * PXL * 64);
#pragma unroll
          for (int kk = 0; kk < PXL / 4; ++kk) {
            const int k = NI * (PXL / 4) + kk;
            float n4[4];
            quad_normals(A.key0, A.key1, iter, A.chain_offset + (uint32_t)chain, (uint32_t)qn * (uint32_t)W + (uint32_t)(c0 + k), n4);
#pragma unroll
            for (int q = 0; q < 4; ++q) sl[(q * PXL + k) * 64] = n4[q];
          }
        }
      }
      PIPE_TICK_SYNC();
    };
    for (int t = 0; t < T_end; t += 4) static_for<0, 4>([&](auto uu) { tick(uu, t + decltype(uu)::value); });
  } else {
    auto c_role = [&](auto vm_tag) __attribute__((always_inline)) {
    constexpr bool VM = decltype(vm_tag)::value;
    const float gam = A.tv.gamma;
    const float* const hin = lds + L::o_hand + (NT - 1) * 8 * RP;
    constexpr int HSTR = CHAIN ? 2 * RP : 4 * RP;
    float* const slab = slab_base + lane;
    double gacc = 0.0;
    float crr[2][PXL], xprev[PXL];
#pragma unroll
    for (int k = 0; k < PXL; ++k) crr[0][k] = crr[1][k] = xprev[k] = 0.f;
    const bool want_obj = RT && !state_only && A.rt_base + kc < A.rt_total;
    double osq = 0.0, otv = 0.0;
    float pprev[RT ? PXL : 1];
#pragma unroll
    for (int k = 0; k < (RT ? PXL : 1); ++k) pprev[k] = 0.f;
    constexpr bool PM = RT && !AL;
    float cmx[PM ? PXL : 1], cmy[PM ? PXL : 1];
    if constexpr (PM) {
#pragma unroll
      for (int j = 0; j < PXL; ++j) {
        const bool in = c0 + j >= st_lo && c0 + j < st_hi;
        cmx[j] = in ? 1.f : 0.f;
        cmy[j] = in && c0 + j + 1 < W ? 1.f : 0.f;
      }
    }
    float exq[4][PXL];
#pragma unroll
    for (int u = 0; u < 4; ++u)
#pragma unroll
      for (int k = 0; k < PXL; ++k) exq[u][k] = 0.f;
    constexpr bool XT = TEAMS == 1;
    if (XT && VM && A.extra) {
#pragma unroll
      for (int u = 0; u < 3; ++u) {
        const int r = u - D;
        gload_raw<PXL>(exq[u], A.extra + (size_t)chain * img + (size_t)min(max(r, 0), H - 1) * W, cl, W, al);
      }
    }
    auto tick = [&](auto uu, const int t) __attribute__((always_inline)) {
      constexpr int U = decltype(uu)::value, P = U & 1;
      constexpr int NI = ((U - D) % 4 + 4) % 4;
      const int o = t - D;
      if (state_only) { PIPE_TICK_SYNC(); return; }
      if (XT && VM && A.extra) {
        const int r3 = o + 3;
        gload_raw<PXL>(exq[(U + 3) & 3], A.extra + (size_t)chain * img + (size_t)min(max(r3, 0), H - 1) * W, cl, W, al);
      }
      float css[PXL], xo[PXL], gv[PXL], prox[PXL];
      prow_load<PXL>(crr[P], hin + (P ^ 1) * HSTR, lane);
      prow_load<PXL>(css, hin + (P ^ 1) * HSTR + RP, lane);
      prow_load<PXL>(xo, ring_row(o), lane);
      if (KT > 0 || A.data_kind == LMC_DATA_IDENTITY || A.data_kind == LMC_DATA_MASK) {
        prow_load<PXL>(gv, lds + L::o_g + (P ^ 1) * RP, lane);
      } else {
#pragma unroll
        for (int j = 0; j < PXL; ++j) gv[j] = 0.f;
      }
      const float ssl0 = (TEAMS == 2 && TM == 1) ? wave_from_left(css[PXL - 1], seam[SA + (P ^ 1) * 2 * (NT + 1) + 2 * NT]) : dpp_left0(css[PXL - 1]);
      float dvs = 0.f;
#pragma unroll
      for (int j = 0; j < PXL; ++j) {
        const float ssl = j == 0 ? ssl0 : css[j - 1];
        const float dv = (crr[P][j] - crr[P ^ 1][j]) + (css[j] - ssl);
        prox[j] = fmaf(-gam, dv, xo[j]);
        if constexpr (PM) { const float dm = dv * cmx[j]; dvs = fmaf(dm, dm, dvs); }
        else if constexpr (RT) dvs = fmaf(dv, dv, dvs);
      }
      if constexpr (RT) {
        if (want_obj && o >= 0 && o < H) {
          osq += (double)dvs;
          if (o >= 1) {
            const float pr_last = dpp_right0(pprev[0]);
            float tvs = 0.f;
#pragma unroll
            for (int j = 0; j < PXL; ++j) {
              if constexpr (PM) {
                const float dx = (prox[j] - pprev[j]) * cmx[j];
                const float dy = ((j == PXL - 1 ? pr_last : pprev[j + 1]) - pprev[j]) * cmy[j];
                tvs += __builtin_amdgcn_sqrtf(fmaf(dx, dx, dy * dy));
              } else {
                const float dx = prox[j] - pprev[j];
                const float dy = (c0 + j + 1 < W) ? (j == PXL - 1 ? pr_last : pprev[j + 1]) - pprev[j] : 0.f;
                tvs += __builtin_amdgcn_sqrtf(fmaf(dx, dx, dy * dy));
              }
            }
            otv += (double)tvs;
          }
#pragma unroll
          for (int j = 0; j < PXL; ++j) pprev[j] = prox[j];
        }
      }
      if (XT && A.ncvx_kind == LMC_NCVX_MC_TV) {
        float xp[PXL], vx[PXL], vy[PXL];
        prow_load<PXL>(xp, ring_row(o + 1), lane);
        const float x0_r = dpp_right0(xo[0]);
        const bool an = A.ncvx_gamma < 0.f, rowin = o >= 0 && o < H, down = o + 1 < H;
        const float gth = fabsf(A.ncvx_gamma);
#pragma unroll
        for (int j = 0; j < PXL; ++j) {
          const float dx = (rowin && down) ? xp[j] - xo[j] : 0.f;
          const float dy = (rowin && c0 + j + 1 < W) ? (j == PXL - 1 ? x0_r : xo[j + 1]) - xo[j] : 0.f;
          if (an) {
            vx[j] = __builtin_amdgcn_rcpf(fmaxf(fabsf(dx), gth)) * dx;
            vy[j] = __builtin_amdgcn_rcpf(fmaxf(fabsf(dy), gth)) * dy;
          } else {
            const float w = __builtin_amdgcn_rcpf(fmaxf(__builtin_amdgcn_sqrtf(fmaf(dx, dx, dy * dy)), gth));
            vx[j] = w * dx;
            vy[j] = w * dy;
          }
        }
        const float vy_l = dpp_left0(vy[PXL - 1]);
#pragma unroll
        for (int j = 0; j < PXL; ++j) {
          gv[j] -= A.ncvx_lambda * -((vx[j] - xprev[j]) + (vy[j] - (j == 0 ? vy_l : vy[j - 1])));
          xprev[j] = vx[j];
        }
      }
      if (XT && A.g_out && o >= 0 && o < H) {
        float xq[PXL];
        prow_load<PXL>(xq, ring_row(o + 1), lane);
        const float xr_last = dpp_right0(xo[0]);
        const bool down = o + 1 < H;
#pragma unroll
        for (int j = 0; j < PXL; ++j) {
          const float dx = down ? xq[j] - xo[j] : 0.f;
          const float dy = (c0 + j + 1 < W) ? (j == PXL - 1 ? xr_last : xo[j + 1]) - xo[j] : 0.f;
          gacc += (double)__builtin_amdgcn_sqrtf(fmaf(dx, dx, dy * dy));
        }
      }
      if (o >= 0 && o < H) {
        const float* const slr = slab + ((o >> 2) & 1) * (4 * PXL * 64);
        const size_t go = (size_t)o * W;
#pragma unroll
        for (int g = 0; g < PXL / 4; ++g) {
          if (c0 + 4 * g < st_hi && c0 + 4 * g + 3 >= st_lo) {
            float xi[4] = {0.f, 0.f, 0.f, 0.f}, ex[4] = {0.f, 0.f, 0.f, 0.f};
            if (A.noise_mode == LMC_NOISE_PHILOX) {
#pragma unroll
              for (int q = 0; q < 4; ++q) xi[q] = slr[(NI * PXL + 4 * g + q) * 64];
            } else if (VM && A.noise_mode == LMC_NOISE_INJECTED) {
              const float* nrow = A.noise + (size_t)chain * img + go;
              if (al) {
                const float4 v = *reinterpret_cast<const float4*>(nrow + c0 + 4 * g);
                xi[0] = v.x; xi[1] = v.y; xi[2] = v.z; xi[3] = v.w;
              } else load4_dword_aligned(xi[0], xi[1], xi[2], xi[3], nrow, c0 + 4 * g, W);
            }
            if (XT && VM && A.extra) {
              ex[0] = exq[U][4 * g]; ex[1] = exq[U][4 * g + 1]; ex[2] = exq[U][4 * g + 2]; ex[3] = exq[U][4 * g + 3];
              if constexpr (!AL) unshift4_dword_aligned(ex[0], ex[1], ex[2], ex[3], c0 + 4 * g, W);
            }
            float ov[4];
#pragma unroll
            for (int q = 0; q < 4; ++q) {
              const float x = xo[4 * g + q];
              float gr = gv[4 * g + q];
              if (XT && VM && A.extra) gr = fmaf(A.extra_coef, x - ex[q], gr);
              ov[q] = fmaf(A.a, x, fmaf(-A.t, gr, fmaf(A.b, prox[4 * g + q], A.s * xi[q])));
            }
            gstore4(xout + go, c0 + 4 * g, st_lo, st_hi, al, ov[0], ov[1], ov[2], ov[3]);
          }
        }
      }
      PIPE_TICK_SYNC();
    };
    for (int t = 0; t < T_end; t += 4) static_for<0, 4>([&](auto uu) { tick(uu, t + decltype(uu)::value); });
    if (XT && A.g_out) {
      const double tot = wave_sum(gacc);
      if (lane == 0) unsafeAtomicAdd(&A.g_out[chain], (double)A.g_scale * tot);
    }
    if constexpr (RT) {
      if (want_obj) {
        const float pr_last = dpp_right0(pprev[0]);
        float tvs = 0.f;
#pragma unroll
        for (int j = 0; j < PXL; ++j) {
          if constexpr (PM) tvs += fabsf((j == PXL - 1 ? pr_last : pprev[j + 1]) - pprev[j]) * cmy[j];
          else tvs += (c0 + j + 1 < W) ? fabsf((j == PXL - 1 ? pr_last : pprev[j + 1]) - pprev[j]) : 0.f;
        }
        otv += (double)tvs;
        const double dg = (double)gam;
        const double tot = wave_sum(0.5 * dg * dg * osq + dg * otv);
        if (lane == 0) unsafeAtomicAdd(A.rt_obj + (size_t)chain * A.rt_stride + A.rt_base + kc, tot);
      }
    }
    };
    if (A.extra != nullptr || A.noise_mode == LMC_NOISE_INJECTED) c_role(std::true_type{});
    else c_role(std::false_type{});
  }
  };
  if constexpr (TEAMS == 2) {
    if (team) roles(std::integral_constant<int, 1>{});
    else roles(std::integral_constant<int, 0>{});
  } else {
    roles(std::integral_constant<int, 0>{});
  }
}

template <int K, int PXL, int KT, bool CHAIN = false, bool WARM = false, bool AL = true, bool RT = false>
__global__ __launch_bounds__(64 * ((K + 1) / 2 + 3), (PXL == 8 || CHAIN) ? (WARM ? LMC_WARM_MIN_WAVES : 1) : 2) void myula_step_pipe_kernel(const StepArgs A) {
  pipe_body<K, PXL, KT, CHAIN, WARM, AL, RT, 1>(A);
}

template <int K, int KT>
__global__ __launch_bounds__(128 * ((K + 1) / 2 + 3), 4) void myula_step_pipe2_kernel(const StepArgs A) {
  pipe_body<K, 4, KT, false, false, true, false, 2>(A);
}


template <int K, int PXL, int KT, bool CHAIN = false>
static constexpr size_t pipe_lds_bytes() { return sizeof(float) * (size_t)PipeLds<K, PXL, CHAIN>::total; }

template <int PXL, int KT, bool CHAIN, int K = 10, bool WARM = false, bool AL = true, bool RT = false>
static hipError_t pipe_launch_one(const StepArgs& a, hipStream_t st) {
  auto kern = myula_step_pipe_kernel<K, PXL, KT, CHAIN, WARM, AL, RT>;
  constexpr size_t lb = pipe_lds_bytes<K, PXL, KT, CHAIN>();
  static bool attr_set[64] = {};
  int dev = 0;
  hipError_t e = hipGetDevice(&dev);
  if (e != hipSuccess) return e;
  if (dev < 0 || dev >= 64 || !attr_set[dev]) {
    e = hipFuncSetAttribute(reinterpret_cast<const void*>(kern), hipFuncAttributeMaxDynamicSharedMemorySize, (int)lb);
    if (e != hipSuccess) return e;
    if (dev >= 0 && dev < 64) attr_set[dev] = true;
  }
  const int BWk = 64 * PXL, U = BWk - 2 * pipe_halo(K, KT, PXL);
  const int nstrips = a.W <= BWk ? 1 : (a.W + U - 1) / U;
#ifdef LMC_EXP_PERM
  StepArgs b = a;
  if (const char* e = getenv("LMC_EXP_PERM")) b.PH = (int)strtoul(e, nullptr, 16);
  hipLaunchKernelGGL(kern, dim3(a.C, nstrips), dim3(64 * ((K + 1) / 2 + 3)), lb, st, b);
  return hipGetLastError();
#endif
  hipLaunchKernelGGL(kern, dim3(a.C, nstrips), dim3(64 * ((K + 1) / 2 + 3)), lb, st, a);
  return hipGetLastError();
}

template <int K, int KT>
static hipError_t pipe_launch_teams(const StepArgs& a, hipStream_t st) {
  auto kern = myula_step_pipe2_kernel<K, KT>;
  constexpr size_t lb = sizeof(float) * (size_t)PipeLds<K, 4, false, 2>::total;
  static_assert(lb <= 160 * 1024, "LDS of one workgroup");
  static bool attr_set[64] = {};
  int dev = 0;
  hipError_t e = hipGetDevice(&dev);
  if (e != hipSuccess) return e;
  if (dev < 0 || dev >= 64 || !attr_set[dev]) {
    e = hipFuncSetAttribute(reinterpret_cast<const void*>(kern), hipFuncAttributeMaxDynamicSharedMemorySize, (int)lb);
    if (e != hipSuccess) return e;
    if (dev >= 0 && dev < 64) attr_set[dev] = true;
  }
  hipLaunchKernelGGL(kern, dim3(a.C), dim3(128 * ((K + 1) / 2 + 3)), lb, st, a);
  return hipGetLastError();
}

template <int K, bool CHAIN>
static hipError_t pipe_dispatch_unaligned(const StepArgs& a, int KT, hipStream_t st) {
  if (a.W > 256) {
    if (KT == 5) return pipe_launch_one<8, 5, CHAIN, K, false, false>(a, st);
    if (KT == 7) return pipe_launch_one<8, 7, CHAIN, K, false, false>(a, st);
    return pipe_launch_one<8, 0, CHAIN, K, false, false>(a, st);
  }
  if (KT == 5) return pipe_launch_one<4, 5, CHAIN, K, false, false>(a, st);
  if (KT == 7) return pipe_launch_one<4, 7, CHAIN, K, false, false>(a, st);
  return pipe_launch_one<4, 0, CHAIN, K, false, false>(a, st);
}

template <int K, bool CHAIN, bool WARM = false>
static hipError_t pipe_dispatch_k(const StepArgs& a, int KT, hipStream_t st) {
  const bool lastlane = (a.W & (a.W > 256 ? 7 : 3)) == 0;
  if constexpr (K == 10 && !WARM) {
    if (!lastlane) return pipe_dispatch_unaligned<K, CHAIN>(a, KT, st);
  }
  if (!lastlane) return hipErrorInvalidConfiguration;
  if (a.W > 256) {
    if (KT == 5) return pipe_launch_one<8, 5, CHAIN, K, WARM>(a, st);
    if (KT == 7) return pipe_launch_one<8, 7, CHAIN, K, WARM>(a, st);
    return pipe_launch_one<8, 0, CHAIN, K, WARM>(a, st);
  }
  if (KT == 5) return pipe_launch_one<4, 5, CHAIN, K, WARM>(a, st);
  if (KT == 7) return pipe_launch_one<4, 7, CHAIN, K, WARM>(a, st);
  return pipe_launch_one<4, 0, CHAIN, K, WARM>(a, st);
}

bool pipe_geometry_ok(const StepArgs& a);
int pipe_taps(StepArgs& a);

hipError_t pipe_dispatch_chain(const StepArgs& a, int K, int KT, hipStream_t st);

}
```

Before: 596,100 chain-it/s.

## Stream multiple chains through persistent two-team pipe workgroups

Turns the two-team pipelined MYULA step kernel into a persistent kernel. It launches at most one workgroup per CU, or a cap set by LMC_PIPE_WGS, and each workgroup streams its chains back-to-back through the same row pipeline. Per-role row/chain cursors (StackRow) replace the per-chain row indices so loads, noise generation and stores follow the stacked chain sequence. The aim is to pay pipeline fill and drain once per workgroup rather than once per chain, and to avoid tail imbalance from 1024 separate workgroups. The cost is lower concurrency per CU (one resident workgroup instead of several) and extra index bookkeeping.

Result: no change. 592,600 chain-it/s (-0.6%).

```diff
diff --git a/include/lmc_atomi.h b/include/lmc_atomi.h
--- a/include/lmc_atomi.h
+++ b/include/lmc_atomi.h
@@ -174,6 +174,7 @@
 int lmc_sampler_enable_timing(lmc_sampler* s, int32_t on);
 int lmc_sampler_last_step_timing(lmc_sampler* s, float* total_ms, int32_t* n_launches);
 const char* lmc_sampler_kernel_name(const lmc_sampler* s);
+int32_t lmc_sampler_step_workgroups(const lmc_sampler* s);
 int lmc_sampler_tv_exit_stats(lmc_sampler* s, int32_t which, int32_t* passes_dev, uint64_t* reruns_host, void* stream);
 
 #define LMC_RCCL_UNIQUE_ID_BYTES 128
diff --git a/lmc_atomi_amd/_capi.py b/lmc_atomi_amd/_capi.py
--- a/lmc_atomi_amd/_capi.py
+++ b/lmc_atomi_amd/_capi.py
@@ -128,6 +128,7 @@
     "lmc_sampler_enable_timing": (C.c_int, [_P, C.c_int32]),
     "lmc_sampler_last_step_timing": (C.c_int, [_P, C.POINTER(C.c_float), C.POINTER(C.c_int32)]),
     "lmc_sampler_kernel_name": (C.c_char_p, [_P]),
+    "lmc_sampler_step_workgroups": (C.c_int32, [_P]),
     "lmc_sampler_tv_exit_stats": (C.c_int, [_P, C.c_int32, _P, C.POINTER(C.c_uint64), _P]),
     "lmc_set_step_variant": (C.c_int, [C.c_int32]),
     "lmc_ulpda_create": (C.c_int, [C.POINTER(lmc_ulpda_config), C.POINTER(_P)]),
diff --git a/lmc_atomi_amd/algs.py b/lmc_atomi_amd/algs.py
--- a/lmc_atomi_amd/algs.py
+++ b/lmc_atomi_amd/algs.py
@@ -144,6 +144,10 @@
     @property
     def kernel_name(self):
         return _dev.lib().lmc_sampler_kernel_name(self._h).decode()
+
+    @property
+    def step_workgroups(self):
+        return int(_dev.lib().lmc_sampler_step_workgroups(self._h))
 
     def tv_exit_stats(self, which="prior"):
         passes = torch.empty(self.n_chains, dtype=torch.int32, device=self.device)
diff --git a/lmc_atomi_amd/csrc/lmc_host.h b/lmc_atomi_amd/csrc/lmc_host.h
--- a/lmc_atomi_amd/csrc/lmc_host.h
+++ b/lmc_atomi_amd/csrc/lmc_host.h
@@ -125,7 +125,7 @@
 int variant_of(const Problem& q);
 float tol_of(const Problem& q);
 hipError_t launch_step(const lmc::StepArgs& A_in, int variant, hipStream_t st, const char** name, float* state0 = nullptr,
-                       float* state1 = nullptr, float* pxbuf = nullptr);
+                       float* state1 = nullptr, float* pxbuf = nullptr, int pipe_wgs = 0, int* pipe_wgs_out = nullptr);
 
 int cg_solve_fused(const Problem& q, float ts, float* u, const float* rhs, float* r, float* p, float* qq, double* scal,
                    int64_t C, int niter, const float* zero_y, hipStream_t st, float* alt_out = nullptr, float** result = nullptr);
@@ -163,6 +163,7 @@
   int pol_blockpair = 1;
   int pol_overlap = 0;
   int pol_bg_wgs = -1;
+  int pol_pipe_wgs = 0;
   lmc::host::Problem prob;
   int C = 0;
   int64_t chain_offset = 0;
@@ -192,4 +193,5 @@
   bool timed = false;
   int last_launches = 0;
   std::string kernel_name;
+  int step_wgs = 0;
 };
diff --git a/lmc_atomi_amd/csrc/lmc_launch.h b/lmc_atomi_amd/csrc/lmc_launch.h
--- a/lmc_atomi_amd/csrc/lmc_launch.h
+++ b/lmc_atomi_amd/csrc/lmc_launch.h
@@ -68,7 +68,8 @@
 int centred_blur_taps(const BlurTaps& T, float* uc, float* vc);
 bool pipe_supported(const StepArgs& a);
 int pipe_links(const StepArgs& a);
-hipError_t launch_step_pipe(StepArgs a, hipStream_t st, float* state0 = nullptr, float* state1 = nullptr, int teams = 0);
+hipError_t launch_step_pipe(StepArgs a, hipStream_t st, float* state0 = nullptr, float* state1 = nullptr, int teams = 0, int wgs_cap = 0,
+                            int* wgs_out = nullptr);
 bool pipe_teams_covered(const StepArgs& a, int KT);
 bool pipe_warm_supported(const StepArgs& a);
 hipError_t launch_step_pipe_warm(StepArgs a, hipStream_t st);
diff --git a/lmc_atomi_amd/csrc/lmc_problem.hip b/lmc_atomi_amd/csrc/lmc_problem.hip
--- a/lmc_atomi_amd/csrc/lmc_problem.hip
+++ b/lmc_atomi_amd/csrc/lmc_problem.hip
@@ -166,7 +166,9 @@
 int variant_of(const Problem& q) { return q.variant ? q.variant : g_variant; }
 float tol_of(const Problem& q) { return q.implicit_tol > 0.f ? q.implicit_tol : (q.implicit_tol < 0.f ? 0.f : g_cg_tol); }
 
-hipError_t launch_step(const lmc::StepArgs& A_in, int variant, hipStream_t st, const char** name, float* state0, float* state1, float* pxbuf) {
+hipError_t launch_step(const lmc::StepArgs& A_in, int variant, hipStream_t st, const char** name, float* state0, float* state1, float* pxbuf, int pipe_wgs,
+                       int* pipe_wgs_out) {
+  if (pipe_wgs_out) *pipe_wgs_out = 0;
   int v = variant;
   if ((v == 0 || v == 5) && lmc::block_supported(A_in)) {
     if (name) *name = "myula_step_block_kernel";
@@ -200,7 +202,7 @@
     const int links = lmc::pipe_links(A);
     if (links == 1 || (links > 1 && state0 && state1 && v != 8)) {
       if (name) *name = "myula_step_pipe_kernel";
-      return lmc::launch_step_pipe(A, st, state0, state1, v == 7 ? 1 : v == 8 ? 2 : 0);
+      return lmc::launch_step_pipe(A, st, state0, state1, v == 7 ? 1 : v == 8 ? 2 : 0, pipe_wgs, pipe_wgs_out);
     }
   }
   if (v == 7 || v == 8) return hipErrorInvalidConfiguration;
diff --git a/lmc_atomi_amd/csrc/lmc_sampler.hip b/lmc_atomi_amd/csrc/lmc_sampler.hip
--- a/lmc_atomi_amd/csrc/lmc_sampler.hip
+++ b/lmc_atomi_amd/csrc/lmc_sampler.hip
@@ -1,3 +1,4 @@
+#include <algorithm>
 #include <cmath>
 #include <cstdlib>
 #include <new>
@@ -95,6 +96,7 @@
     s->pol_blockpair = ipl == 1 ? 0 : (ipl == 2 ? 1 : (env_int("LMC_BLOCK_PAIR", 1) != 0));
     s->pol_overlap = q.moments_overlap ? q.moments_overlap : (getenv("LMC_MOMENTS_OVERLAP") ? (env_int("LMC_MOMENTS_OVERLAP", 0) ? 1 : -1) : 0);
     s->pol_bg_wgs = q.moments_bg_wgs > 0 ? q.moments_bg_wgs : env_int("LMC_MOMENTS_BG_WGS", -1);
+    s->pol_pipe_wgs = std::max(0, env_int("LMC_PIPE_WGS", 0));
     if (q.prox_scale) { s->pol_pair = 0; s->pol_blockpair = 0; }
   }
   if (e == hipSuccess && s->prob.tv_warm) {
@@ -369,7 +371,7 @@
     kname = "myula_step_pipe_kernel(warm)";
     s->wcur ^= 1;
   } else {
-    e = launch_step(A, variant_of(s->prob), st, &kname, s->tvstate[0], s->tvstate[1], s->pxbuf);
+    e = launch_step(A, variant_of(s->prob), st, &kname, s->tvstate[0], s->tvstate[1], s->pxbuf, s->pol_pipe_wgs, &s->step_wgs);
   }
   if (e == hipErrorInvalidConfiguration) return fail(LMC_E_UNSUPPORTED, "no step-kernel variant covers this configuration");
   HIP_TRY(e);
@@ -734,6 +736,7 @@
 }
 
 const char* lmc_sampler_kernel_name(const lmc_sampler* s) { return s ? s->kernel_name.c_str() : ""; }
+int32_t lmc_sampler_step_workgroups(const lmc_sampler* s) { return s ? s->step_wgs : 0; }
 
 int lmc_sampler_tv_exit_stats(lmc_sampler* s, int32_t which, int32_t* passes_dev, uint64_t* reruns_host, void* stream) {
   if (!s || (which != 0 && which != 1)) return fail(LMC_E_INVALID, "bad arguments");
diff --git a/lmc_atomi_amd/csrc/lmc_step_pipe.hip b/lmc_atomi_amd/csrc/lmc_step_pipe.hip
--- a/lmc_atomi_amd/csrc/lmc_step_pipe.hip
+++ b/lmc_atomi_amd/csrc/lmc_step_pipe.hip
@@ -60,13 +60,14 @@
          a.ncvx_kind == LMC_NCVX_NONE && !a.extra;
 }
 
-hipError_t launch_step_pipe(StepArgs a, hipStream_t st, float* state0, float* state1, int teams) {
+hipError_t launch_step_pipe(StepArgs a, hipStream_t st, float* state0, float* state1, int teams, int wgs_cap, int* wgs_out) {
+  if (wgs_out) *wgs_out = 0;
   const int links = pipe_links(a);
   if (links == 0 || (links > 1 && (!state0 || !state1))) return hipErrorInvalidConfiguration;
   const int KT = pipe_taps(a);
   const bool two = links == 1 && pipe_teams_covered(a, KT);
   if (teams == 2 && !two) return hipErrorInvalidConfiguration;
-  if (two && teams != 1) return pipe_launch_teams<10, 5>(a, st);
+  if (two && teams != 1) return pipe_launch_teams<10, 5>(a, st, wgs_cap, wgs_out);
   if (links == 1) {
     switch (a.tv.niter) {
       case 2: return pipe_dispatch_k<2, false>(a, KT, st);
diff --git a/lmc_atomi_amd/csrc/lmc_step_pipe_kernel.h b/lmc_atomi_amd/csrc/lmc_step_pipe_kernel.h
--- a/lmc_atomi_amd/csrc/lmc_step_pipe_kernel.h
+++ b/lmc_atomi_amd/csrc/lmc_step_pipe_kernel.h
@@ -1,4 +1,5 @@
 #pragma once
+#include <algorithm>
 #include "lmc_device.h"
 #include "lmc_launch.h"
 
@@ -238,11 +239,28 @@
   return (need + PXL - 1) / PXL * PXL;
 }
 
+struct StackGeom { int Pd, first, last, step; };
+struct StackRow {
+  int c, r;
+  __device__ __forceinline__ void init(int s, const StackGeom& g) {
+    c = g.first; r = s;
+    while (r >= g.Pd && c < g.last) { r -= g.Pd; c += g.step; }
+  }
+  __device__ __forceinline__ void next(const StackGeom& g) {
+    ++r;
+    const int lim = c < g.last ? g.Pd : 0x7fffffff;
+    const bool wrap = r == lim;
+    r = wrap ? 0 : r;
+    c += wrap ? g.step : 0;
+  }
+};
+
 #ifndef LMC_PIPE2_ROLES
 #define LMC_PIPE2_ROLES 0x5D3BC4A291E6F780ull
 #endif
-template <int K, int PXL, int KT, bool CHAIN, bool WARM, bool AL, bool RT, int TEAMS>
+template <int K, int PXL, int KT, bool CHAIN, bool WARM, bool AL, bool RT, int TEAMS, bool STREAM = false>
 __device__ __forceinline__ void pipe_body(const StepArgs& A) {
+  static_assert(!STREAM || TEAMS == 2, "chains streamed through a workgroup: the two-team kernel only");
   static_assert(!WARM || CHAIN, "the warm dual uses the state hand-over of the chained launches");
   static_assert(!RT || (!WARM && (K & 1) == 0), "per-chain exit: cold start, even K");
   static_assert(!RT || AL || pipe_halo(K, KT, PXL) >= K + 2, "per-chain exit on column strips: the halo holds the objective's extra column");
@@ -325,7 +343,15 @@
   constexpr int SA = 0, SB = 4 * (NT + 1), SR = SB + 4 * NT;
   static_assert(TEAMS == 1 || SR + 8 <= L::total - L::o_seam, "seam records");
 
-  const int T_end = (H + D + 3) & ~3;
+  StackGeom sg{0, chain, chain, 0};
+  int jl = 0;
+  if constexpr (STREAM) {
+    sg.step = (int)gridDim.x;
+    jl = (A.C - 1 - chain) / sg.step;
+    sg.Pd = (H + 5) & ~3;
+    sg.last = chain + jl * sg.step;
+  }
+  const int T_end = (jl * sg.Pd + H + D + 3) & ~3;
   float* const xring = lds + L::o_x;
   auto ring_row = [&](int row) -> float* { return xring + ((unsigned)(row + RB) % (unsigned)RB) * RP; };
 
@@ -393,6 +419,13 @@
           gload_raw<PXL>(spre[u][f], sin ? sin + (size_t)f * img + (size_t)min(max(rs, 0), H - 1) * W : xin, c0, W, al);
       }
     }
+    StackRow s_pub, s_xpf, s_ypf, s_res;
+    if constexpr (STREAM) {
+      s_pub.init(0, sg);
+      s_xpf.init(kXPF, sg);
+      s_ypf.init(kYPF + 1 - D + (KT - 1) - HW + LAGT, sg);
+      s_res.init(1 - D + (KT - 1) + LAGT - HW, sg);
+    }
     double facc = 0.0;
     float Rprev[TEAMS == 2 ? PXL : 1];
 #pragma unroll
@@ -400,7 +433,7 @@
     auto tick = [&](auto uu, const int t) __attribute__((always_inline)) {
       constexpr int U = decltype(uu)::value, P = U & 1;
       if constexpr (KT > 0) {
-        const int r3 = t + kYPF + 1 - D + (KT - 1) - HW + LAGT;
+        const int r3 = STREAM ? s_ypf.r : t + kYPF + 1 - D + (KT - 1) - HW + LAGT;
         gload_raw<PXL>(ypre[(U + kYPF) & 3], A.y + (size_t)min(max(r3, 0), H - 1) * W, cl, W, al);
       } else if (pw_id || pw_mask) {
         const size_t ro = (size_t)min(max(t + kYPF + 1 - D, 0), H - 1) * W;
@@ -411,9 +444,10 @@
         float xv[PXL];
         gfix_raw<PXL, AL>(xpre[U], c0, W);
 #pragma unroll
-        for (int k = 0; k < PXL; ++k) xv[k] = (t < H && col_in(k)) ? xpre[U][k] : 0.f;
+        for (int k = 0; k < PXL; ++k) xv[k] = ((STREAM ? s_pub.r : t) < H && col_in(k)) ? xpre[U][k] : 0.f;
         prow_store<PXL>(ring_row(t), lane, xv);
-        gload_raw<PXL>(xpre[U], xin + (size_t)min(t + kXPF, H - 1) * W, cl, W, al);
+        if constexpr (STREAM) gload_raw<PXL>(xpre[U], A.x_in + ((size_t)s_xpf.c * H + min(s_xpf.r, H - 1)) * W, cl, W, al);
+        else gload_raw<PXL>(xpre[U], xin + (size_t)min(t + kXPF, H - 1) * W, cl, W, al);
       }
       if constexpr (CHAIN) {
         float* hb = lds + L::o_hand0 + P * 4 * RP;
@@ -457,7 +491,8 @@
       const int r = i - HW;
       float R[PXL];
       {
-        const bool rowok = r >= 0 && r < H;
+        const int rl = STREAM ? s_res.r : r;
+        const bool rowok = rl >= 0 && rl < H;
         const float rmask = rowok ? 1.f : 0.f;
         gfix_raw<PXL, AL>(ypre[U & 3], c0, W);
 #pragma unroll
@@ -535,6 +570,7 @@
           prow_store<PXL>(lds + L::o_g + P * RP, lane, gout);
         }
       }
+      if constexpr (STREAM) { s_pub.next(sg); s_xpf.next(sg); s_ypf.next(sg); s_res.next(sg); }
       PIPE_TICK_SYNC();
     };
     for (int t = 0; t < T_end; t += 4) static_for<0, 4>([&](auto uu) { tick(uu, t + decltype(uu)::value); });
@@ -637,6 +673,8 @@
     constexpr bool SL = TEAMS == 2 && TM == 1, SRt = TEAMS == 2 && TM == 0;
     const float* const seam_in = seam + (TM == 1 ? SA + 2 * wave - 2 : SB + 2 * (wave - 1));
     float* const seam_out = seam + (TM == 0 ? SA + 2 * wave - 1 : SB + 2 * (wave - 1));
+    StackRow s_b1, s_b2;
+    if constexpr (STREAM) { s_b1.init(-E - 2 * k1 - 1, sg); s_b2.init(-E - 2 * k2 - 1, sg); }
     auto tick = [&](auto uu, const int t) __attribute__((always_inline)) {
       constexpr int P = decltype(uu)::value & 1;
       const int a2 = t - E - 2 * k2, a1 = t - E - 2 * k1;
@@ -644,7 +682,7 @@
       if constexpr (TEAMS == 2) edge = *reinterpret_cast<const float2*>(seam_in + (P ^ 1) * (TM == 1 ? 2 * (NT + 1) : 2 * NT));
       float ss2_edge = 0.f;
       if constexpr (!SINGLE) {
-        const float cdown = ((unsigned)(a2 - 1) >= (unsigned)(H - 1)) ? 0.f : cstep;
+        const float cdown = ((unsigned)(STREAM ? s_b2.r : a2 - 1) >= (unsigned)(H - 1)) ? 0.f : cstep;
         DualRow<NP> out;
         if (live2) {
           StageObj ob;
@@ -679,7 +717,7 @@
         }
         if (live1) {
           pairs_load<NP>(xk[P], ring_row(a1), lane);
-          const float cdown = ((unsigned)(a1 - 1) >= (unsigned)(H - 1)) ? 0.f : cstep;
+          const float cdown = ((unsigned)(STREAM ? s_b1.r : a1 - 1) >= (unsigned)(H - 1)) ? 0.f : cstep;
           StageObj ob;
           om.md = cdown != 0.f ? 1.f : 0.f;
           if constexpr (FIRST) pipe_stage_first<NP, AL, RT, SRt>(xk[P], sol1, cdown, crc, beta1, o1[P], &ob, &om, edge.x);
@@ -698,6 +736,7 @@
           so[1] = TM == 0 ? ss2_edge : sol2[0].x;
         }
       }
+      if constexpr (STREAM) { s_b1.next(sg); s_b2.next(sg); }
       PIPE_TICK_SYNC();
     };
     for (int t = 0; t < T_end; t += 4) static_for<0, 4>([&](auto uu) { tick(uu, t + decltype(uu)::value); });
@@ -732,24 +771,29 @@
   } else if (wave == NT + 2) {
     float* const slab = slab_base + lane;
     const uint32_t iter = A.iteration;
+    StackRow s_q;
+    if constexpr (STREAM) s_q.init(4 - D, sg);
     auto tick = [&](auto uu, const int t) __attribute__((always_inline)) {
       constexpr int U = decltype(uu)::value;
       constexpr int NI = ((U - D) % 4 + 4) % 4;
       const int o = t - D;
       if (A.noise_mode == LMC_NOISE_PHILOX && !state_only) {
-        const int qn = ((o - NI) >> 2) + 1;
+        const int qs = ((o - NI) >> 2) + 1;
+        const int qn = STREAM ? (s_q.r - NI) >> 2 : qs;
+        const uint32_t qchain = STREAM ? (uint32_t)s_q.c : (uint32_t)chain;
         if (qn >= 0 && 4 * qn < H) {
-          float* const sl = slab + (qn & 1) * (4 * PXL * 64);
+          float* const sl = slab + (qs & 1) * (4 * PXL * 64);
 #pragma unroll
           for (int kk = 0; kk < PXL / 4; ++kk) {
             const int k = NI * (PXL / 4) + kk;
             float n4[4];
-            quad_normals(A.key0, A.key1, iter, A.chain_offset + (uint32_t)chain, (uint32_t)qn * (uint32_t)W + (uint32_t)(c0 + k), n4);
+            quad_normals(A.key0, A.key1, iter, A.chain_offset + qchain, (uint32_t)qn * (uint32_t)W + (uint32_t)(c0 + k), n4);
 #pragma unroll
             for (int q = 0; q < 4; ++q) sl[(q * PXL + k) * 64] = n4[q];
           }
         }
       }
+      if constexpr (STREAM) s_q.next(sg);
       PIPE_TICK_SYNC();
     };
     for (int t = 0; t < T_end; t += 4) static_for<0, 4>([&](auto uu) { tick(uu, t + decltype(uu)::value); });
@@ -792,10 +836,13 @@
         gload_raw<PXL>(exq[u], A.extra + (size_t)chain * img + (size_t)min(max(r, 0), H - 1) * W, cl, W, al);
       }
     }
+    StackRow s_o;
+    if constexpr (STREAM) s_o.init(-D, sg);
     auto tick = [&](auto uu, const int t) __attribute__((always_inline)) {
       constexpr int U = decltype(uu)::value, P = U & 1;
       constexpr int NI = ((U - D) % 4 + 4) % 4;
       const int o = t - D;
+      const int ol = STREAM ? s_o.r : o;
       if (state_only) { PIPE_TICK_SYNC(); return; }
       if (XT && VM && A.extra) {
         const int r3 = o + 3;
@@ -883,9 +930,9 @@
           gacc += (double)__builtin_amdgcn_sqrtf(fmaf(dx, dx, dy * dy));
         }
       }
-      if (o >= 0 && o < H) {
+      if (ol >= 0 && ol < H) {
         const float* const slr = slab + ((o >> 2) & 1) * (4 * PXL * 64);
-        const size_t go = (size_t)o * W;
+        const size_t go = (size_t)ol * W;
 #pragma unroll
         for (int g = 0; g < PXL / 4; ++g) {
           if (c0 + 4 * g < st_hi && c0 + 4 * g + 3 >= st_lo) {
@@ -894,7 +941,7 @@
 #pragma unroll
               for (int q = 0; q < 4; ++q) xi[q] = slr[(NI * PXL + 4 * g + q) * 64];
             } else if (VM && A.noise_mode == LMC_NOISE_INJECTED) {
-              const float* nrow = A.noise + (size_t)chain * img + go;
+              const float* nrow = A.noise + (size_t)(STREAM ? s_o.c : chain) * img + go;
               if (al) {
                 const float4 v = *reinterpret_cast<const float4*>(nrow + c0 + 4 * g);
                 xi[0] = v.x; xi[1] = v.y; xi[2] = v.z; xi[3] = v.w;
@@ -912,10 +959,11 @@
               if (XT && VM && A.extra) gr = fmaf(A.extra_coef, x - ex[q], gr);
               ov[q] = fmaf(A.a, x, fmaf(-A.t, gr, fmaf(A.b, prox[4 * g + q], A.s * xi[q])));
             }
-            gstore4(xout + go, c0 + 4 * g, st_lo, st_hi, al, ov[0], ov[1], ov[2], ov[3]);
+            gstore4(STREAM ? A.x_out + (size_t)s_o.c * img + go : xout + go, c0 + 4 * g, st_lo, st_hi, al, ov[0], ov[1], ov[2], ov[3]);
           }
         }
       }
+      if constexpr (STREAM) s_o.next(sg);
       PIPE_TICK_SYNC();
     };
     for (int t = 0; t < T_end; t += 4) static_for<0, 4>([&](auto uu) { tick(uu, t + decltype(uu)::value); });
@@ -956,9 +1004,9 @@
   pipe_body<K, PXL, KT, CHAIN, WARM, AL, RT, 1>(A);
 }
 
-template <int K, int KT>
+template <int K, int KT, bool STREAM = true>
 __global__ __launch_bounds__(128 * ((K + 1) / 2 + 3), 4) void myula_step_pipe2_kernel(const StepArgs A) {
-  pipe_body<K, 4, KT, false, false, true, false, 2>(A);
+  pipe_body<K, 4, KT, false, false, true, false, 2, STREAM>(A);
 }
 
 
@@ -991,7 +1039,7 @@
 }
 
 template <int K, int KT>
-static hipError_t pipe_launch_teams(const StepArgs& a, hipStream_t st) {
+static hipError_t pipe_launch_teams(const StepArgs& a, hipStream_t st, int wgs_cap = 0, int* wgs_out = nullptr) {
   auto kern = myula_step_pipe2_kernel<K, KT>;
   constexpr size_t lb = sizeof(float) * (size_t)PipeLds<K, 4, false, 2>::total;
   static_assert(lb <= 160 * 1024, "LDS of one workgroup");
@@ -1004,7 +1052,17 @@
     if (e != hipSuccess) return e;
     if (dev >= 0 && dev < 64) attr_set[dev] = true;
   }
-  hipLaunchKernelGGL(kern, dim3(a.C), dim3(128 * ((K + 1) / 2 + 3)), lb, st, a);
+  static int n_cu[64] = {};
+  int cus = (dev >= 0 && dev < 64) ? n_cu[dev] : 0;
+  if (cus <= 0) {
+    e = hipDeviceGetAttribute(&cus, hipDeviceAttributeMultiprocessorCount, dev);
+    if (e != hipSuccess) return e;
+    if (cus <= 0) return hipErrorInvalidDevice;
+    if (dev >= 0 && dev < 64) n_cu[dev] = cus;
+  }
+  const int wgs = std::max(1, std::min(a.C, wgs_cap > 0 ? wgs_cap : cus));
+  if (wgs_out) *wgs_out = wgs;
+  hipLaunchKernelGGL(kern, dim3(wgs), dim3(128 * ((K + 1) / 2 + 3)), lb, st, a);
   return hipGetLastError();
 }
 
```
